# gradslam/gradslam

Measured on AMD Instinct MI355X. Metric: frames/sec PointFusion 640x480 RGB-D, higher is better.
Workload: dtype f32

## Files before the change

gradslam_amd/_C.py:

```python
import ctypes as C
import os

import torch

_HERE = os.path.dirname(os.path.abspath(__file__))
LIB_PATH = os.environ.get("GRADSLAM_HIP_LIB") or os.path.join(_HERE, "csrc", "libgradslam_hip.so")
if os.environ.get("GRADSLAM_HIP_LIB"):
    import warnings
    warnings.warn("GRADSLAM_HIP_LIB overrides the product library: %s" % LIB_PATH, RuntimeWarning)
ABI_VERSION = 3

_lib = None

_vp, _i64, _i32, _f = C.c_void_p, C.c_int64, C.c_int, C.c_float


class IcpParams(C.Structure):
    _fields_ = [("mode", C.c_int), ("numiters", C.c_int), ("damp", C.c_float),
                ("dist_thresh", C.c_float), ("lambda_max", C.c_float), ("B", C.c_float),
                ("B2", C.c_float), ("nu", C.c_float)]


class MapView(C.Structure):
    _fields_ = [("points", C.c_void_p), ("normals", C.c_void_p), ("colors", C.c_void_p), ("ccounts", C.c_void_p),
                ("capacity", C.c_int64), ("n_bound", C.c_int64), ("n_dev", C.c_void_p)]


class LocalizeSeq(C.Structure):
    _fields_ = [("vertex", C.c_void_p), ("depth", C.c_void_p), ("K16", C.c_void_p), ("prev_pose16", C.c_void_p),
                ("map", MapView), ("out_pose16", C.c_void_p), ("scratch", C.c_void_p)]


class UpdateSeq(C.Structure):
    _fields_ = [("map", MapView), ("vertex", C.c_void_p), ("normal", C.c_void_p), ("depth", C.c_void_p),
                ("rgb", C.c_void_p), ("alpha", C.c_void_p), ("pose16", C.c_void_p), ("K16", C.c_void_p),
                ("gvertex", C.c_void_p), ("gnormal", C.c_void_p), ("best_pix", C.c_void_p),
                ("new_count_out", C.c_void_p), ("scratch", C.c_void_p)]


class StepSeq(C.Structure):
    _fields_ = [("depth", C.c_void_p), ("rgb", C.c_void_p), ("K16", C.c_void_p), ("prev_pose16", C.c_void_p),
                ("out_pose16", C.c_void_p), ("vertex", C.c_void_p), ("normal", C.c_void_p), ("alpha", C.c_void_p),
                ("gvertex", C.c_void_p), ("gnormal", C.c_void_p), ("best_pix", C.c_void_p),
                ("new_count_out", C.c_void_p), ("map", MapView), ("loc_scratch", C.c_void_p),
                ("upd_scratch", C.c_void_p)]


class RenderSeq(C.Structure):
    _fields_ = [("map", MapView), ("poses16", C.c_void_p), ("K16", C.c_void_p), ("depth", C.c_void_p),
                ("color", C.c_void_p), ("normal", C.c_void_p), ("confidence", C.c_void_p), ("index", C.c_void_p),
                ("scratch", C.c_void_p)]


_PROTOS = {
    "gs_abi_version": [],
    "gs_last_error": [],
    "gs_scratch_bytes": [_i64, _i64],
    "gs_profile_begin": [_i32],
    "gs_profile_end": [],
    "gs_profile_read": [_i32, C.POINTER(C.c_double), C.POINTER(C.c_int64), C.POINTER(C.c_double)],
    "gs_frame_maps_f32": [_vp, _vp, _i32, _i32, _f, _vp, _vp, _vp, _vp, _vp],
    "gs_global_maps_f32": [_vp, _vp, _vp, _vp, _i32, _i32, _vp, _vp, _vp],
    "gs_alpha_f32": [_vp, _i64, _f, _f, _vp, _vp],
    "gs_alpha_backward_f32": [_vp, _i64, _f, _f, _vp, _vp, _vp, _vp],
    "gs_downsample_frame_f32": [_vp, _vp, _vp, _vp, _i32, _i32, _i32, _vp, _vp, _vp, _vp, _vp, _vp],
    "gs_project_map_f32": [_vp, _i64, _vp, _vp, _i32, _i32, _vp, _vp],
    "gs_active_table_i64": [_vp, _i64, _i32, _i64, _vp, _vp, _vp, _vp],
    "gs_select_targets_f32": [_vp, _i64, _i32, _i32, _vp, _vp, _vp, _vp, _vp, _vp, _i64, _vp, _vp, _vp],
    "gs_downsample_table_f32": [_vp, _i64, _i32, _vp, _vp, _vp, _vp, _vp, _vp, _vp, _vp, _vp],
    "gs_knn1_f32": [_vp, _i64, _vp, _i64, _vp, _vp, _vp, _vp],
    "gs_knn1_grid_scratch_bytes": [_i64, _i64],
    "gs_knn1_grid_f32": [_vp, _i64, _vp, _i64, _vp, _vp, _vp, C.POINTER(C.c_int64), _vp],
    "gs_gauss_newton_rows_f32": [_vp, _i64, _vp, _vp, _i64, _f, _vp, _vp, _vp, _vp, _vp, _vp],
    "gs_solve_normal_eq_f32": [_vp, _vp, _vp, _i64, _i32, _f, _vp, _vp],
    "gs_se3_exp_f32": [_vp, _vp, _vp],
    "gs_se3_exp_backward_f32": [_vp, _vp, _vp, _vp],
    "gs_transform_points_f32": [_vp, _i64, _vp, _vp, _vp],
    "gs_icp_scratch_bytes": [_i64, _i64],
    "gs_icp_f32": [_vp, _i64, _vp, _vp, _i64, _vp, _vp, C.POINTER(IcpParams), _vp, _vp, _vp, _vp],
    "gs_icp_trace_f32": [_vp, _i32, _vp, _vp],
    "gs_icp_dc_f32": [_vp, _i64, _vp, _vp, _vp, _i64, _vp, _vp, _vp, C.POINTER(IcpParams), _vp, _vp, _vp, _vp],
    "gs_frame_maps_backward_f32": [_vp, _vp, _i32, _i32, _f, _vp, _vp, _vp, _vp, _vp, _vp, _vp, _vp],
    "gs_frame_maps_backward_kbar_scratch_bytes": [_i32, _i32],
    "gs_global_maps_backward_f32": [_vp, _vp, _vp, _vp, _i32, _i32, _vp, _vp, _vp],
    "gs_downsample_frame_backward_f32": [_vp, _vp, _i32, _i32, _i32, _vp, _vp, _vp],
    "gs_icp_tape_bytes": [_i64, _i32],
    "gs_icp_tape_f32": [_vp, _i64, _vp, _vp, _i64, _vp, _vp, C.POINTER(IcpParams), _vp, _vp, _vp, _vp, _vp],
    "gs_icp_backward_scratch_bytes": [_i64, _i64],
    "gs_icp_backward_f32": [_vp, _vp, _i64, _vp, _vp, _i64, _vp, C.POINTER(IcpParams), _vp, _vp, _vp, _vp, _vp, _vp,
                            _vp],
    "gs_similar_rows_f32": [_vp, _i64, _vp, _vp, _vp, _vp, _i32, _f, _f, _vp, _vp],
    "gs_best_unique_rows_f32": [_vp, _i64, _vp, _vp, _vp, _i32, _i32, _i64, _vp, _vp, _vp, _vp, _vp],
    "gs_associate_f32": [_vp, _i64, _vp, _vp, _vp, _vp, _vp, _i32, _i32, _f, _f, _vp, _vp, _vp, _vp],
    "gs_best_table_i64": [_vp, _i32, _i32, _i64, _vp, _vp, _vp, _vp],
    "gs_rows_to_best_pix": [_vp, _i64, _i32, _i32, _vp, _vp],
    "gs_fuse_append_f32": [_vp, _vp, _vp, _vp, _i64, _i64, _vp, _vp, _vp, _vp, _vp, _vp, _i32, _i32, _i32,
                           _vp, _vp, _vp],
    "gs_append_valid_f32": [_vp, _vp, _vp, _vp, _i64, _i64, _vp, _vp, _vp, _vp, _vp, _i32, _i32, _vp, _vp, _vp],
    "gs_ingest_depth_u16_f32": [_vp, _i32, _i32, _vp, _i32, _i32, C.c_double, _vp],
    "gs_ingest_color_u8_f32": [_vp, _i32, _i32, _vp, _i32, _i32, _i32, _vp],
    "gs_ingest_frames_native_f32": [_vp, _vp, _i64, _i32, _i32, C.c_double, _i32, _vp, _vp, _vp],
    "gs_host_device_pointer": [_vp, C.POINTER(C.c_void_p)],
    "gs_global_maps_pose_backward_scratch_bytes": [_i32, _i32],
    "gs_global_maps_pose_backward_f32": [_vp, _vp, _vp, _vp, _vp, _i32, _i32, _vp, _vp, _vp],
    "gs_fuse_append_backward_f32": [_vp, _vp, _vp, _vp, _i64, _vp, _vp, _vp, _vp, _vp, _vp, _i32, _i32, _i32, _vp, _vp,
                                    _vp, _vp, _i64, _vp, _vp, _vp, _vp, _vp, _vp, _vp, _vp, _vp, _vp],
    "gs_update_map_scratch_bytes": [_i64, _i32, _i32],
    "gs_update_map_fusion_dc_f32": [_vp, _vp, _vp, _vp, _i64, _vp, _i64, _vp, _vp, _vp, _vp, _vp, _vp, _vp, _i32, _i32,
                                    _f, _f, _i32, _vp, _vp, _vp, _vp, _vp, _vp],
    "gs_icp_map_dc_f32": [_vp, _i64, _vp, _vp, _vp, _vp, _i64, _vp, _i32, _i32, _vp, _vp, C.POINTER(IcpParams), _vp, _vp,
                          _vp],
    "gs_lattice_source_f32": [_vp, _vp, _vp, _i32, _i32, _i32, _vp, _vp],
    "gs_relative_pose_f32": [_vp, _vp, _i64, _vp, _vp],
    "gs_project_map_dc_f32": [_vp, _i64, _vp, _vp, _vp, _i32, _i32, _vp, _vp],
    "gs_select_targets_dc_f32": [_vp, _i64, _vp, _i32, _i32, _vp, _vp, _vp, _vp, _vp, _vp, _i64, _vp, _vp, _vp],
    "gs_associate_dc_f32": [_vp, _i64, _vp, _vp, _vp, _vp, _vp, _vp, _i32, _i32, _f, _f, _vp, _vp, _vp, _vp],
    "gs_fuse_append_dc_f32": [_vp, _vp, _vp, _vp, _i64, _vp, _i64, _vp, _vp, _vp, _vp, _vp, _vp, _i32, _i32, _i32,
                              _vp, _vp, _vp],
    "gs_append_valid_dc_f32": [_vp, _vp, _vp, _vp, _i64, _vp, _i64, _vp, _vp, _vp, _vp, _vp, _i32, _i32, _vp, _vp,
                               _vp],
    "gs_frame_maps_batch_f32": [_vp, _i64, _i64, _vp, _i32, _i32, _i32, _i32, _f, _vp, _vp, _vp, _vp],
    "gs_localize_scratch_bytes": [_i32, _i32, _i32, _i64],
    "gs_localize_batch_f32": [C.POINTER(LocalizeSeq), _i32, _i32, _i32, _i32, C.POINTER(IcpParams), _vp],
    "gs_update_map_fusion_batch_f32": [C.POINTER(UpdateSeq), _i32, _i32, _i32, _f, _f, _i32, _vp],
    "gs_project_points_f32": [_vp, _i32, _i64, _vp, _i64, _vp, _vp],
    "gs_unproject_points_f32": [_vp, _i32, _i64, _vp, _i64, _vp, _vp, _vp],
    "gs_lie_small_f32": [_i32, _vp, _vp, _vp],
    "gs_localize_far_stats_i64": [_vp, _i32, _i32, _i32, _i64, C.POINTER(C.c_int64), _vp],
    "gs_localize_list_stats_i64": [_vp, _i32, _i32, _i32, _i64, C.POINTER(C.c_int64), _vp],
    "gs_localize_solve_stats_i64": [_vp, _i32, _i32, _i32, _i64, C.POINTER(C.c_int64), _vp],
    "gs_pointfusion_step_batch_f32": [C.POINTER(StepSeq), _i32, _i32, _i32, _i32, C.POINTER(IcpParams), _f, _f, _f, _i32, _vp],
    "gs_render_scratch_bytes": [_i32, _i32, _i32],
    "gs_render_map_dc_f32": [C.POINTER(RenderSeq), _i32, _i32, _i32, _i32, _i32, _f, _i32, _vp],
}
_RESTYPE = {"gs_last_error": C.c_char_p, "gs_scratch_bytes": _i64, "gs_icp_scratch_bytes": _i64,
            "gs_knn1_grid_scratch_bytes": _i64, "gs_update_map_scratch_bytes": _i64, "gs_global_maps_pose_backward_scratch_bytes": _i64, "gs_icp_tape_bytes": _i64, "gs_icp_backward_scratch_bytes": _i64,
            "gs_localize_scratch_bytes": _i64, "gs_frame_maps_backward_kbar_scratch_bytes": _i64,
            "gs_render_scratch_bytes": _i64}
EXPORTS = tuple(_PROTOS)


class HipExtensionError(RuntimeError):
    pass


def lib():
    global _lib
    if _lib is None:
        if not os.path.exists(LIB_PATH):
            raise HipExtensionError(
                "gradslam_amd: %s is missing. Build it with `python -m gradslam_amd.csrc.build` "
                "(hipcc --offload-arch=gfx950). There is no CPU / PyTorch fallback." % LIB_PATH)
        handle = C.CDLL(LIB_PATH)
        for name, argtypes in _PROTOS.items():
            fn = getattr(handle, name)
            fn.argtypes = argtypes
            fn.restype = _RESTYPE.get(name, C.c_int)
        if handle.gs_abi_version() != ABI_VERSION:
            raise HipExtensionError("libgradslam_hip.so ABI %d != expected %d; rebuild"
                                    % (handle.gs_abi_version(), ABI_VERSION))
        _lib = handle
    return _lib


def check(status, what):
    if status != 0:
        raise HipExtensionError("%s failed (code %d): %s" % (what, status, lib().gs_last_error().decode()))


def require_device(*tensors):
    dev = None
    for t in tensors:
        if t is None:
            continue
        if not t.is_cuda:
            raise HipExtensionError(
                "gradslam_amd kernels run on the GPU only (got a %s tensor). Move the data to a HIP "
                "device; there is no CPU fallback." % t.device)
        if not t.is_contiguous():
            raise HipExtensionError("internal error: non-contiguous tensor passed to the HIP library")
        if dev is None:
            dev = t.device
        elif t.device != dev:
            raise HipExtensionError("tensors live on different devices: %s vs %s" % (dev, t.device))
    return dev


def ptr(t):
    return None if t is None else C.c_void_p(t.data_ptr())


def stream(device):
    return C.c_void_p(torch.cuda.current_stream(device).cuda_stream)


class Workspace:
    _instances = {}

    def __init__(self, device):
        self.device = device
        self._bufs = {}

    @classmethod
    def get(cls, device):
        device = torch.device(device)
        if device.index is None:
            device = torch.device("cuda", torch.cuda.current_device())
        key = (device, torch.cuda.current_stream(device).cuda_stream)
        ws = cls._instances.get(key)
        if ws is None:
            ws = cls._instances[key] = Workspace(device)
        return ws

    def bytes(self, name, nbytes):
        buf = self._bufs.get(name)
        if buf is None or buf.numel() < nbytes:
            nbytes = int(nbytes * 1.5) + 4096
            buf = self._bufs[name] = torch.empty(nbytes, dtype=torch.uint8, device=self.device)
        return buf

    def scratch(self, n_map, n_pix):
        return self.bytes("scratch", lib().gs_scratch_bytes(int(n_map), int(n_pix)))

    def tensor(self, name, shape, dtype):
        n = 1
        for s in shape:
            n *= int(s)
        item = torch.empty((), dtype=dtype).element_size()
        buf = self.bytes(name, max(n, 1) * item)
        return buf[: n * item].view(dtype).view(*shape)
```

gradslam_amd/csrc/gs_common.h:

```cpp
#pragma once
#include <hip/hip_runtime.h>
#include <atomic>
#include <stdint.h>
#include <stdio.h>

#include "../../include/gradslam_hip.h"

#define GS_ABI_VERSION 3

constexpr int GS_MAX_BATCH = 8;
struct GsClearJob {
  int n;
  size_t bytes;
  char* ptr[GS_MAX_BATCH];
};
constexpr int GS_CLEAR_ITEMS = 8;
struct GsPixelTables {
  int n;
  uint64_t* key_pix[GS_MAX_BATCH];
  int32_t* best_pix[GS_MAX_BATCH];
  int32_t* any_flag[GS_MAX_BATCH];
  int32_t* call_flag;
};
int gs_frame_maps_batch_clear(const float* depth, int64_t depth_stride_seq, int64_t depth_stride_frame, const float* K16,
                              int n_frames, int frames_per_K, int H, int W, float two_sigma_sq, float* vertex,
                              float* normal, float* alpha, const GsClearJob* job, void* stream,
                              const GsPixelTables* tables = nullptr);

int gs_update_map_fusion_batch_impl(const gs_update_seq* seqs_host, int B, int H, int W, float dist_th, float dot_th,
                                    int renorm_all, void* stream, bool tables_ready);
int32_t* gs_update_map_call_flag(void* scratch_of_first_sequence);
void gs_update_map_tables(void* scratch, int32_t** any_flag, uint64_t** key_pix);

void gs_set_error(const char* fmt, ...);

#define GS_REQUIRE(cond, msg)                  \
  do {                                         \
    if (!(cond)) {                             \
      gs_set_error("%s: %s", __func__, msg);   \
      return GS_ERR_INVALID;                   \
    }                                          \
  } while (0)

#define GS_HIP(call)                                                            \
  do {                                                                          \
    hipError_t e_ = (call);                                                     \
    if (e_ != hipSuccess) {                                                     \
      gs_set_error("%s: %s -> %s", __func__, #call, hipGetErrorString(e_));     \
      return GS_ERR_HIP;                                                        \
    }                                                                           \
  } while (0)

#define GS_LAUNCH_CHECK() GS_HIP(hipGetLastError())

static inline hipStream_t gs_stream(void* s) { return reinterpret_cast<hipStream_t>(s); }
static inline int64_t gs_ceil_div(int64_t a, int64_t b) { return (a + b - 1) / b; }
static inline size_t gs_align(size_t x, size_t a = 256) { return (x + a - 1) / a * a; }

enum GsProfKind { GS_PROF_KNN = 0, GS_PROF_LINEARIZE = 1, GS_PROF_FRAME = 2, GS_PROF_PROJECT = 3,
                  GS_PROF_ASSOC = 4, GS_PROF_FUSE = 5, GS_PROF_COMPACT = 6, GS_PROF_SOLVE = 7, GS_PROF_ICP_FUSED = 8,
                  GS_PROF_KINDS = 9 };
extern std::atomic<bool> g_gs_prof_on;
int gs_prof_open(int kind, double work, hipStream_t st, int launches);
void gs_prof_close(int slot, hipStream_t st);
struct GsProf {
  int slot;
  hipStream_t st;
  GsProf(int kind, double work, hipStream_t s, int launches = 1) : slot(-1), st(s) {
    if (g_gs_prof_on) slot = gs_prof_open(kind, work, s, launches);
  }
  ~GsProf() {
    if (slot >= 0) gs_prof_close(slot, st);
  }
};

#define GS_DEV __device__ __forceinline__

GS_DEV float gs_fma(float a, float b, float c) { return __builtin_fmaf(a, b, c); }

GS_DEV float gs_dot3_fma(float a0, float a1, float a2, float b0, float b1, float b2) {
  float acc = a0 * b0;
  acc = gs_fma(a1, b1, acc);
  acc = gs_fma(a2, b2, acc);
  return acc;
}
GS_DEV float gs_dot3_plain(float a0, float a1, float a2, float b0, float b1, float b2) {
  float p0 = a0 * b0, p1 = a1 * b1, p2 = a2 * b2;
  float s = p0 + p1;
  return s + p2;
}
GS_DEV float gs_norm3(float x, float y, float z) {
  float acc = x * x;
  acc = gs_fma(y, y, acc);
  acc = gs_fma(z, z, acc);
  return __builtin_sqrtf(acc);
}

GS_DEV float gs_expf_spec(float x) {
  if (x < -87.0f) return 0.0f;
  if (x > 88.0f) return __builtin_inff();
  float n = __builtin_rintf(x * 1.44269504088896341f);
  float r = gs_fma(-n, 0.693359375f, x);
  r = gs_fma(-n, -2.12194440e-4f, r);
  float p = 1.9875691500e-4f;
  p = gs_fma(p, r, 1.3981999507e-3f);
  p = gs_fma(p, r, 8.3334519073e-3f);
  p = gs_fma(p, r, 4.1665795894e-2f);
  p = gs_fma(p, r, 1.6666665459e-1f);
  p = gs_fma(p, r, 5.0000001201e-1f);
  float r2 = r * r;
  float y = gs_fma(p, r2, r);
  y = y + 1.0f;
  int32_t bits = __float_as_int(y) + (((int32_t)n) << 23);
  return __int_as_float(bits);
}

GS_DEV float gs_alpha_of(float vx, float vy, float vz, float two_sigma_sq, float eps) {
  float s = vx * vx + vy * vy;
  s = s + vz * vz;
  float a = gs_expf_spec((-s) / two_sigma_sq);
  a = a < eps ? eps : a;
  a = a > 1.01f ? 1.01f : a;
  return a;
}

struct GsKinv {
  float k00, k11, k02, k12;
};
GS_DEV GsKinv gs_kinv(const float* __restrict__ K) {
  const float eps = 1e-6f;
  float fx = K[0], fy = K[5], cx = K[2], cy = K[6];
  GsKinv r;
  r.k00 = 1.0f / (fx + eps);
  r.k11 = 1.0f / (fy + eps);
  r.k02 = (-1.0f * cx) / (fx + eps);
  r.k12 = (-1.0f * cy) / (fy + eps);
  return r;
}

GS_DEV void gs_rigid_fma(const float* __restrict__ T, float p0, float p1, float p2, float& o0,
                         float& o1, float& o2) {
  o0 = gs_dot3_fma(T[0], T[1], T[2], p0, p1, p2) + T[3];
  o1 = gs_dot3_fma(T[4], T[5], T[6], p0, p1, p2) + T[7];
  o2 = gs_dot3_fma(T[8], T[9], T[10], p0, p1, p2) + T[11];
}

struct GsCount {
  int64_t host;
  const int64_t* dev;
};
GS_DEV int64_t gs_count(const GsCount c) {
  if (!c.dev) return c.host;
  const int64_t raw = *c.dev;
  const uint32_t lo = (uint32_t)__builtin_amdgcn_readfirstlane((int)(uint32_t)raw);
  const uint32_t hi = (uint32_t)__builtin_amdgcn_readfirstlane((int)(uint32_t)((uint64_t)raw >> 32));
  const int64_t v = (int64_t)(((uint64_t)hi << 32) | lo);
  return v < c.host ? (v < 0 ? 0 : v) : c.host;
}

constexpr int GS_WAVE = 64;

GS_DEV int gs_wave_incl_scan(int v) {
  const int lane = threadIdx.x & (GS_WAVE - 1);
#pragma unroll
  for (int d = 1; d < GS_WAVE; d <<= 1) {
    int t = __shfl_up(v, d, GS_WAVE);
    if (lane >= d) v += t;
  }
  return v;
}

template <int BLOCK>
GS_DEV int gs_block_excl_scan(int v, int* smem, int* total) {
  constexpr int NW = BLOCK / GS_WAVE;
  const int lane = threadIdx.x & (GS_WAVE - 1);
  const int wave = threadIdx.x / GS_WAVE;
  int incl = gs_wave_incl_scan(v);
  if (lane == GS_WAVE - 1) smem[wave] = incl;
  __syncthreads();
  if (threadIdx.x == 0) {
    int run = 0;
    for (int w = 0; w < NW; ++w) {
      int c = smem[w];
      smem[w] = run;
      run += c;
    }
    smem[NW] = run;
  }
  __syncthreads();
  int base = smem[wave];
  *total = smem[NW];
  __syncthreads();
  return base + incl - v;
}

GS_DEV double gs_wave_sum_f64(double v) {
#pragma unroll
  for (int d = GS_WAVE / 2; d > 0; d >>= 1) v += __shfl_down(v, d, GS_WAVE);
  return v;
}
```

gradslam_amd/csrc/gs_frame.hip:

```cpp
#include <stdarg.h>
#include <string.h>

#include "gs_compact.h"

static thread_local char g_err[512] = "";

void gs_set_error(const char* fmt, ...) {
  va_list ap;
  va_start(ap, fmt);
  vsnprintf(g_err, sizeof(g_err), fmt, ap);
  va_end(ap);
}

#include <mutex>
#include <vector>
std::atomic<bool> g_gs_prof_on{false};
namespace {
std::mutex g_prof_mu;
struct ProfRec { hipEvent_t a, b; int kind; double work; bool closed; int launches; };
std::vector<ProfRec> g_prof;
size_t g_prof_used = 0;
double g_prof_ms[GS_PROF_KINDS], g_prof_work[GS_PROF_KINDS];
int64_t g_prof_n[GS_PROF_KINDS];
}
// ... 12 lines not shown
}

extern "C" int gs_profile_begin(int max_records) {
  GS_REQUIRE(max_records > 0 && max_records <= (1 << 20), "max_records out of range");
  std::lock_guard<std::mutex> lock(g_prof_mu);
  while (g_prof.size() < (size_t)max_records) {
    ProfRec r;
    GS_HIP(hipEventCreate(&r.a));
    GS_HIP(hipEventCreate(&r.b));
    r.kind = 0; r.work = 0; r.closed = false; r.launches = 1;
    g_prof.push_back(r);
  }
  g_prof_used = 0;
  for (int k = 0; k < GS_PROF_KINDS; ++k) { g_prof_ms[k] = 0; g_prof_work[k] = 0; g_prof_n[k] = 0; }
  g_gs_prof_on = true;
  return GS_OK;
}
extern "C" int gs_profile_end(void) {
  g_gs_prof_on = false;
  GS_HIP(hipDeviceSynchronize());
  std::lock_guard<std::mutex> lock(g_prof_mu);
  for (size_t i = 0; i < g_prof_used; ++i) {
    const ProfRec& r = g_prof[i];
    if (!r.closed) continue;
    float ms = 0.f;
    if (hipEventElapsedTime(&ms, r.a, r.b) != hipSuccess) continue;
    g_prof_ms[r.kind] += ms; g_prof_work[r.kind] += r.work; g_prof_n[r.kind] += r.launches;
  }
  return GS_OK;
}
extern "C" int gs_profile_read(int kind, double* ms_total, int64_t* launches, double* work_total) {
  GS_REQUIRE(kind >= 0 && kind < GS_PROF_KINDS && ms_total && launches && work_total, "bad arguments");
  std::lock_guard<std::mutex> lock(g_prof_mu);
  *ms_total = g_prof_ms[kind]; *launches = g_prof_n[kind]; *work_total = g_prof_work[kind];
  return GS_OK;
}

extern "C" int gs_abi_version(void) { return GS_ABI_VERSION; }
extern "C" const char* gs_last_error(void) { return g_err; }

extern "C" int64_t gs_scratch_bytes(int64_t n_map, int64_t n_pix) {
  int64_t n = n_map > n_pix ? n_map : n_pix;
  return (int64_t)(gs_cp_scratch_bytes(n) + gs_align(8 * (size_t)(n_pix > 0 ? n_pix : 1)) +
                   gs_align(8 * (size_t)(n_map > 0 ? n_map : 1)) + 4096);
}

__global__ void gs_cp_scan_tiles_kernel(const int32_t* __restrict__ tile_counts, int64_t ntiles,
                                        int64_t* __restrict__ tile_offsets,
                                        int64_t* __restrict__ count_out, GsCount base_count) {
  __shared__ int smem[1024 / GS_WAVE + 1];
  __shared__ int64_t carry;
  if (threadIdx.x == 0) carry = 0;
  __syncthreads();
  for (int64_t t0 = 0; t0 < ntiles; t0 += 1024) {
    int64_t t = t0 + threadIdx.x;
    int c = (t < ntiles) ? tile_counts[t] : 0;
    int total;
    int excl = gs_block_excl_scan<1024>(c, smem, &total);
    if (t < ntiles) tile_offsets[t] = carry + excl;
    __syncthreads();
    if (threadIdx.x == 0) carry += total;
    __syncthreads();
  }
  if (threadIdx.x == 0 && count_out) count_out[0] = gs_count(base_count) + carry;
}

constexpr int FM_TW = 64;
constexpr int FM_TH = 8;
constexpr int FM_LW = FM_TW + 2;
constexpr int FM_LH = FM_TH + 2;

GS_DEV void fm_vertex(float d, int h, int w, const GsKinv& k, float& x, float& y, float& z) {
  float u = (float)w, v = (float)h;
  float ax = k.k00 * u;
  ax = gs_fma(0.0f, v, ax);
  ax = gs_fma(k.k02, 1.0f, ax);
  float ay = 0.0f * u;
  ay = gs_fma(k.k11, v, ay);
  ay = gs_fma(k.k12, 1.0f, ay);
  float az = 0.0f * u;
  az = gs_fma(0.0f, v, az);
  az = gs_fma(1.0f, 1.0f, az);
  float validf = d > 0.0f ? 1.0f : 0.0f;
  x = (ax * d) * validf;
  y = (ay * d) * validf;
  z = (az * d) * validf;
}

struct GsRow3 {
  float x, y, z;
};
GS_DEV void frame_maps_body(const float* __restrict__ depth, const float* __restrict__ K16, int H, int W,
                            float two_sigma_sq, float* __restrict__ vertex, float* __restrict__ normal,
                            float* __restrict__ alpha, uint8_t* __restrict__ valid,
                            uint64_t* __restrict__ key_pix = nullptr, int32_t* __restrict__ best_pix = nullptr) {
  __shared__ float tile[FM_LH][FM_LW];
  const int w_base = blockIdx.x * FM_TW, h_base = blockIdx.y * FM_TH;
  for (int i = threadIdx.x; i < FM_LH * FM_LW; i += 256) {
    int lh = i / FM_LW, lw = i - lh * FM_LW;
    int gh = h_base + lh - 1, gw = w_base + lw - 1;
    gh = gh < 0 ? 0 : (gh > H - 1 ? H - 1 : gh);
    gw = gw < 0 ? 0 : (gw > W - 1 ? W - 1 : gw);
    tile[lh][lw] = depth[(size_t)gh * W + gw];
  }
  __syncthreads();
  const GsKinv k = gs_kinv(K16);
  const int lane = threadIdx.x & 63, wave = threadIdx.x >> 6;
  const int w = w_base + lane;
  if (w >= W) return;
#pragma unroll
  for (int r = 0; r < 2; ++r) {
    const int lh = wave * 2 + r;
    const int h = h_base + lh;
    if (h >= H) continue;
    const size_t p = (size_t)h * W + w;
    const float d = tile[lh + 1][lane + 1];
    float vx, vy, vz;
    fm_vertex(d, h, w, k, vx, vy, vz);
    if (vertex) reinterpret_cast<GsRow3*>(vertex)[p] = GsRow3{vx, vy, vz};
    if (valid) valid[p] = d > 0.0f ? 1 : 0;
    if (alpha) alpha[p] = gs_alpha_of(vx, vy, vz, two_sigma_sq, 1e-7f);
    if (key_pix) { key_pix[p] = ~0ull; best_pix[p] = -1; }
    if (normal) {
      const int w0 = (w < W - 1) ? w : W - 2;
      const int h0 = (h < H - 1) ? h : H - 2;
      const int lw0 = w0 - w_base + 1, lh0 = h0 - h_base + 1;
      float a0x, a0y, a0z, a1x, a1y, a1z, b0x, b0y, b0z, b1x, b1y, b1z;
      fm_vertex(tile[lh + 1][lw0], h, w0, k, a0x, a0y, a0z);
      fm_vertex(tile[lh + 1][lw0 + 1], h, w0 + 1, k, a1x, a1y, a1z);
      fm_vertex(tile[lh0][lane + 1], h0, w, k, b0x, b0y, b0z);
      fm_vertex(tile[lh0 + 1][lane + 1], h0 + 1, w, k, b1x, b1y, b1z);
      const float dhx = a1x - a0x, dhy = a1y - a0y, dhz = a1z - a0z;
      const float dvx = b1x - b0x, dvy = b1y - b0y, dvz = b1z - b0z;
      const float nx = gs_fma(dhy, dvz, -(dhz * dvy));
      const float ny = gs_fma(dhz, dvx, -(dhx * dvz));
      const float nz = gs_fma(dhx, dvy, -(dhy * dvx));
      const float nrm = gs_norm3(nx, ny, nz);
      const float den = (nrm == 0.0f) ? 1.0f : nrm;
      const float validf = d > 0.0f ? 1.0f : 0.0f;
      reinterpret_cast<GsRow3*>(normal)[p] = GsRow3{(nx / den) * validf, (ny / den) * validf, (nz / den) * validf};
    }
  }
}

__global__ void __launch_bounds__(256) gs_frame_maps_kernel(
    const float* __restrict__ depth, const float* __restrict__ K16, int H, int W, float two_sigma_sq,
    float* __restrict__ vertex, float* __restrict__ normal, float* __restrict__ alpha,
    uint8_t* __restrict__ valid) {
  frame_maps_body(depth, K16, H, W, two_sigma_sq, vertex, normal, alpha, valid);
}
__global__ void __launch_bounds__(256) gs_frame_maps_batch_kernel(
    const float* __restrict__ depth, int64_t stride_seq, int64_t stride_frame, const float* __restrict__ K16,
    int frames_per_K, int H, int W, float two_sigma_sq, float* __restrict__ vertex, float* __restrict__ normal,
    float* __restrict__ alpha, const int n_frames, const GsClearJob job, const GsPixelTables tabs) {
  if ((int)blockIdx.z >= n_frames) {
    const size_t blk = ((size_t)(blockIdx.z - n_frames) * gridDim.y + blockIdx.y) * gridDim.x + blockIdx.x;
    const size_t n16 = job.bytes / 16, per = (n16 + 256 * GS_CLEAR_ITEMS - 1) / (256 * GS_CLEAR_ITEMS);
    const size_t r = blk / per;
    if (r >= (size_t)job.n) return;
    float4* dst = reinterpret_cast<float4*>(job.ptr[r]);
    const size_t base = (blk % per) * 256 * GS_CLEAR_ITEMS + threadIdx.x;
#pragma unroll
    for (int u = 0; u < GS_CLEAR_ITEMS; ++u) {
      const size_t i = base + (size_t)u * 256;
      if (i < n16) dst[i] = make_float4(0.0f, 0.0f, 0.0f, 0.0f);
    }
    return;
  }
  const size_t f = blockIdx.z, P = (size_t)H * W;
  const size_t b = f / frames_per_K, l = f % frames_per_K;
  const bool tb = (int)f < tabs.n;
  if (tb && blockIdx.x == 0 && blockIdx.y == 0 && threadIdx.x == 0) {
    tabs.any_flag[f][0] = 0;
    tabs.any_flag[f][1] = 0;
    if (f == 0 && tabs.call_flag) *tabs.call_flag = 0;
  }
  frame_maps_body(depth + b * stride_seq + l * stride_frame, K16 + 16 * b, H, W, two_sigma_sq, vertex + 3 * f * P,
                  normal ? normal + 3 * f * P : nullptr, alpha ? alpha + f * P : nullptr, nullptr,
                  tb ? tabs.key_pix[f] : nullptr, tb ? tabs.best_pix[f] : nullptr);
}

extern "C" int gs_frame_maps_f32(const float* depth, const float* K16, int H, int W,
                                 float two_sigma_sq, float* vertex, float* normal, float* alpha,
                                 uint8_t* valid, void* stream) {
  GS_REQUIRE(depth && K16, "depth and K16 must not be NULL");
  GS_REQUIRE(H >= 2 && W >= 2, "image must be at least 2x2");
  dim3 grid((unsigned)gs_ceil_div(W, FM_TW), (unsigned)gs_ceil_div(H, FM_TH));
  const double bytes = (double)H * W * (4.0 + (vertex ? 12 : 0) + (normal ? 12 : 0) + (alpha ? 4 : 0) + (valid ? 1 : 0));
  GsProf prof(GS_PROF_FRAME, bytes, gs_stream(stream));
  hipLaunchKernelGGL(gs_frame_maps_kernel, grid, dim3(256), 0, gs_stream(stream), depth, K16, H, W,
                     two_sigma_sq, vertex, normal, alpha, valid);
  GS_LAUNCH_CHECK();
  return GS_OK;
}

int gs_frame_maps_batch_clear(const float* depth, int64_t depth_stride_seq, int64_t depth_stride_frame, const float* K16,
                              int n_frames, int frames_per_K, int H, int W, float two_sigma_sq, float* vertex,
                              float* normal, float* alpha, const GsClearJob* job, void* stream,
                              const GsPixelTables* tables) {
  GS_REQUIRE(depth && K16 && vertex, "depth, K16 and vertex must not be NULL");
  GsPixelTables tabs;
  tabs.n = 0; tabs.call_flag = nullptr;
  if (tables && tables->n > 0) {
    GS_REQUIRE(tables->n <= GS_MAX_BATCH && tables->n <= n_frames, "bad pixel tables");
    tabs = *tables;
  }
  GS_REQUIRE(H >= 2 && W >= 2, "image must be at least 2x2");
  GS_REQUIRE(n_frames > 0 && n_frames <= 65535 && frames_per_K > 0 && n_frames % frames_per_K == 0, "bad frame count");
  GS_REQUIRE(depth_stride_frame >= (int64_t)H * W && depth_stride_seq >= 0, "bad depth strides");
  dim3 grid((unsigned)gs_ceil_div(W, FM_TW), (unsigned)gs_ceil_div(H, FM_TH), (unsigned)n_frames);
  GsClearJob none;
  none.n = 0; none.bytes = 0;
  if (job && job->n > 0 && job->bytes > 0) {
    GS_REQUIRE(job->n <= GS_MAX_BATCH && job->bytes % 16 == 0, "bad clear job");
    const int64_t per = gs_ceil_div((int64_t)(job->bytes / 16), 256 * GS_CLEAR_ITEMS);
    const int64_t slices = gs_ceil_div(per * job->n, (int64_t)grid.x * grid.y);
    GS_REQUIRE(n_frames + slices <= 65535, "clear job too large for the launch");
    grid.z += (unsigned)slices;
  } else {
    job = &none;
  }
  const double bytes = (double)n_frames * H * W * (4.0 + 12.0 + (normal ? 12 : 0) + (alpha ? 4 : 0)) +
                       (double)tabs.n * H * W * 12.0;
  GsProf prof(GS_PROF_FRAME, bytes, gs_stream(stream));
  hipLaunchKernelGGL(gs_frame_maps_batch_kernel, grid, dim3(256), 0, gs_stream(stream), depth, depth_stride_seq,
                     depth_stride_frame, K16, frames_per_K, H, W, two_sigma_sq, vertex, normal, alpha, n_frames, *job, tabs);
  GS_LAUNCH_CHECK();
  return GS_OK;
}

extern "C" int gs_frame_maps_batch_f32(const float* depth, int64_t depth_stride_seq, int64_t depth_stride_frame,
                                       const float* K16, int n_frames, int frames_per_K, int H, int W,
                                       float two_sigma_sq, float* vertex, float* normal, float* alpha, void* stream) {
  return gs_frame_maps_batch_clear(depth, depth_stride_seq, depth_stride_frame, K16, n_frames, frames_per_K, H, W,
                                   two_sigma_sq, vertex, normal, alpha, nullptr, stream);
}

__global__ void __launch_bounds__(256) gs_global_maps_kernel(
    const float* __restrict__ vertex, const float* __restrict__ normal,
    const float* __restrict__ depth, const float* __restrict__ pose16, int64_t P,
    float* __restrict__ gvertex, float* __restrict__ gnormal) {
  const int64_t p = (int64_t)blockIdx.x * 256 + threadIdx.x;
  if (p >= P) return;
  float T[12];
#pragma unroll
  for (int i = 0; i < 12; ++i) T[i] = pose16[i];
  if (gvertex) {
    const float v0 = vertex[3 * p], v1 = vertex[3 * p + 1], v2 = vertex[3 * p + 2];
    const float validf = depth[p] > 0.0f ? 1.0f : 0.0f;
    float g0, g1, g2;
    gs_rigid_fma(T, v0, v1, v2, g0, g1, g2);
    gvertex[3 * p] = g0 * validf;
    gvertex[3 * p + 1] = g1 * validf;
    gvertex[3 * p + 2] = g2 * validf;
  }
  if (gnormal) {
    const float n0 = normal[3 * p], n1 = normal[3 * p + 1], n2 = normal[3 * p + 2];
    gnormal[3 * p] = gs_dot3_fma(T[0], T[1], T[2], n0, n1, n2);
    gnormal[3 * p + 1] = gs_dot3_fma(T[4], T[5], T[6], n0, n1, n2);
    gnormal[3 * p + 2] = gs_dot3_fma(T[8], T[9], T[10], n0, n1, n2);
  }
}

extern "C" int gs_global_maps_f32(const float* vertex, const float* normal, const float* depth,
                                  const float* pose16, int H, int W, float* gvertex,
                                  float* gnormal, void* stream) {
  GS_REQUIRE(H > 0 && W > 0, "empty image");
  GS_REQUIRE(!gvertex || (vertex && depth), "gvertex needs vertex and depth");
  GS_REQUIRE(!gnormal || normal, "gnormal needs normal");
  const int64_t P = (int64_t)H * W;
  hipStream_t st = gs_stream(stream);
  if (!pose16) {
    if (gvertex) GS_HIP(hipMemcpyAsync(gvertex, vertex, P * 12, hipMemcpyDeviceToDevice, st));
    if (gnormal) GS_HIP(hipMemcpyAsync(gnormal, normal, P * 12, hipMemcpyDeviceToDevice, st));
    return GS_OK;
  }
  GsProf prof(GS_PROF_FRAME, (double)P * (4.0 + (gvertex ? 24 : 0) + (gnormal ? 24 : 0)), st);
  hipLaunchKernelGGL(gs_global_maps_kernel, dim3((unsigned)gs_ceil_div(P, 256)), dim3(256), 0, st,
                     vertex, normal, depth, pose16, P, gvertex, gnormal);
  GS_LAUNCH_CHECK();
  return GS_OK;
}

__global__ void __launch_bounds__(256) gs_alpha_kernel(const float* __restrict__ pts, int64_t n,
                                                       float two_sigma_sq, float eps,
                                                       float* __restrict__ alpha) {
  const int64_t i = (int64_t)blockIdx.x * 256 + threadIdx.x;
  if (i >= n) return;
  alpha[i] = gs_alpha_of(pts[3 * i], pts[3 * i + 1], pts[3 * i + 2], two_sigma_sq, eps);
}

extern "C" int gs_alpha_f32(const float* points, int64_t n, float two_sigma_sq, float eps,
                            float* alpha, void* stream) {
  GS_REQUIRE(n >= 0, "negative n");
  if (n == 0) return GS_OK;
  GS_REQUIRE(points && alpha, "NULL pointer");
  hipLaunchKernelGGL(gs_alpha_kernel, dim3((unsigned)gs_ceil_div(n, 256)), dim3(256), 0,
                     gs_stream(stream), points, n, two_sigma_sq, eps, alpha);
  GS_LAUNCH_CHECK();
  return GS_OK;
}

__global__ void __launch_bounds__(256) gs_alpha_bwd_kernel(const float* __restrict__ pts, int64_t n, float two_sigma_sq,
                                                           float eps, const float* __restrict__ alpha_bar,
                                                           float* __restrict__ pts_bar, float* __restrict__ sigma_terms) {
  const int64_t i = (int64_t)blockIdx.x * 256 + threadIdx.x;
  if (i >= n) return;
  const float x = pts[3 * i], y = pts[3 * i + 1], z = pts[3 * i + 2];
  float S = x * x + y * y;
  S = S + z * z;
  const float a = gs_expf_spec((-S) / two_sigma_sq);
  const bool pass = a >= eps && a <= 1.01f;
  const float g = pass ? alpha_bar[i] * a : 0.0f;
  const float k = -2.0f / two_sigma_sq;
  pts_bar[3 * i] = g * k * x;
  pts_bar[3 * i + 1] = g * k * y;
  pts_bar[3 * i + 2] = g * k * z;
  if (sigma_terms) sigma_terms[i] = g * S;
}

extern "C" int gs_alpha_backward_f32(const float* points, int64_t n, float two_sigma_sq, float eps,
                                     const float* alpha_bar, float* points_bar, float* sigma_terms, void* stream) {
  GS_REQUIRE(n >= 0, "negative n");
  if (n == 0) return GS_OK;
  GS_REQUIRE(points && alpha_bar && points_bar, "NULL pointer");
  hipLaunchKernelGGL(gs_alpha_bwd_kernel, dim3((unsigned)gs_ceil_div(n, 256)), dim3(256), 0, gs_stream(stream), points, n,
                     two_sigma_sq, eps, alpha_bar, points_bar, sigma_terms);
  GS_LAUNCH_CHECK();
  return GS_OK;
}

GS_DEV void fb_ray(int h, int w, const GsKinv& k, float& rx, float& ry) {
  rx = k.k00 * (float)w + k.k02;
  ry = k.k11 * (float)h + k.k12;
}
GS_DEV void fb_vertex(const float* __restrict__ depth, int W, int h, int w, const GsKinv& k, float* v) {
  const float d = depth[(size_t)h * W + w];
  float rx, ry;
  fb_ray(h, w, k, rx, ry);
  const float m = d > 0.0f ? 1.0f : 0.0f;
  v[0] = rx * d * m; v[1] = ry * d * m; v[2] = d * m;
}

__global__ void __launch_bounds__(256) gs_frame_bwd_diff_kernel(const float* __restrict__ depth,
                                                                const float* __restrict__ K16, int H, int W,
                                                                const float* __restrict__ normal_bar,
                                                                float* __restrict__ dhdv_bar) {
  const int64_t p = (int64_t)blockIdx.x * 256 + threadIdx.x;
  if (p >= (int64_t)H * W) return;
  const int h = (int)(p / W), w = (int)(p % W);
  const GsKinv k = gs_kinv(K16);
  const int w0 = (w < W - 1) ? w : W - 2, h0 = (h < H - 1) ? h : H - 2;
  float a0[3], a1[3], b0[3], b1[3];
  fb_vertex(depth, W, h, w0, k, a0);
  fb_vertex(depth, W, h, w0 + 1, k, a1);
  fb_vertex(depth, W, h0, w, k, b0);
  fb_vertex(depth, W, h0 + 1, w, k, b1);
  const float dh[3] = {a1[0] - a0[0], a1[1] - a0[1], a1[2] - a0[2]};
  const float dv[3] = {b1[0] - b0[0], b1[1] - b0[1], b1[2] - b0[2]};
  const float nr[3] = {dh[1] * dv[2] - dh[2] * dv[1], dh[2] * dv[0] - dh[0] * dv[2], dh[0] * dv[1] - dh[1] * dv[0]};
  const float nrm = sqrtf(nr[0] * nr[0] + nr[1] * nr[1] + nr[2] * nr[2]);
  const float m = depth[p] > 0.0f ? 1.0f : 0.0f;
  const float g[3] = {normal_bar[3 * p] * m, normal_bar[3 * p + 1] * m, normal_bar[3 * p + 2] * m};
  float nb[3];
  if (nrm > 0.0f) {
    const float inv = 1.0f / nrm;
    const float nh[3] = {nr[0] * inv, nr[1] * inv, nr[2] * inv};
    const float dot = nh[0] * g[0] + nh[1] * g[1] + nh[2] * g[2];
    for (int c = 0; c < 3; ++c) nb[c] = (g[c] - nh[c] * dot) * inv;
  } else {
    for (int c = 0; c < 3; ++c) nb[c] = g[c];
  }
  float* o = dhdv_bar + 6 * p;
  o[0] = dv[1] * nb[2] - dv[2] * nb[1];
  o[1] = dv[2] * nb[0] - dv[0] * nb[2];
  o[2] = dv[0] * nb[1] - dv[1] * nb[0];
  o[3] = nb[1] * dh[2] - nb[2] * dh[1];
  o[4] = nb[2] * dh[0] - nb[0] * dh[2];
  o[5] = nb[0] * dh[1] - nb[1] * dh[0];
// ... 156 lines not shown
```

gradslam_amd/csrc/gs_fuse.hip:

```cpp
#include "gs_assoc_dev.h"
#include "gs_compact.h"

__global__ void __launch_bounds__(256) gs_fuse_init_kernel(int32_t* __restrict__ pix_of, int64_t n,
                                                           int32_t* __restrict__ any_flag) {
  const int64_t i = (int64_t)blockIdx.x * 256 + threadIdx.x;
  if (i == 0) *any_flag = 0;
  if (i < n) pix_of[i] = -1;
}

__global__ void __launch_bounds__(256) gs_fuse_scatter_kernel(const int32_t* __restrict__ best_pix,
                                                              int64_t P, GsCount n_map_c,
                                                              int32_t* __restrict__ pix_of,
                                                              int32_t* __restrict__ any_flag) {
  const int64_t p = (int64_t)blockIdx.x * 256 + threadIdx.x;
  if (p >= P) return;
  const int32_t n = best_pix[p];
  if (n >= 0 && n < gs_count(n_map_c)) {
    pix_of[n] = (int32_t)p;
    *any_flag = 1;
  }
}

struct FrameGlobalMaps {
  const float* __restrict__ gvertex;
  const float* __restrict__ gnormal;
  __device__ void operator()(const int64_t p, float* fp, float* fn) const {
#pragma unroll
    for (int k = 0; k < 3; ++k) {
      fp[k] = gvertex[3 * p + k];
      fn[k] = gnormal[3 * p + k];
    }
  }
  __device__ void vertex_of(const int64_t p, float* fp) const {
#pragma unroll
    for (int k = 0; k < 3; ++k) fp[k] = gvertex[3 * p + k];
  }
  __device__ void normal_of(const int64_t p, float* fn) const {
#pragma unroll
    for (int k = 0; k < 3; ++k) fn[k] = gnormal[3 * p + k];
  }
};
struct FrameLocalMaps {
  const float* __restrict__ vertex;
  const float* __restrict__ normal;
  float T[12];
  __device__ void operator()(const int64_t p, float* fp, float* fn) const {
    float v[3], n[3];
#pragma unroll
    for (int k = 0; k < 3; ++k) {
      v[k] = vertex[3 * p + k];
      n[k] = normal[3 * p + k];
    }
    const float validf = v[2] > 0.0f ? 1.0f : 0.0f;
    float g0, g1, g2;
    gs_rigid_fma(T, v[0], v[1], v[2], g0, g1, g2);
    fp[0] = g0 * validf; fp[1] = g1 * validf; fp[2] = g2 * validf;
    fn[0] = gs_dot3_fma(T[0], T[1], T[2], n[0], n[1], n[2]);
    fn[1] = gs_dot3_fma(T[4], T[5], T[6], n[0], n[1], n[2]);
    fn[2] = gs_dot3_fma(T[8], T[9], T[10], n[0], n[1], n[2]);
  }
  __device__ void vertex_of(const int64_t p, float* fp) const {
    float v[3];
#pragma unroll
    for (int k = 0; k < 3; ++k) v[k] = vertex[3 * p + k];
    const float validf = v[2] > 0.0f ? 1.0f : 0.0f;
    float g0, g1, g2;
    gs_rigid_fma(T, v[0], v[1], v[2], g0, g1, g2);
    fp[0] = g0 * validf; fp[1] = g1 * validf; fp[2] = g2 * validf;
  }
  __device__ void normal_of(const int64_t p, float* fn) const {
    float n[3];
#pragma unroll
    for (int k = 0; k < 3; ++k) n[k] = normal[3 * p + k];
    fn[0] = gs_dot3_fma(T[0], T[1], T[2], n[0], n[1], n[2]);
    fn[1] = gs_dot3_fma(T[4], T[5], T[6], n[0], n[1], n[2]);
    fn[2] = gs_dot3_fma(T[8], T[9], T[10], n[0], n[1], n[2]);
  }
};
GS_DEV FrameLocalMaps frame_local_maps(const float* vertex, const float* normal, const float* pose16) {
  FrameLocalMaps f;
  f.vertex = vertex; f.normal = normal;
#pragma unroll
  for (int i = 0; i < 12; ++i) f.T[i] = pose16[i];
  return f;
}

template <class Frame>
GS_DEV void fuse_merge_row(float* __restrict__ points, float* __restrict__ normals, float* __restrict__ colors,
                           float* __restrict__ ccounts, const int64_t n, const int32_t p, const Frame& frame,
                           const float* __restrict__ rgb, const float* __restrict__ alpha) {
  const float a = p >= 0 ? alpha[p] : 0.0f;
  const float cc = ccounts[n];
  float P[3], N[3], C[3], fp[3] = {0.0f, 0.0f, 0.0f}, fn[3] = {0.0f, 0.0f, 0.0f}, fc[3] = {0.0f, 0.0f, 0.0f};
#pragma unroll
  for (int k = 0; k < 3; ++k) {
    P[k] = points[3 * n + k];
    N[k] = normals[3 * n + k];
    C[k] = colors[3 * n + k];
  }
  if (p >= 0) {
    frame((int64_t)p, fp, fn);
#pragma unroll
    for (int k = 0; k < 3; ++k) fc[k] = rgb[3 * (int64_t)p + k];
  }
  const float cc2 = cc + a;
  const float inv = 1.0f / (cc2 == 0.0f ? 1.0f : cc2);
#pragma unroll
  for (int k = 0; k < 3; ++k) {
    P[k] = ((cc * P[k]) + (a * fp[k])) * inv;
    N[k] = ((cc * N[k]) + (a * fn[k])) * inv;
    C[k] = ((cc * C[k]) + (a * fc[k])) * inv;
  }
#pragma unroll
  for (int k = 0; k < 3; ++k) points[3 * n + k] = P[k];
#pragma unroll
  for (int k = 0; k < 3; ++k) normals[3 * n + k] = N[k];
#pragma unroll
  for (int k = 0; k < 3; ++k) colors[3 * n + k] = C[k];
  ccounts[n] = cc2;
}

__global__ void __launch_bounds__(256) gs_fuse_merge_kernel(
    float* __restrict__ points, float* __restrict__ normals, float* __restrict__ colors,
    float* __restrict__ ccounts, GsCount n_map_c, const int32_t* __restrict__ pix_of,
    const int32_t* __restrict__ any_flag, const float* __restrict__ gvertex,
    const float* __restrict__ gnormal, const float* __restrict__ rgb, const float* __restrict__ alpha,
    int renorm_all) {
  const int64_t n = (int64_t)blockIdx.x * 256 + threadIdx.x;
  if (n >= gs_count(n_map_c)) return;
  if (*any_flag == 0 && renorm_all != 2) return;
  const int32_t p = pix_of[n];
  if (p < 0 && !renorm_all) return;
  fuse_merge_row(points, normals, colors, ccounts, n, p, FrameGlobalMaps{gvertex, gnormal}, rgb, alpha);
}

struct PredNewPixel {
  const float* depth;
  const int32_t* best_pix;
  __device__ bool operator()(int64_t p) const {
    return depth[p] > 0.0f && (best_pix == nullptr || best_pix[p] < 0);
  }
};
template <class Frame>
struct EmitAppendT {
  float* points;
  float* normals;
  float* colors;
  float* ccounts;
  GsCount n_map;
  Frame frame;
  const float* rgb;
  const float* alpha;
  __device__ void operator()(int64_t p, int64_t pos) const {
    const int64_t r = gs_count(n_map) + pos;
    float v[3], nn[3] = {0.0f, 0.0f, 0.0f}, c[3] = {0.0f, 0.0f, 0.0f};
    frame.vertex_of(p, v);
    if (normals) frame.normal_of(p, nn);
    if (colors) {
#pragma unroll
      for (int k = 0; k < 3; ++k) c[k] = rgb[3 * p + k];
    }
    const float a = ccounts ? alpha[p] : 0.0f;
#pragma unroll
    for (int k = 0; k < 3; ++k) points[3 * r + k] = v[k];
    if (normals) {
#pragma unroll
      for (int k = 0; k < 3; ++k) normals[3 * r + k] = nn[k];
    }
    if (colors) {
#pragma unroll
      for (int k = 0; k < 3; ++k) colors[3 * r + k] = c[k];
    }
    if (ccounts) ccounts[r] = a;
  }
};
typedef EmitAppendT<FrameGlobalMaps> EmitAppend;

static int fuse_append(float* points, float* normals, float* colors, float* ccounts, GsCount n_map_c,
                       int64_t capacity, const int32_t* best_pix, const float* gvertex, const float* gnormal,
                       const float* rgb, const float* alpha, const float* depth, int H, int W, int renorm_all,
                       int64_t* new_count_out, void* scratch, void* stream) {
  const int64_t n_map_host = n_map_c.host;
  GS_REQUIRE(H > 0 && W > 0 && n_map_host >= 0 && capacity >= n_map_host, "bad sizes");
  GS_REQUIRE(points && normals && colors && ccounts && best_pix && gvertex && gnormal && rgb && alpha &&
                 depth && new_count_out && scratch,
             "NULL pointer");
  hipStream_t st = gs_stream(stream);
  const int64_t P = (int64_t)H * W;
  const int64_t n_map = n_map_host;
  char* base = reinterpret_cast<char*>(scratch) + gs_cp_scratch_bytes(P > n_map ? P : n_map);
  int32_t* any_flag = reinterpret_cast<int32_t*>(base);
  int32_t* pix_of = reinterpret_cast<int32_t*>(base + 256);
  GsProf prof(GS_PROF_FUSE, 88.0 * (double)n_map + 45.0 * (double)P, st);
  if (n_map > 0) {
    hipLaunchKernelGGL(gs_fuse_init_kernel, dim3((unsigned)gs_ceil_div(n_map, 256)), dim3(256), 0, st,
                       pix_of, n_map, any_flag);
    hipLaunchKernelGGL(gs_fuse_scatter_kernel, dim3((unsigned)gs_ceil_div(P, 256)), dim3(256), 0, st,
                       best_pix, P, n_map_c, pix_of, any_flag);
    hipLaunchKernelGGL(gs_fuse_merge_kernel, dim3((unsigned)gs_ceil_div(n_map, 256)), dim3(256), 0, st,
                       points, normals, colors, ccounts, n_map_c, pix_of, any_flag, gvertex, gnormal, rgb,
                       alpha, renorm_all);
    GS_LAUNCH_CHECK();
  }
  EmitAppend emit{points, normals, colors, ccounts, n_map_c, FrameGlobalMaps{gvertex, gnormal}, rgb, alpha};
  return gs_compact(GsCount{P, nullptr}, PredNewPixel{depth, best_pix}, emit, new_count_out, n_map_c, capacity,
                    scratch, st);
}

extern "C" int gs_fuse_append_f32(float* points, float* normals, float* colors, float* ccounts,
                                  int64_t n_map_host, int64_t capacity, const int32_t* best_pix,
                                  const float* gvertex, const float* gnormal, const float* rgb,
                                  const float* alpha, const float* depth, int H, int W, int renorm_all,
                                  int64_t* new_count_out, void* scratch, void* stream) {
  return fuse_append(points, normals, colors, ccounts, GsCount{n_map_host, nullptr}, capacity, best_pix, gvertex,
                     gnormal, rgb, alpha, depth, H, W, renorm_all, new_count_out, scratch, stream);
}
extern "C" int gs_fuse_append_dc_f32(float* points, float* normals, float* colors, float* ccounts,
                                     int64_t n_map_bound, const int64_t* n_map_dev, int64_t capacity,
                                     const int32_t* best_pix, const float* gvertex, const float* gnormal,
                                     const float* rgb, const float* alpha, const float* depth, int H, int W,
                                     int renorm_all, int64_t* new_count_out, void* scratch, void* stream) {
  GS_REQUIRE(n_map_dev && capacity >= n_map_bound + (int64_t)H * W, "device-count fuse needs capacity >= bound + H*W");
  return fuse_append(points, normals, colors, ccounts, GsCount{n_map_bound, n_map_dev}, capacity, best_pix,
                     gvertex, gnormal, rgb, alpha, depth, H, W, renorm_all, new_count_out, scratch, stream);
}

static int append_valid(float* points, float* normals, float* colors, float* ccounts, GsCount n_map_c,
                        int64_t capacity, const float* gvertex, const float* gnormal, const float* rgb,
                        const float* alpha, const float* depth, int H, int W, int64_t* new_count_out,
                        void* scratch, void* stream) {
  GS_REQUIRE(H > 0 && W > 0 && n_map_c.host >= 0 && capacity >= n_map_c.host, "bad sizes");
  GS_REQUIRE(points && gvertex && depth && new_count_out && scratch, "NULL pointer");
  EmitAppend emit{points, gnormal ? normals : nullptr, rgb ? colors : nullptr, alpha ? ccounts : nullptr,
                  n_map_c, FrameGlobalMaps{gvertex, gnormal}, rgb, alpha};
  return gs_compact(GsCount{(int64_t)H * W, nullptr}, PredNewPixel{depth, nullptr}, emit, new_count_out, n_map_c,
                    capacity, scratch, gs_stream(stream));
}
extern "C" int gs_append_valid_f32(float* points, float* normals, float* colors, float* ccounts,
                                   int64_t n_map_host, int64_t capacity, const float* gvertex,
                                   const float* gnormal, const float* rgb, const float* alpha,
                                   const float* depth, int H, int W, int64_t* new_count_out,
                                   void* scratch, void* stream) {
  return append_valid(points, normals, colors, ccounts, GsCount{n_map_host, nullptr}, capacity, gvertex, gnormal,
                      rgb, alpha, depth, H, W, new_count_out, scratch, stream);
}
extern "C" int gs_append_valid_dc_f32(float* points, float* normals, float* colors, float* ccounts,
                                      int64_t n_map_bound, const int64_t* n_map_dev, int64_t capacity,
                                      const float* gvertex, const float* gnormal, const float* rgb,
                                      const float* alpha, const float* depth, int H, int W,
                                      int64_t* new_count_out, void* scratch, void* stream) {
  GS_REQUIRE(n_map_dev && capacity >= n_map_bound + (int64_t)H * W, "device-count append needs capacity >= bound + H*W");
  return append_valid(points, normals, colors, ccounts, GsCount{n_map_bound, n_map_dev}, capacity, gvertex,
                      gnormal, rgb, alpha, depth, H, W, new_count_out, scratch, stream);
}

__global__ void __launch_bounds__(256) gs_fuse_bwd_rows_kernel(
    const float* __restrict__ points, const float* __restrict__ normals, const float* __restrict__ colors,
    const float* __restrict__ ccounts, int64_t n_old, const int32_t* __restrict__ pix_of,
    const int32_t* __restrict__ any_flag, const float* __restrict__ gvertex, const float* __restrict__ gnormal,
    const float* __restrict__ rgb, const float* __restrict__ alpha, int renorm_all,
    const float* __restrict__ P_bar, const float* __restrict__ N_bar, const float* __restrict__ C_bar,
    const float* __restrict__ F_bar, float* __restrict__ oP_bar, float* __restrict__ oN_bar,
    float* __restrict__ oC_bar, float* __restrict__ oF_bar, float* __restrict__ gv_bar, float* __restrict__ gn_bar,
    float* __restrict__ rgb_bar, float* __restrict__ alpha_bar) {
  const int64_t n = (int64_t)blockIdx.x * 256 + threadIdx.x;
  if (n >= n_old) return;
  const int32_t p = (*any_flag != 0) ? pix_of[n] : -1;
  if ((*any_flag == 0 && renorm_all != 2) || (p < 0 && !renorm_all)) {
#pragma unroll
    for (int k = 0; k < 3; ++k) {
      oP_bar[3 * n + k] = P_bar[3 * n + k];
      oN_bar[3 * n + k] = N_bar[3 * n + k];
      oC_bar[3 * n + k] = C_bar[3 * n + k];
    }
    oF_bar[n] = F_bar[n];
    return;
  }
  const double a = p >= 0 ? (double)alpha[p] : 0.0;
  const double cc = (double)ccounts[n];
  const double cc2 = cc + a;
  const double inv = 1.0 / (cc2 == 0.0 ? 1.0 : cc2);
  double inv_bar = 0.0, cc_bar = 0.0, a_bar = 0.0;
  const float* olds[3] = {points, normals, colors};
  const float* frames[3] = {gvertex, gnormal, rgb};
  const float* bars[3] = {P_bar, N_bar, C_bar};
  float* obars[3] = {oP_bar, oN_bar, oC_bar};
  float* fbars[3] = {gv_bar, gn_bar, rgb_bar};
#pragma unroll
  for (int t = 0; t < 3; ++t) {
#pragma unroll
    for (int k = 0; k < 3; ++k) {
      const double x = (double)olds[t][3 * n + k];
      const double f = p >= 0 ? (double)frames[t][3 * (int64_t)p + k] : 0.0;
      const double xb = (double)bars[t][3 * n + k];
      const double ub = xb * inv;
      inv_bar += xb * (cc * x + a * f);
      obars[t][3 * n + k] = (float)(cc * ub);
      if (p >= 0) fbars[t][3 * (int64_t)p + k] = (float)(a * ub);
      cc_bar += x * ub;
      a_bar += f * ub;
    }
  }
  const double cc2_bar = (double)F_bar[n] + (cc2 != 0.0 ? -inv * inv * inv_bar : 0.0);
  oF_bar[n] = (float)(cc_bar + cc2_bar);
  if (p >= 0) alpha_bar[p] = (float)(a_bar + cc2_bar);
}

struct EmitAppendBackward {
  const float* P_bar;
  const float* N_bar;
  const float* C_bar;
  const float* F_bar;
  int64_t n_old;
  float* gv_bar;
  float* gn_bar;
  float* rgb_bar;
  float* alpha_bar;
  __device__ void operator()(int64_t p, int64_t pos) const {
    const int64_t r = n_old + pos;
#pragma unroll
    for (int k = 0; k < 3; ++k) {
      gv_bar[3 * p + k] = P_bar[3 * r + k];
      gn_bar[3 * p + k] = N_bar[3 * r + k];
      rgb_bar[3 * p + k] = C_bar[3 * r + k];
    }
    alpha_bar[p] = F_bar[r];
  }
};

extern "C" int gs_fuse_append_backward_f32(const float* points, const float* normals, const float* colors,
                                           const float* ccounts, int64_t n_old, const int32_t* best_pix,
                                           const float* gvertex, const float* gnormal, const float* rgb,
                                           const float* alpha, const float* depth, int H, int W, int renorm_all,
                                           const float* P_bar, const float* N_bar, const float* C_bar,
                                           const float* F_bar, int64_t n_new, float* old_points_bar,
                                           float* old_normals_bar, float* old_colors_bar, float* old_ccounts_bar,
                                           float* gvertex_bar, float* gnormal_bar, float* rgb_bar, float* alpha_bar,
                                           void* scratch, void* stream) {
  GS_REQUIRE(H > 0 && W > 0 && n_old >= 0 && n_new >= n_old, "bad sizes");
  GS_REQUIRE(best_pix && gvertex && gnormal && rgb && alpha && depth && P_bar && N_bar && C_bar && F_bar && gvertex_bar &&
                 gnormal_bar && rgb_bar && alpha_bar && scratch,
             "NULL pointer");
  hipStream_t st = gs_stream(stream);
  const int64_t P = (int64_t)H * W;
  GS_HIP(hipMemsetAsync(gvertex_bar, 0, 12 * (size_t)P, st));
  GS_HIP(hipMemsetAsync(gnormal_bar, 0, 12 * (size_t)P, st));
  GS_HIP(hipMemsetAsync(rgb_bar, 0, 12 * (size_t)P, st));
  GS_HIP(hipMemsetAsync(alpha_bar, 0, 4 * (size_t)P, st));
  char* base = reinterpret_cast<char*>(scratch) + gs_cp_scratch_bytes(P > n_old ? P : n_old);
  int32_t* any_flag = reinterpret_cast<int32_t*>(base);
  int32_t* pix_of = reinterpret_cast<int32_t*>(base + 256);
  if (n_old > 0) {
    GS_REQUIRE(points && normals && colors && ccounts && old_points_bar && old_normals_bar && old_colors_bar &&
                   old_ccounts_bar,
               "NULL pointer");
    const GsCount n_old_c{n_old, nullptr};
    hipLaunchKernelGGL(gs_fuse_init_kernel, dim3((unsigned)gs_ceil_div(n_old, 256)), dim3(256), 0, st, pix_of, n_old,
                       any_flag);
    hipLaunchKernelGGL(gs_fuse_scatter_kernel, dim3((unsigned)gs_ceil_div(P, 256)), dim3(256), 0, st, best_pix, P,
                       n_old_c, pix_of, any_flag);
    hipLaunchKernelGGL(gs_fuse_bwd_rows_kernel, dim3((unsigned)gs_ceil_div(n_old, 256)), dim3(256), 0, st, points,
                       normals, colors, ccounts, n_old, pix_of, any_flag, gvertex, gnormal, rgb, alpha, renorm_all, P_bar,
                       N_bar, C_bar, F_bar, old_points_bar, old_normals_bar, old_colors_bar, old_ccounts_bar,
                       gvertex_bar, gnormal_bar, rgb_bar, alpha_bar);
    GS_LAUNCH_CHECK();
  }
  EmitAppendBackward emit{P_bar, N_bar, C_bar, F_bar, n_old, gvertex_bar, gnormal_bar, rgb_bar, alpha_bar};
  int64_t* cnt = reinterpret_cast<int64_t*>(base + 128);
  return gs_compact(P, PredNewPixel{depth, best_pix}, emit, cnt, 0, n_new - n_old, scratch, st);
}

constexpr int32_t MU_TIE_MARK = 0x7fffffff;
struct MuSeq {
  float* points; float* normals; float* colors; float* ccounts;
  GsCount n_map;
  int64_t capacity;
  const float* vertex; const float* normal; const float* depth; const float* rgb; const float* alpha;
  const float* pose16; const float* K16;
  float* gvertex; float* gnormal;
  int32_t* best_pix;
  int64_t* new_count_out;
  int32_t* any_flag;
  uint64_t* key_pix;
  int32_t* tile_counts;
  uint64_t* key_pt;
  int32_t* pix;
  int32_t* pix_of;
};
struct MuBatch {
  int B, H, W, renorm_all;
  int64_t P, ntiles;
  float u_hi, v_hi, dist_th, dot_th;
  int32_t* call_flag;
  int zero_call_flag;
  MuSeq s[GS_MAX_BATCH];
};

__global__ void __launch_bounds__(256) gs_mu_pixel_init_kernel(const MuBatch mb) {
  const MuSeq& q = mb.s[blockIdx.x % mb.B];
  const int64_t p = (int64_t)(blockIdx.x / mb.B) * 256 + threadIdx.x;
  if (p == 0) { q.any_flag[0] = 0; q.any_flag[1] = 0; }
  if (blockIdx.x == 0 && threadIdx.x == 0 && mb.zero_call_flag) *mb.call_flag = 0;
  if (p >= mb.P) return;
  float T[12];
#pragma unroll
  for (int i = 0; i < 12; ++i) T[i] = q.pose16[i];
  const float validf = q.depth[p] > 0.0f ? 1.0f : 0.0f;
  float g0, g1, g2;
  gs_rigid_fma(T, q.vertex[3 * p], q.vertex[3 * p + 1], q.vertex[3 * p + 2], g0, g1, g2);
  q.gvertex[3 * p] = g0 * validf;
  q.gvertex[3 * p + 1] = g1 * validf;
  q.gvertex[3 * p + 2] = g2 * validf;
  const float n0 = q.normal[3 * p], n1 = q.normal[3 * p + 1], n2 = q.normal[3 * p + 2];
  q.gnormal[3 * p] = gs_dot3_fma(T[0], T[1], T[2], n0, n1, n2);
  q.gnormal[3 * p + 1] = gs_dot3_fma(T[4], T[5], T[6], n0, n1, n2);
  q.gnormal[3 * p + 2] = gs_dot3_fma(T[8], T[9], T[10], n0, n1, n2);
  q.key_pix[p] = ~0ull;
  q.best_pix[p] = -1;
}

__global__ void __launch_bounds__(256) gs_mu_project_key_kernel(const MuBatch mb) {
  const MuSeq& q = mb.s[blockIdx.x % mb.B];
  const int64_t n = (int64_t)(blockIdx.x / mb.B) * 256 + threadIdx.x;
  if (n >= gs_count(q.n_map)) return;
  const GsCamera c = gs_camera(q.pose16, q.K16);
  const int32_t p = gs_project_point(c, q.points[3 * n], q.points[3 * n + 1], q.points[3 * n + 2], mb.H, mb.W, mb.u_hi,
                                     mb.v_hi);
  int32_t pk = -1;
  if (p >= 0) {
    float fp[3], fn[3];
    if (q.gvertex) FrameGlobalMaps{q.gvertex, q.gnormal}((int64_t)p, fp, fn);
    else frame_local_maps(q.vertex, q.normal, q.pose16)((int64_t)p, fp, fn);
    if (gs_is_similar_v(q.points, q.normals, fp, fn, n, mb.dist_th, mb.dot_th)) {
      const uint64_t k = gs_assoc_key_v(q.points, q.ccounts, fp, n);
      const unsigned long long old = atomicMin(reinterpret_cast<unsigned long long*>(&q.key_pix[p]), (unsigned long long)k);
      if (old == (unsigned long long)k) {
        q.best_pix[p] = MU_TIE_MARK;
        q.any_flag[1] = 1;
      }
      q.key_pt[n] = k;
      pk = p;
    }
  }
  q.pix[n] = pk;
}

GS_DEV void mu_settle_ties(const MuSeq& q, const unsigned blk, const unsigned nblk) {
  if (q.any_flag[1] == 0) return;
  const int64_t n_map = gs_count(q.n_map);
  for (int64_t n = (int64_t)blk * GS_CP_BLOCK + threadIdx.x; n < n_map; n += (int64_t)nblk * GS_CP_BLOCK) {
    const int32_t p = q.pix[n];
    if (p < 0 || q.best_pix[p] == -1) continue;
    if (q.key_pt[n] == q.key_pix[p]) atomicMin(reinterpret_cast<unsigned*>(&q.best_pix[p]), (unsigned)n);
  }
}

__global__ void __launch_bounds__(GS_CP_BLOCK) gs_mu_winner_count_kernel(const MuBatch mb) {
  __shared__ int smem[GS_CP_BLOCK / GS_WAVE + 1];
  const MuSeq& q = mb.s[blockIdx.x % mb.B];
  const unsigned blk = blockIdx.x / mb.B;
  const int64_t base = (int64_t)blk * GS_CP_TILE + (int64_t)threadIdx.x * GS_CP_ITEMS;
  int c = 0;
  uint64_t kk[GS_CP_ITEMS];
  float dd[GS_CP_ITEMS];
#pragma unroll
  for (int i = 0; i < GS_CP_ITEMS; ++i) {
    const int64_t pc = base + i < mb.P ? base + i : mb.P - 1;
    kk[i] = q.key_pix[pc];
    dd[i] = q.depth[pc];
  }
  bool any = false;
#pragma unroll
  for (int i = 0; i < GS_CP_ITEMS; ++i) {
    const int64_t p = base + i;
    if (p < mb.P) {
      const bool matched = kk[i] != ~0ull;
      any = any || matched;
      if (dd[i] > 0.0f && !matched) ++c;
    }
  }
  if (any) {
    q.any_flag[0] = 1;
    *mb.call_flag = 1;
  }
  int total;
  (void)gs_block_excl_scan<GS_CP_BLOCK>(c, smem, &total);
  if (threadIdx.x == 0) q.tile_counts[blk] = total;
  mu_settle_ties(q, blk, gridDim.x / mb.B);
}

GS_DEV void mu_merge_body(const MuBatch& mb, const unsigned bid) {
  const MuSeq& q = mb.s[bid % mb.B];
  const int64_t n = (int64_t)(bid / mb.B) * 256 + threadIdx.x;
  if (n >= gs_count(q.n_map)) return;
  if (*mb.call_flag == 0) return;
  int32_t p = q.pix[n];
  if (p >= 0) {
    bool win = q.key_pt[n] == q.key_pix[p];
    if (win) {
      const int32_t bp = q.best_pix[p];
      win = bp == -1 || bp == (int32_t)n;
      if (win && bp == -1) q.best_pix[p] = (int32_t)n;
    }
    if (!win) p = -1;
  }
  if (p < 0 && !mb.renorm_all) return;
  if (q.gvertex) fuse_merge_row(q.points, q.normals, q.colors, q.ccounts, n, p, FrameGlobalMaps{q.gvertex, q.gnormal}, q.rgb, q.alpha);
  else fuse_merge_row(q.points, q.normals, q.colors, q.ccounts, n, p, frame_local_maps(q.vertex, q.normal, q.pose16), q.rgb, q.alpha);
}

GS_DEV void mu_append_body(const MuBatch& mb, const unsigned bid) {
  __shared__ int smem[GS_CP_BLOCK / GS_WAVE + 1];
  const MuSeq& q = mb.s[bid % mb.B];
  const unsigned blk = bid / mb.B;
  int before = 0, all = 0;
  for (int64_t t = threadIdx.x; t < mb.ntiles; t += GS_CP_BLOCK) {
    const int v = q.tile_counts[t];
    all += v;
    if (t < (int64_t)blk) before += v;
  }
  int tile_prefix, total_new, tile_new;
  (void)gs_block_excl_scan<GS_CP_BLOCK>(before, smem, &tile_prefix);
  (void)gs_block_excl_scan<GS_CP_BLOCK>(all, smem, &total_new);
  const int64_t n_map = gs_count(q.n_map);
  if (blk == 0 && threadIdx.x == 0) q.new_count_out[0] = n_map + total_new;
  const int64_t base = (int64_t)blk * GS_CP_TILE + (int64_t)threadIdx.x * GS_CP_ITEMS;
  bool keep[GS_CP_ITEMS];
  int c = 0;
  {
    uint64_t kk[GS_CP_ITEMS];
    float dd[GS_CP_ITEMS];
#pragma unroll
    for (int i = 0; i < GS_CP_ITEMS; ++i) {
      const int64_t pc = base + i < mb.P ? base + i : mb.P - 1;
      kk[i] = q.key_pix[pc];
      dd[i] = q.depth[pc];
    }
#pragma unroll
    for (int i = 0; i < GS_CP_ITEMS; ++i) {
      keep[i] = base + i < mb.P && dd[i] > 0.0f && kk[i] == ~0ull;
      c += keep[i] ? 1 : 0;
    }
  }
  int w = gs_block_excl_scan<GS_CP_BLOCK>(c, smem, &tile_new);
  __shared__ unsigned short loc_s[GS_CP_TILE];
#pragma unroll
  for (int i = 0; i < GS_CP_ITEMS; ++i) {
    if (keep[i]) loc_s[w++] = (unsigned short)(threadIdx.x * GS_CP_ITEMS + i);
  }
  __syncthreads();
  const int64_t tile_base = (int64_t)blk * GS_CP_TILE;
  if (q.gvertex) {
    const EmitAppend emit{q.points, q.normals, q.colors, q.ccounts, q.n_map, FrameGlobalMaps{q.gvertex, q.gnormal}, q.rgb, q.alpha};
    for (int r = threadIdx.x; r < tile_new; r += GS_CP_BLOCK) {
      const int64_t pos = (int64_t)tile_prefix + r;
      if (n_map + pos < q.capacity) emit(tile_base + loc_s[r], pos);
    }
  } else {
    const EmitAppendT<FrameLocalMaps> emit{q.points, q.normals, q.colors, q.ccounts, q.n_map,
                                           frame_local_maps(q.vertex, q.normal, q.pose16), q.rgb, q.alpha};
    for (int r = threadIdx.x; r < tile_new; r += GS_CP_BLOCK) {
      const int64_t pos = (int64_t)tile_prefix + r;
      if (n_map + pos < q.capacity) emit(tile_base + loc_s[r], pos);
    }
  }
}

static_assert(GS_CP_BLOCK == 256, "merge and append blocks share a launch");
__global__ void __launch_bounds__(256) gs_mu_merge_append_kernel(const MuBatch mb, const unsigned nb_append) {
  if (blockIdx.x < nb_append) mu_append_body(mb, blockIdx.x);
  else mu_merge_body(mb, blockIdx.x - nb_append);
}

extern "C" int64_t gs_update_map_scratch_bytes(int64_t n_map_bound, int H, int W) {
  const int64_t P = (int64_t)H * W;
  return (int64_t)(256 + gs_align(8 * (size_t)P) + gs_align(4 * (size_t)gs_cp_tiles(P)) +
                   gs_align(8 * (size_t)(n_map_bound > 0 ? n_map_bound : 1)) +
                   2 * gs_align(4 * (size_t)(n_map_bound > 0 ? n_map_bound : 1)) + 4096);
}

int32_t* gs_update_map_call_flag(void* scratch0) { return reinterpret_cast<int32_t*>(scratch0) + 32; }
void gs_update_map_tables(void* scratch, int32_t** any_flag, uint64_t** key_pix) {
  *any_flag = reinterpret_cast<int32_t*>(scratch);
  *key_pix = reinterpret_cast<uint64_t*>(reinterpret_cast<char*>(scratch) + 256);
}

static int update_chunk(const gs_update_seq* seqs, int B, int H, int W, float dist_th, float dot_th, int renorm_all,
                        hipStream_t st, int phase, int32_t* call_flag, bool first_chunk, bool tables_ready) {
  MuBatch mb;
  mb.B = B; mb.H = H; mb.W = W; mb.renorm_all = renorm_all;
  mb.call_flag = call_flag; mb.zero_call_flag = first_chunk ? 1 : 0;
  mb.P = (int64_t)H * W;
  mb.ntiles = gs_cp_tiles(mb.P);
  mb.u_hi = (float)((double)W - 0.999); mb.v_hi = (float)((double)H - 0.999);
  mb.dist_th = dist_th; mb.dot_th = dot_th;
  int64_t n_max = 0;
  double bytes_assoc = 0.0, bytes_fuse = 0.0;
  for (int b = 0; b < B; ++b) {
    const gs_update_seq& u = seqs[b];
    const int64_t n_map = u.map.n_bound;
    n_max = n_map > n_max ? n_map : n_max;
    char* q = reinterpret_cast<char*>(u.scratch);
    MuSeq& m = mb.s[b];
    m.points = u.map.points; m.normals = u.map.normals; m.colors = u.map.colors; m.ccounts = u.map.ccounts;
    m.n_map = GsCount{u.map.n_bound, u.map.n_dev};
    m.capacity = u.map.capacity;
    m.vertex = u.vertex; m.normal = u.normal; m.depth = u.depth; m.rgb = u.rgb; m.alpha = u.alpha;
    m.pose16 = u.pose16; m.K16 = u.K16;
    m.gvertex = u.gvertex; m.gnormal = u.gnormal; m.best_pix = u.best_pix; m.new_count_out = u.new_count_out;
    m.any_flag = reinterpret_cast<int32_t*>(q); q += 256;
    m.key_pix = reinterpret_cast<uint64_t*>(q); q += gs_align(8 * (size_t)mb.P);
    m.tile_counts = reinterpret_cast<int32_t*>(q); q += gs_align(4 * (size_t)mb.ntiles);
    m.key_pt = reinterpret_cast<uint64_t*>(q); q += gs_align(8 * (size_t)(n_map > 0 ? n_map : 1));
    m.pix = reinterpret_cast<int32_t*>(q); q += gs_align(4 * (size_t)(n_map > 0 ? n_map : 1));
    m.pix_of = reinterpret_cast<int32_t*>(q);
    bytes_assoc += 72.0 * (double)n_map;
    bytes_fuse += 104.0 * (double)n_map + 49.0 * (double)mb.P;
  }
  const unsigned uB = (unsigned)B;
  const unsigned pb = uB * (unsigned)gs_ceil_div(mb.P, 256), nb = uB * (unsigned)gs_ceil_div(n_max > 0 ? n_max : 1, 256);
  if (phase == 0) {
    if (!tables_ready) {
      GsProf prof(GS_PROF_FRAME, (double)B * (double)mb.P * 64.0, st);
      hipLaunchKernelGGL(gs_mu_pixel_init_kernel, dim3(pb), dim3(256), 0, st, mb);
    }
    if (n_max > 0) {
      GsProf prof(GS_PROF_ASSOC, bytes_assoc, st, 1);
      hipLaunchKernelGGL(gs_mu_project_key_kernel, dim3(nb), dim3(256), 0, st, mb);
    }
    GsProf prof(GS_PROF_FUSE, bytes_fuse / 3.0, st, 1);
    hipLaunchKernelGGL(gs_mu_winner_count_kernel, dim3(uB * (unsigned)mb.ntiles), dim3(GS_CP_BLOCK), 0, st, mb);
  } else {
    GsProf prof(GS_PROF_FUSE, bytes_fuse * (2.0 / 3.0), st, 1);
    const unsigned nb_append = uB * (unsigned)mb.ntiles;
    hipLaunchKernelGGL(gs_mu_merge_append_kernel, dim3(nb_append + (n_max > 0 ? nb : 0u)), dim3(256), 0, st, mb, nb_append);
  }
  GS_LAUNCH_CHECK();
  return GS_OK;
}

int gs_update_map_fusion_batch_impl(const gs_update_seq* seqs_host, int B, int H, int W, float dist_th, float dot_th,
                                    int renorm_all, void* stream, bool tables_ready) {
  GS_REQUIRE(seqs_host && B > 0 && H > 0 && W > 0, "bad arguments");
  GS_REQUIRE((int64_t)H * W < (1ll << 31), "too large for int32 indices");
  for (int b = 0; b < B; ++b) {
    const gs_update_seq& u = seqs_host[b];
    GS_REQUIRE(u.map.n_bound >= 0 && u.map.n_bound < 0x7fffffff, "bad map size");
    GS_REQUIRE(u.map.capacity >= u.map.n_bound + (int64_t)H * W, "capacity must cover n_bound + H*W rows");
    GS_REQUIRE(u.map.points && u.map.normals && u.map.colors && u.map.ccounts && u.vertex && u.normal && u.depth && u.rgb &&
                   u.alpha && u.pose16 && u.K16 && u.best_pix && u.new_count_out && u.scratch,
               "NULL pointer");
    GS_REQUIRE((u.gvertex && u.gnormal) || (tables_ready && !u.gvertex && !u.gnormal), "gvertex / gnormal: both or none");
    GS_REQUIRE(u.new_count_out != u.map.n_dev, "new_count_out must not alias the map's device count");
  }
  hipStream_t st = gs_stream(stream);
  int32_t* call_flag = gs_update_map_call_flag(seqs_host[0].scratch);
  for (int phase = 0; phase < 2; ++phase) {
    for (int c0 = 0; c0 < B; c0 += GS_MAX_BATCH) {
      const int nb = B - c0 < GS_MAX_BATCH ? B - c0 : GS_MAX_BATCH;
      const int rc = update_chunk(seqs_host + c0, nb, H, W, dist_th, dot_th, renorm_all, st, phase, call_flag, c0 == 0,
                                  tables_ready);
      if (rc != GS_OK) return rc;
    }
  }
  return GS_OK;
}

extern "C" int gs_update_map_fusion_batch_f32(const gs_update_seq* seqs_host, int B, int H, int W, float dist_th,
                                              float dot_th, int renorm_all, void* stream) {
  return gs_update_map_fusion_batch_impl(seqs_host, B, H, W, dist_th, dot_th, renorm_all, stream, false);
}

extern "C" int gs_update_map_fusion_dc_f32(float* points, float* normals, float* colors, float* ccounts,
                                           int64_t n_map_bound, const int64_t* n_map_dev, int64_t capacity,
                                           const float* vertex, const float* normal, const float* depth,
                                           const float* rgb, const float* alpha, const float* pose16,
                                           const float* K16, int H, int W, float dist_th, float dot_th,
                                           int renorm_all, float* gvertex, float* gnormal, int32_t* best_pix,
                                           int64_t* new_count_out, void* scratch, void* stream) {
  gs_update_seq u;
  u.map = gs_map_view{points, normals, colors, ccounts, capacity, n_map_bound, n_map_dev};
  u.vertex = vertex; u.normal = normal; u.depth = depth; u.rgb = rgb; u.alpha = alpha;
  u.pose16 = pose16; u.K16 = K16;
  u.gvertex = gvertex; u.gnormal = gnormal; u.best_pix = best_pix; u.new_count_out = new_count_out; u.scratch = scratch;
  return gs_update_map_fusion_batch_f32(&u, 1, H, W, dist_th, dot_th, renorm_all, stream);
}
```

gradslam_amd/csrc/gs_icp_loop.hip:

```cpp
#include <stdlib.h>
#include <string.h>

#include <memory>
#include <type_traits>

#include "gs_icp_math.h"
#include "gs_knn.h"
#include "gs_knn_bbox.h"

constexpr int GS_ICP_MAX_ITERS = 1024;
struct GsIcpState {
  IcpSmall s[2];
  float trace[GS_ICP_MAX_ITERS * 12];
};

struct TapePtrs {
  float* src;
  int32_t* idx;
  float* sys;
};
GS_DEV void tape_write_sys(float* __restrict__ sys, int it, const double* S, float damp) {
  float* t = sys + 28 * it;
  for (int i = 0; i < 27; ++i) t[i] = (float)S[i];
  t[27] = damp;
// ... 1022 lines not shown
  GS_REQUIRE(prm, "params_host must not be NULL");
  GS_REQUIRE(n_src > 0 && n_tgt > 0, "empty point set");
  GS_REQUIRE(n_tgt < 0x7fffffffll && n_src < 0x7fffffffll, "too many points");
  GS_REQUIRE(src && tgt && tgt_normals && init16 && out_T16 && icp_scratch, "NULL pointer");
  GS_REQUIRE(prm->numiters >= 0 && prm->numiters <= GS_ICP_MAX_ITERS, "numiters must be in [0, 1024]");
  GS_REQUIRE(prm->mode == 0 || prm->mode == 1, "mode must be 0 (ICP) or 1 (gradICP)");
  hipStream_t st = gs_stream(stream);
  IcpScratch sc = icp_carve(icp_scratch, n_src);
  hipLaunchKernelGGL(gs_icp_init_kernel, dim3(1), dim3(64), 0, st, sc.state, init16, prm->damp, prm->numiters,
                     compose16, out_T16);
  const bool dev_counts = n_src_dev || n_tgt_dev || flt.pix;
  const bool use_grid = prm->numiters > 0 && (dev_counts || (icp_grid_enabled() && gs_knn_use_grid(n_src, n_tgt)));
  const GsCount n_src_c{n_src, n_src_dev}, n_tgt_c{n_tgt, n_tgt_dev};
  float* bufs[2] = {sc.srcA, sc.srcB};
  TapePtrs tp = {nullptr, nullptr, nullptr};
  if (tape) {
    GsIcpTape t = gs_icp_tape_carve(tape, n_src, prm->numiters);
    tp.src = t.src; tp.idx = t.idx; tp.sys = t.sys;
  }
  auto cloud = [&](int it) { return tp.src ? tp.src + (size_t)it * 3 * (size_t)n_src : bufs[it & 1]; };
  auto tidx = [&](int it, int which) { return tp.idx ? tp.idx + ((size_t)it * 2 + which) * (size_t)n_src : nullptr; };

  if (use_grid) {
    int rc = gs_knn_grid_build(tgt, n_tgt_c, n_src, sc.grid, st, flt, tgt_normals);
    if (rc != GS_OK) return rc;
    GridMem gm = grid_carve(sc.grid, n_src, n_tgt);
    const int nfs = (int)icp_rows(n_src);
    const bool reduce_rows = nfs > FS_REDUCE_ROWS;
    const float* cur_in = src;
    int h = 0;
    double prof_bytes = 0.0;
    if (g_gs_prof_on) {
      int64_t n_binned = n_tgt;
      if (flt.pix) {
        unsigned hits = 0;
        GS_HIP(hipMemcpyAsync(&hits, gm.bbox + 6, 4, hipMemcpyDeviceToHost, st));
        GS_HIP(hipStreamSynchronize(st));
        n_binned = hits;
      }
      prof_bytes = icp_alg_bytes(prm->numiters, n_src, n_src, n_binned);
    }
    std::unique_ptr<GsProf> prof_loop(new GsProf(GS_PROF_ICP_FUSED, prof_bytes, st, 2 * prm->numiters));
    const IcpHalfPlan plan = icp_half_plan(n_src, 1);
    IcpHalfBatch hb;
    hb.B = 1;
    hb.weak_room = 0.0f;
    hb.l[0] = IcpHalfLists{nullptr, nullptr, nullptr, nullptr};
    hb.w[0] = IcpHalfWide{nullptr, nullptr};
    for (int it = 0; it < prm->numiters; ++it) {
      float* cur = cloud(it);
      hb.s[0] = IcpHalfSeq{cur_in, cur, tgt, tgt_normals, n_tgt_c, gm.g, gm.cell_start, gm.sorted, gm.sorted_n,
                           reinterpret_cast<float*>(sc.best), sc.partials[(h + 1) & 1], sc.partials[h & 1], &sc.state->s[h & 1], &sc.state->s[(h + 1) & 1],
                           sc.state->trace, out_idx, tidx(it, 0), nullptr};
      icp_half_launch<true>(plan, hb, n_src_c, prm, it, 0, st);
      ++h;
      if (reduce_rows) {
        GsProf prof(GS_PROF_SOLVE, 1.0, st);
        hipLaunchKernelGGL(gs_icp_reduce_rows_kernel, dim3(1), dim3(FS_BLOCK), 0, st, sc.partials[(h + 1) & 1], n_src_c,
                           sc.rowred);
      }
      hb.s[0] = IcpHalfSeq{cur, nullptr, tgt, tgt_normals, n_tgt_c, gm.g, gm.cell_start, gm.sorted, gm.sorted_n,
                           reinterpret_cast<float*>(sc.best), reduce_rows ? sc.rowred : sc.partials[(h + 1) & 1], sc.partials[h & 1], &sc.state->s[h & 1],
                           &sc.state->s[(h + 1) & 1], sc.state->trace, nullptr, tidx(it, 1), tp.sys};
      icp_half_launch<false>(plan, hb, n_src_c, prm, it, reduce_rows ? 1 : 0, st);
      ++h;
      cur_in = cur;
    }
    prof_loop.reset();
    if (prm->numiters > 0) {
      GsProf prof(GS_PROF_SOLVE, 1.0, st);
      hipLaunchKernelGGL(gs_icp_finish_kernel, dim3(1), dim3(FS_BLOCK), 0, st, sc.partials[(h + 1) & 1], n_src_c,
                         sc.state, h & 1, *prm, compose16, out_T16);
    }
    GS_LAUNCH_CHECK();
    if (tape) return icp_tape_finish(tape, sc.state, n_src, prm->numiters, st);
    return GS_OK;
  }

  GS_HIP(hipMemsetAsync(sc.best, 0xff, 8 * (size_t)n_src, st));
  const int nblk = (int)gs_ceil_div(n_src, LIN_BLOCK);
  double* partials = sc.partials[0];
  const float* cur_in = src;
  for (int it = 0; it < prm->numiters; ++it) {
    float* cur = cloud(it);
    gs_knn_brute_launch(cur_in, sc.state->s[0].T_step, cur, n_src, tgt, n_tgt, sc.best, st);
    {
      GsProf prof(GS_PROF_LINEARIZE, 44.0 * (double)n_src, st);
      hipLaunchKernelGGL((gs_icp_linearize_kernel<true>), dim3(nblk), dim3(LIN_BLOCK), 0, st, cur, nullptr, n_src,
                         tgt, tgt_normals, n_tgt, sc.best, prm->dist_thresh, partials, out_idx, tidx(it, 0));
    }
    {
      GsProf prof(GS_PROF_SOLVE, 1.0, st);
      hipLaunchKernelGGL(gs_icp_solve_kernel, dim3(1), dim3(SUM_BLOCK), 0, st, partials, nblk, sc.state, it, tp.sys);
    }
    gs_knn_brute_launch(cur, sc.state->s[0].Tr, nullptr, n_src, tgt, n_tgt, sc.best, st);
    {
      GsProf prof(GS_PROF_LINEARIZE, 44.0 * (double)n_src, st);
      hipLaunchKernelGGL((gs_icp_linearize_kernel<false>), dim3(nblk), dim3(LIN_BLOCK), 0, st, cur,
                         sc.state->s[0].Tr, n_src, tgt, tgt_normals, n_tgt, sc.best, prm->dist_thresh, partials,
                         nullptr, tidx(it, 1));
    }
    {
      GsProf prof(GS_PROF_SOLVE, 1.0, st);
      hipLaunchKernelGGL(gs_icp_update_kernel, dim3(1), dim3(SUM_BLOCK), 0, st, partials, nblk, sc.state, *prm, it,
                         compose16, out_T16);
    }
    cur_in = cur;
  }
  GS_LAUNCH_CHECK();
  if (tape) return icp_tape_finish(tape, sc.state, n_src, prm->numiters, st);
  return GS_OK;
}

extern "C" int gs_icp_f32(const float* src, int64_t n_src, const float* tgt, const float* tgt_normals,
                          int64_t n_tgt, const float* init16, const float* compose16,
                          const gs_icp_params* prm, float* out_T16, int64_t* out_idx, void* icp_scratch,
                          void* stream) {
  return icp_run(src, n_src, tgt, tgt_normals, n_tgt, init16, compose16, prm, out_T16, out_idx, icp_scratch, nullptr,
                 stream);
}

extern "C" int gs_icp_dc_f32(const float* src, int64_t n_src_bound, const int64_t* n_src_dev, const float* tgt,
                             const float* tgt_normals, int64_t n_tgt_bound, const int64_t* n_tgt_dev,
                             const float* init16, const float* compose16, const gs_icp_params* prm, float* out_T16,
                             int64_t* out_idx, void* icp_scratch, void* stream) {
  return icp_run(src, n_src_bound, tgt, tgt_normals, n_tgt_bound, init16, compose16, prm, out_T16, out_idx,
                 icp_scratch, nullptr, stream, n_src_dev, n_tgt_dev);
}

extern "C" int gs_icp_map_dc_f32(const float* src, int64_t n_src_bound, const int64_t* n_src_dev,
                                 const float* map_points, const float* map_normals, const int32_t* pix,
                                 int64_t n_map_bound, const int64_t* n_map_dev, int W, int ds, const float* init16,
                                 const float* compose16, const gs_icp_params* prm, float* out_T16,
                                 void* icp_scratch, void* stream) {
  GS_REQUIRE(pix && W > 0 && ds > 0, "bad target filter");
  return icp_run(src, n_src_bound, map_points, map_normals, n_map_bound, init16, compose16, prm, out_T16, nullptr,
                 icp_scratch, nullptr, stream, n_src_dev, n_map_dev, GsTargetFilter{pix, W, ds});
}


struct LocSeq {
  const float* vertex;
  const float* depth;
  const float* pose16;
  float* lattice;
  GsIcpState* state;
  float* out_pose16;
  char* clear_ptr;
  int64_t* n_valid;
  int* far_n;
  int* lstat;
  float4* wl_cq;
  unsigned* sync;
};
struct LocBatch {
  int B, W, ds, Wl;
  int64_t n_lat;
  size_t clear_bytes;
  float damp;
  int numiters;
  int count_valid;
  LocSeq s[GS_MAX_BATCH];
};
constexpr int LP_CLEAR_ITEMS = 8;

GS_DEV void loc_prep_block(const LocBatch& lb, const unsigned bid, const unsigned nb_lat) {
  const LocSeq& q = lb.s[bid % lb.B];
  const unsigned blk = bid / lb.B;
  if (blk < nb_lat) {
    const int64_t e = (int64_t)blk * 256 + threadIdx.x;
    int valid = 0;
    if (e < lb.n_lat) {
      const int64_t p = (e / lb.Wl) * lb.ds * (int64_t)lb.W + (e % lb.Wl) * lb.ds;
      float g0 = __builtin_nanf(""), g1 = g0, g2 = g0;
      if (q.depth[p] > 0.0f) {
        float T[12];
#pragma unroll
        for (int i = 0; i < 12; ++i) T[i] = q.pose16[i];
        gs_rigid_fma(T, q.vertex[3 * p], q.vertex[3 * p + 1], q.vertex[3 * p + 2], g0, g1, g2);
        valid = 1;
      }
      q.lattice[3 * e] = g0; q.lattice[3 * e + 1] = g1; q.lattice[3 * e + 2] = g2;
      if (q.wl_cq) q.wl_cq[e] = make_float4(0.0f, 0.0f, 0.0f, 0.0f);
    }
    const unsigned long long m = lb.count_valid ? __ballot(valid) : 0ull;
    if ((threadIdx.x & 63) == 0 && m) atomicAdd(reinterpret_cast<unsigned long long*>(q.n_valid), (unsigned long long)__popcll(m));
    if (blk == 0 && threadIdx.x == 0) {
      IcpSmall sm;
      for (int i = 0; i < 16; ++i) {
        const float id = (i % 5 == 0) ? 1.0f : 0.0f;
        sm.T_total[i] = id; sm.T_step[i] = id; sm.Tr[i] = id;
      }
      for (int i = 0; i < 8; ++i) sm.xi[i] = 0.0f;
      sm.damp = lb.damp;
      sm.err = 0.0f;
      sm.pad[0] = sm.pad[1] = 0.0f;
      q.state->s[0] = sm;
      q.state->s[1] = sm;
      if (q.far_n)
        for (int i = 0; i < FS_FAR_PASSES; ++i) q.far_n[i] = 0;
      if (q.lstat)
        for (int i = 0; i < 3 * GL_STAT_LAUNCHES; ++i) q.lstat[i] = 0;
      if (q.sync)
        for (int i = 0; i < PS_WORDS; ++i) q.sync[i] = 0u;
      if (lb.numiters == 0) icp_write_result(sm, q.pose16, q.out_pose16);
    }
    return;
  }
  float4* dst = reinterpret_cast<float4*>(q.clear_ptr);
  const size_t n16 = lb.clear_bytes / 16;
  const size_t base = (size_t)(blk - nb_lat) * 256 * LP_CLEAR_ITEMS + threadIdx.x;
#pragma unroll
  for (int u = 0; u < LP_CLEAR_ITEMS; ++u) {
    const size_t i = base + (size_t)u * 256;
    if (i < n16) dst[i] = make_float4(0.0f, 0.0f, 0.0f, 0.0f);
  }
}
__global__ void __launch_bounds__(256) gs_loc_prep_kernel(const LocBatch lb, unsigned nb_lat) {
  loc_prep_block(lb, blockIdx.x, nb_lat);
}
static_assert(GB_BLOCK == 256, "lattice and bbox blocks share a launch");
__global__ void __launch_bounds__(256) gs_loc_prep_bbox_kernel(const LocBatch lb, const GsGridBatch gb, const unsigned nb_lat,
                                                               const float u_hi, const float v_hi) {
  const unsigned n_prep = (unsigned)lb.B * nb_lat;
  if (blockIdx.x < n_prep) loc_prep_block(lb, blockIdx.x, nb_lat);
  else gridb_bbox_block(gb, blockIdx.x - n_prep, u_hi, v_hi);
}

struct IcpRowsBatch {
  int B;
  const double* in[GS_MAX_BATCH];
  double* out[GS_MAX_BATCH];
};
__global__ void __launch_bounds__(FS_BLOCK) gs_icp_reduce_rows_batch_kernel(const IcpRowsBatch rb, GsCount n_src_c) {
  __shared__ double S[32];
  __shared__ double sub[FS_BLOCK / 32][32];
  const int nrows = (int)((gs_count(n_src_c) + FS_QPB - 1) / FS_QPB);
  icp_sum_rows<FS_BLOCK>(rb.in[blockIdx.x], nrows, S, sub);
  if (threadIdx.x < LIN_NV) rb.out[blockIdx.x][threadIdx.x] = S[threadIdx.x];
}

struct IcpFinishBatch {
  int B;
  const double* partials_in[GS_MAX_BATCH];
  GsIcpState* st[GS_MAX_BATCH];
  const float* compose16[GS_MAX_BATCH];
  float* out_T16[GS_MAX_BATCH];
  unsigned* sync[GS_MAX_BATCH];
  int nb, h0;
};
__global__ void __launch_bounds__(FS_BLOCK) gs_icp_finish_batch_kernel(const IcpFinishBatch fb, GsCount n_src_c, int buf,
                                                                       gs_icp_params prm) {
  __shared__ double red[FS_BLOCK / GS_WAVE];
  const int b = blockIdx.x;
  const int nrows_in = (int)((gs_count(n_src_c) + FS_QPB - 1) / FS_QPB);
  const double e1 = icp_sum_col27<FS_BLOCK>(fb.partials_in[b], nrows_in, red);
  if (threadIdx.x != 0) return;
  GsIcpState* st = fb.st[b];
  IcpSmall sm = st->s[buf];
  const int it = prm.numiters - 1;
  icp_update_math((float)e1, sm, prm, it < GS_ICP_MAX_ITERS ? st->trace + 12 * it : nullptr);
  st->s[buf ^ 1] = sm;
  icp_write_result(sm, fb.compose16[b], fb.out_T16[b]);
  if (unsigned* sy = fb.sync[b]) {
    const unsigned arrived = sy[PS_ARRIVED], want = (unsigned)fb.nb * (unsigned)(2 * prm.numiters - fb.h0);
    if (!(sy[PS_ERROR] == 0u && arrived == want && sy[PS_TICKET] >= (unsigned)fb.nb))
      for (int i = 0; i < 16; ++i) fb.out_T16[b][i] = __builtin_nanf("");
    sy[PS_NB] = (unsigned)fb.nb;
    sy[PS_H0] = (unsigned)fb.h0;
  }
}

static int64_t loc_lattice(int H, int W, int ds) { return (int64_t)((H + ds - 1) / ds) * ((W + ds - 1) / ds); }

struct ListMem {
  float4* lq;
  uint32_t* ls;
  int* stat;
};
static size_t list_mem_bytes(int64_t n_lat) {
  return gs_align(16 * (size_t)n_lat) + gs_align(4 * GL_SLOTS * (size_t)n_lat) + gs_align(4 * 3 * GL_STAT_LAUNCHES);
}
static ListMem list_carve(void* base, int64_t n_lat) {
  char* p = reinterpret_cast<char*>(base);
  ListMem m;
  m.lq = reinterpret_cast<float4*>(p); p += gs_align(16 * (size_t)n_lat);
  m.ls = reinterpret_cast<uint32_t*>(p); p += gs_align(4 * GL_SLOTS * (size_t)n_lat);
  m.stat = reinterpret_cast<int*>(p);
  return m;
}

struct FarMem {
  uint32_t* c;
  float4* cq;
  int* idx;
  int* n;
};
static size_t far_mem_bytes(int64_t n_lat) {
  return gs_align(4 * GS_FAR_SLOTS * (size_t)n_lat) + gs_align(16 * (size_t)n_lat) +
         gs_align(4 * FS_FAR_PASSES * (size_t)n_lat) + 256;
}
static FarMem far_carve(void* base, int64_t n_lat) {
  char* p = reinterpret_cast<char*>(base);
  FarMem m;
  m.c = reinterpret_cast<uint32_t*>(p); p += gs_align(4 * GS_FAR_SLOTS * (size_t)n_lat);
  m.cq = reinterpret_cast<float4*>(p); p += gs_align(16 * (size_t)n_lat);
  m.idx = reinterpret_cast<int*>(p); p += gs_align(4 * FS_FAR_PASSES * (size_t)n_lat);
  m.n = reinterpret_cast<int*>(p);
  return m;
}

struct FarBuildSeq {
  const float* src;
  const int* idx;
  const int* n;
  const GsGrid* gp;
  const int* cell_start;
  const float4* sorted;
  float* d2prev;
  FarMem m;
};
struct FarBuildBatch {
  int B;
  FarBuildSeq s[GS_MAX_BATCH];
};
constexpr int FAR_BLOCK = 512;
constexpr int FAR_BLOCKS_PER_SEQ = 64;
__global__ void __launch_bounds__(FAR_BLOCK) gs_icp_far_build_kernel(const FarBuildBatch fb) {
  const FarBuildSeq& q = fb.s[blockIdx.x % fb.B];
  const int blk = (int)(blockIdx.x / fb.B);
  const int n = *q.n;
  if (blk >= n) return;
  constexpr int NG = FAR_BLOCK / FS_HG;
  __shared__ float qs[NG][3];
  __shared__ float d1_s[NG];
  __shared__ uint8_t flag_s[NG];
  __shared__ int unres_q[NG], sq_s[NG];
  __shared__ int unres_n;
  __shared__ uint32_t stage_s[NG][GS_FAR_SLOTS + 4];
  const GsGrid g = *q.gp;
  const int grp = threadIdx.x / FS_HG, l16 = threadIdx.x & (FS_HG - 1);
  for (int base = blk; base < n; base += FAR_BLOCKS_PER_SEQ * NG) {
    if (threadIdx.x == 0) unres_n = 0;
    __syncthreads();
    const int e = base + grp * FAR_BLOCKS_PER_SEQ;
    if (e < n) {
      const int sq = q.idx[e];
      const float hx = q.src[3 * (int64_t)sq], hy = q.src[3 * (int64_t)sq + 1], hz = q.src[3 * (int64_t)sq + 2];
      const float4 found = q.m.cq[sq];
      const float d1 = sqrtf(found.x);
      const int kdone = (int)found.y;
      if (kdone >= 0) {
        const float R = far_emit_cube<FS_HG>(g, q.cell_start, q.sorted, hx, hy, hz, l16, d1, kdone, stage_s[grp],
                                             reinterpret_cast<int*>(&stage_s[grp][GS_FAR_SLOTS]));
        for (int u = l16; u < GS_FAR_SLOTS; u += FS_HG) q.m.c[GS_FAR_SLOTS * (int64_t)sq + u] = stage_s[grp][u];
        if (l16 == 0) {
          q.m.cq[sq] = make_float4(hx, hy, hz, R);
          if (R > 0.0f) q.d2prev[sq] = __uint_as_float(__float_as_uint(q.d2prev[sq]) | 0x80000000u);
        }
      } else if (l16 == 0) {
        qs[grp][0] = hx; qs[grp][1] = hy; qs[grp][2] = hz;
        d1_s[grp] = d1;
        sq_s[grp] = sq;
        unres_q[atomicAdd(&unres_n, 1)] = grp;
      }
    }
    __syncthreads();
    const int nun = unres_n;
    for (int u = 0; u < nun; u += FS_BQ) {
      const int nq = nun - u < FS_BQ ? nun - u : FS_BQ;
      block_brute_collect_multi<FAR_BLOCK, FS_BQ>(qs, unres_q + u, nq, q.sorted, q.cell_start[g.ncell], d1_s,
                                                  GS_FAR_RADD * g.c, sq_s, q.m.cq, q.m.c, flag_s);
      if ((int)threadIdx.x < nq) {
        const int gq = unres_q[u + threadIdx.x];
        const int s2 = sq_s[gq];
        if (flag_s[gq]) q.d2prev[s2] = __uint_as_float(__float_as_uint(q.d2prev[s2]) | 0x80000000u);
      }
    }
    __syncthreads();
  }
}

extern "C" int64_t gs_localize_scratch_bytes(int H, int W, int ds, int64_t n_map_bound) {
  if (H < 1 || W < 1 || ds < 1) return 0;
  const int64_t n_lat = loc_lattice(H, W, ds);
  return (int64_t)(gs_align(12 * (size_t)n_lat) + gs_align(4 * (size_t)(n_map_bound > 0 ? n_map_bound : 1)) + 256) +
         gs_icp_scratch_bytes(n_lat, n_map_bound) + (int64_t)list_mem_bytes(n_lat) +
         (int64_t)far_mem_bytes(n_lat);
}

static int64_t loc_rows(const gs_map_view& m) { return m.capacity > m.n_bound ? m.capacity : m.n_bound; }

struct LocCarve {
  float* lattice;
  int32_t* pix;
  int64_t* n_valid;
  IcpScratch sc;
  GridMem gm;
};
static LocCarve loc_carve(const gs_localize_seq& q, int64_t n_lat) {
  LocCarve c;
  char* p = reinterpret_cast<char*>(q.scratch);
  c.lattice = reinterpret_cast<float*>(p); p += gs_align(12 * (size_t)n_lat);
  const int64_t rows = loc_rows(q.map);
  c.pix = reinterpret_cast<int32_t*>(p); p += gs_align(4 * (size_t)rows);
  c.n_valid = reinterpret_cast<int64_t*>(p); p += 256;
  c.sc = icp_carve(p, n_lat);
  c.gm = grid_carve(c.sc.grid, n_lat, rows);
  return c;
}

static bool ps_device_fits() {
  constexpr int MAX_DEV = 64;
  static signed char fits[MAX_DEV] = {};
  int dev = 0;
  if (hipGetDevice(&dev) != hipSuccess || dev < 0 || dev >= MAX_DEV) return false;
  if (fits[dev] == 0) {
    hipDeviceProp_t p;
    const bool ok = hipGetDeviceProperties(&p, dev) == hipSuccess && strncmp(p.gcnArchName, "gfx950", 6) == 0 &&
                    p.multiProcessorCount == (int)(GS_XCDS * PS_CUS_PER_XCD);
    fits[dev] = ok ? 1 : -1;
  }
  return fits[dev] == 1;
}

static int localize_chunk(const gs_localize_seq* seqs, int B, int H, int W, int ds, const gs_icp_params* prm,
                          hipStream_t st, bool grid_cleared) {
  const int64_t n_lat = loc_lattice(H, W, ds);
  const int Wl = (W + ds - 1) / ds;
  LocBatch lb;
  GsGridBatch gb;
  IcpScratch sc[GS_MAX_BATCH];
  GridMem gm[GS_MAX_BATCH];
  lb.B = gb.B = B;
  lb.W = gb.W = W; gb.H = H;
  lb.ds = gb.ds = ds;
  lb.Wl = Wl; lb.n_lat = n_lat; lb.damp = prm->damp; lb.numiters = prm->numiters;
  gb.cells_cap = gs_knn_grid_cells_cap(n_lat);
  for (int b = 0; b < B; ++b) {
    const gs_localize_seq& q = seqs[b];
    const LocCarve cv = loc_carve(q, n_lat);
    float* lattice = cv.lattice;
    int32_t* pix = cv.pix;
    int64_t* n_valid = cv.n_valid;
    sc[b] = cv.sc;
    gm[b] = cv.gm;
    lb.s[b] = LocSeq{q.vertex, q.depth, q.prev_pose16, lattice, sc[b].state, q.out_pose16,
                     reinterpret_cast<char*>(gm[b].g), n_valid, nullptr, nullptr, nullptr,
                     reinterpret_cast<unsigned*>(sc[b].rowred + LIN_NV)};
    static int binned_normals = -1;
    if (binned_normals < 0) {
      const char* e = getenv("GRADSLAM_HIP_ICP_BINNED_NORMALS");
      binned_normals = (e && atoi(e) == 0) ? 0 : 1;
    }
    if (!binned_normals) gm[b].sorted_n = nullptr;
    gb.s[b] = GsGridSeq{q.map.points, GsCount{q.map.n_bound, q.map.n_dev}, pix, q.prev_pose16, q.K16,
                        binned_normals ? q.map.normals : nullptr, gm[b]};
    if (g_gs_prof_on) GS_HIP(hipMemsetAsync(n_valid, 0, 8, st));
  }
  static int far_lists = -1;
  if (far_lists < 0) {
    const char* e = getenv("GRADSLAM_HIP_ICP_FAR");
    far_lists = (e && atoi(e) != 0) ? 1 : 0;
  }
  const bool far_on = far_lists == 1 && prm->numiters > 0;
  FarMem fm[GS_MAX_BATCH];
  for (int b = 0; b < B; ++b) {
    fm[b] = far_carve(reinterpret_cast<char*>(sc[b].state) + gs_icp_scratch_bytes(n_lat, loc_rows(seqs[b].map)) +
                          list_mem_bytes(n_lat), n_lat);
    lb.s[b].far_n = fm[b].n;
    if (!far_on) fm[b] = FarMem{nullptr, nullptr, nullptr, nullptr};
  }
  static int ord_lists = -1, lists_from = FS_LISTS_FROM;
  if (ord_lists < 0) {
    const char* e = getenv("GRADSLAM_HIP_ICP_LISTS");
    ord_lists = (e && atoi(e) == 0) ? 0 : 1;
    const char* f = getenv("GRADSLAM_HIP_ICP_LISTS_FROM");
    if (f && atoi(f) >= 0) lists_from = atoi(f);
  }
  ListMem lm[GS_MAX_BATCH];
  for (int b = 0; b < B; ++b) {
    lm[b] = list_carve(reinterpret_cast<char*>(sc[b].state) + gs_icp_scratch_bytes(n_lat, loc_rows(seqs[b].map)), n_lat);
    lb.s[b].lstat = lm[b].stat;
  }
  static int wide_lists = -1;
  if (wide_lists < 0) {
    const char* e = getenv("GRADSLAM_HIP_ICP_WIDE");
    wide_lists = (e && atoi(e) == 0) ? 0 : 1;
  }
  const bool wide_on = wide_lists == 1 && !far_on && prm->numiters > 0;
  FarMem wm[GS_MAX_BATCH];
  for (int b = 0; b < B; ++b) {
    wm[b] = far_carve(reinterpret_cast<char*>(sc[b].state) + gs_icp_scratch_bytes(n_lat, loc_rows(seqs[b].map)) +
                          list_mem_bytes(n_lat), n_lat);
    lb.s[b].wl_cq = wide_on ? wm[b].cq : nullptr;
  }
  lb.count_valid = g_gs_prof_on ? 1 : 0;
  lb.clear_bytes = gs_knn_grid_clear_bytes(gm[0], gb.cells_cap);
  const unsigned nb_lat = (unsigned)gs_ceil_div(n_lat, 256);
  const unsigned nb_clear = (unsigned)gs_ceil_div((int64_t)(lb.clear_bytes / 16), 256 * LP_CLEAR_ITEMS);
  {
    double bytes = 0.0;
    for (int b = 0; b < B; ++b) bytes += 28.0 * n_lat + 24.0 * seqs[b].map.n_bound + 16.0 * gb.cells_cap;
    GsProf prof(GS_PROF_COMPACT, bytes, st, grid_cleared ? 4 : 5);
    int rc;
    if (grid_cleared) {
      const float u_hi = (float)((double)W - 0.999), v_hi = (float)((double)H - 0.999);
      hipLaunchKernelGGL(gs_loc_prep_bbox_kernel, dim3((unsigned)B * nb_lat + gs_knn_gridb_bbox_blocks(gb)), dim3(256), 0, st,
                         lb, gb, nb_lat, u_hi, v_hi);
      rc = gs_knn_grid_build_batch(gb, st, true);
    } else {
      hipLaunchKernelGGL(gs_loc_prep_kernel, dim3((unsigned)B * (nb_lat + nb_clear)), dim3(256), 0, st, lb, nb_lat);
      rc = gs_knn_grid_build_batch(gb, st);
    }
    if (rc != GS_OK) return rc;
  }
  if (prm->numiters == 0) { GS_LAUNCH_CHECK(); return GS_OK; }

  const int nfs = (int)icp_rows(n_lat);
  const bool reduce_rows = nfs > FS_REDUCE_ROWS;
  const GsCount n_src_c{n_lat, nullptr};
  double prof_bytes = 0.0;
  if (g_gs_prof_on) {
    for (int b = 0; b < B; ++b) {
      unsigned hits = 0;
      int64_t nv = 0;
      GS_HIP(hipMemcpyAsync(&hits, gm[b].bbox + 6, 4, hipMemcpyDeviceToHost, st));
      GS_HIP(hipMemcpyAsync(&nv, lb.s[b].n_valid, 8, hipMemcpyDeviceToHost, st));
      GS_HIP(hipStreamSynchronize(st));
      prof_bytes += icp_alg_bytes(prm->numiters, n_lat, nv, hits);
    }
  }
  std::unique_ptr<GsProf> prof_loop(new GsProf(GS_PROF_ICP_FUSED, prof_bytes, st, 2 * prm->numiters));
  static int persist_env = -1;
  if (persist_env < 0) {
    const char* e = getenv("GRADSLAM_HIP_ICP_PERSIST");
    persist_env = (e && atoi(e) == 1) ? 1 : 0;
  }
  const int ps_upb = (int)gs_ceil_div((int64_t)icp_rows(n_lat), PS_CUS_PER_XCD);
  const int ps_nb = (int)gs_ceil_div((int64_t)icp_rows(n_lat), ps_upb > 0 ? ps_upb : 1);
  bool persist_on = persist_env == 1 && ord_lists == 1 && !far_on && B <= (int)GS_XCDS && ps_upb <= PS_UPB &&
                    prm->numiters > lists_from + 1 && !getenv("GRADSLAM_HIP_ICP_TIMELINE") &&
                    !getenv("GRADSLAM_HIP_ICP_LANES") && ps_device_fits();
  for (int b = 0; b < B && persist_on; ++b) persist_on = gm[b].sorted_n != nullptr;
  const IcpHalfPlan plan = icp_half_plan(n_lat, B, far_on ? 4 : (persist_on ? 2 : 8));
  bool lists_on = ord_lists == 1 && !far_on && plan.upb * plan.G * FS_QPB <= FS_BLOCK;
  if (plan.G != 2) persist_on = false;
  for (int b = 0; b < B && lists_on; ++b) {
    const char* end = reinterpret_cast<const char*>(seqs[b].scratch) + gs_localize_scratch_bytes(H, W, ds, loc_rows(seqs[b].map));
    const char* first = reinterpret_cast<const char*>(reduce_rows ? sc[b].rowred : sc[b].partials[1]);
    if (reinterpret_cast<const char*>(sc[b].partials[0]) > first) first = reinterpret_cast<const char*>(sc[b].partials[0]);
    if (reinterpret_cast<const char*>(sc[b].partials[1]) > first) first = reinterpret_cast<const char*>(sc[b].partials[1]);
    if (end - first < (ptrdiff_t)(sizeof(double) * LIN_NV * FS_BLOCK)) lists_on = false;
  }
  IcpHalfBatch hb;
  hb.B = B;
  static float weak_room = -1.0f;
  if (weak_room < 0.0f) {
    const char* e = getenv("GRADSLAM_HIP_ICP_WEAK_ROOM");
    weak_room = e ? (float)atof(e) : 0.0f;
    if (!(weak_room >= 0.0f && weak_room < 1.0f)) weak_room = 0.0f;
  }
  hb.weak_room = weak_room;
  int h = 0;
  if (!lists_on) persist_on = false;
  int ps_it0 = prm->numiters, ps_h0 = 0;
  if (persist_on) {
    ps_it0 = lists_from + 1;
    if (ps_it0 >= prm->numiters) { persist_on = false; ps_it0 = prm->numiters; }
  }
  for (int it = 0; it < ps_it0; ++it) {
    for (int b = 0; b < B; ++b) {
      const gs_localize_seq& q = seqs[b];
      const float* cur_in = it == 0 ? lb.s[b].lattice : (((it - 1) & 1) ? sc[b].srcB : sc[b].srcA);
      float* cur = (it & 1) ? sc[b].srcB : sc[b].srcA;
      hb.s[b] = IcpHalfSeq{cur_in, cur, q.map.points, q.map.normals, GsCount{q.map.n_bound, q.map.n_dev}, gm[b].g,
                           gm[b].cell_start, gm[b].sorted, gm[b].sorted_n, reinterpret_cast<float*>(sc[b].best),
                           sc[b].partials[(h + 1) & 1], sc[b].partials[h & 1],
                           &sc[b].state->s[h & 1], &sc[b].state->s[(h + 1) & 1], sc[b].state->trace, nullptr, nullptr,
                           nullptr, fm[b].cq, fm[b].c, fm[b].idx, fm[b].n};
      hb.w[b] = wide_on ? IcpHalfWide{wm[b].cq, wm[b].c} : IcpHalfWide{nullptr, nullptr};
      hb.l[b] = lists_on ? IcpHalfLists{lm[b].lq, lm[b].ls, lm[b].stat, lb.s[b].sync + PS_WEAK}
                         : IcpHalfLists{nullptr, nullptr, nullptr, nullptr};
    }
    icp_half_launch<true>(plan, hb, n_src_c, prm, it, 0, st, lists_on && it > lists_from ? 2 : 0);
    if (far_on && fs_far_pass(it) >= 0) {
      const int fp = fs_far_pass(it);
      FarBuildBatch fbb;
      fbb.B = B;
      for (int b = 0; b < B; ++b)
        fbb.s[b] = FarBuildSeq{(it & 1) ? sc[b].srcB : sc[b].srcA, fm[b].idx + (int64_t)fp * n_lat, fm[b].n + fp, gm[b].g,
                               gm[b].cell_start, gm[b].sorted, reinterpret_cast<float*>(sc[b].best), fm[b]};
      hipLaunchKernelGGL(gs_icp_far_build_kernel, dim3((unsigned)B * FAR_BLOCKS_PER_SEQ), dim3(FAR_BLOCK), 0, st, fbb);
    }
    ++h;
    if (reduce_rows) {
      IcpRowsBatch rb;
      rb.B = B;
      for (int b = 0; b < B; ++b) { rb.in[b] = sc[b].partials[(h + 1) & 1]; rb.out[b] = sc[b].rowred; }
      hipLaunchKernelGGL(gs_icp_reduce_rows_batch_kernel, dim3((unsigned)B), dim3(FS_BLOCK), 0, st, rb, n_src_c);
    }
    for (int b = 0; b < B; ++b) {
      IcpHalfSeq& u = hb.s[b];
      u.src_in = (it & 1) ? sc[b].srcB : sc[b].srcA;
      u.src_out = nullptr;
      u.partials_in = reduce_rows ? sc[b].rowred : sc[b].partials[(h + 1) & 1];
      u.partials_out = sc[b].partials[h & 1];
      u.st_in = &sc[b].state->s[h & 1];
      u.st_out = &sc[b].state->s[(h + 1) & 1];
    }
    icp_half_launch<false>(plan, hb, n_src_c, prm, it, reduce_rows ? 1 : 0, st,
                           lists_on ? (it == lists_from ? (persist_on ? 3 : 1) : (it > lists_from ? 2 : 0)) : 0);
    ++h;
  }
  if (persist_on) {
    IcpPersistBatch pb;
    pb.B = B;
    pb.nb = ps_nb;
    pb.upb = ps_upb;
    pb.h0 = ps_h0 = h;
    pb.tl_h = 0;
    pb.timeline = nullptr;
    for (int b = 0; b < B; ++b) {
      const gs_localize_seq& q = seqs[b];
      pb.s[b] = IcpPersistSeq{((ps_it0 - 1) & 1) ? sc[b].srcB : sc[b].srcA, GsCount{q.map.n_bound, q.map.n_dev}, gm[b].g, gm[b].cell_start,
                              gm[b].sorted, gm[b].sorted_n, {sc[b].partials[0], sc[b].partials[1]}, sc[b].state, lm[b].lq, lm[b].ls,
                              lm[b].stat, wide_on ? wm[b].cq : nullptr, wide_on ? wm[b].c : nullptr, lb.s[b].sync};
    }
#ifdef GS_ICP_TIMELINE
    static const char* ptl_path = getenv("GRADSLAM_HIP_ICP_PERSIST_TIMELINE");
    static unsigned long long* ptl_buf = nullptr;
    constexpr size_t PTL_WORDS = 72 * (size_t)GS_XCDS * PS_CUS_PER_XCD;
    if (ptl_path) {
      if (!ptl_buf && hipMalloc(&ptl_buf, 8 * PTL_WORDS) != hipSuccess) ptl_buf = nullptr;
      if (ptl_buf) {
        (void)hipMemsetAsync(ptl_buf, 0, 8 * PTL_WORDS, st);
        pb.timeline = ptl_buf;
        static const char* tl_it_env = getenv("GRADSLAM_HIP_ICP_TIMELINE_IT");
        pb.tl_h = 2 * (tl_it_env ? atoi(tl_it_env) : prm->numiters - 1);
      }
    }
#endif
    hipLaunchKernelGGL(gs_icp_persist_kernel, dim3(GS_XCDS * PS_CUS_PER_XCD), dim3(PS_BLOCK), 0, st, pb, n_lat, prm->dist_thresh,
                       *prm);
#ifdef GS_ICP_TIMELINE
    if (pb.timeline) {
      std::unique_ptr<unsigned long long[]> hbuf(new unsigned long long[PTL_WORDS]);
      if (hipStreamSynchronize(st) == hipSuccess && hipMemcpy(hbuf.get(), ptl_buf, 8 * PTL_WORDS, hipMemcpyDeviceToHost) == hipSuccess) {
        FILE* f = fopen(ptl_path, "w");
        if (f) {
          fprintf(f, "# B=%d nb=%d upb=%d h0=%d tl_h=%d: per block: xcc lb end | first half: wait_done sums scalar check rare arrived at_barrier research hard brute - - | look-ahead: the same | start releases... (100 MHz ticks)\n",
                  B, pb.nb, pb.upb, pb.h0, pb.tl_h);
          for (size_t i = 0; i < PTL_WORDS / 72; ++i) {
            const unsigned long long* r = hbuf.get() + 72 * i;
            if (!r[0]) continue;
            fprintf(f, "%llu %llu %llu |", r[1], r[2], r[3]);
            for (int k = 8; k < 32; ++k) fprintf(f, " %llu%s", r[k], k == 19 ? " |" : "");
            fprintf(f, " | %llu", r[4]);
            for (int k = 32; k < 72; ++k) fprintf(f, " %llu", r[k]);
            fprintf(f, "\n");
          }
          fclose(f);
        }
      }
    }
#endif
    h = 2 * prm->numiters;
  }
  prof_loop.reset();
  {
    GsProf prof(GS_PROF_SOLVE, 1.0, st);
    IcpFinishBatch fb;
    fb.B = B;
    fb.nb = persist_on ? ps_nb : 0;
    fb.h0 = persist_on ? ps_h0 : 0;
    for (int b = 0; b < B; ++b) {
      fb.partials_in[b] = sc[b].partials[(h + 1) & 1];
      fb.st[b] = sc[b].state;
      fb.compose16[b] = seqs[b].prev_pose16;
      fb.out_T16[b] = seqs[b].out_pose16;
      fb.sync[b] = persist_on ? lb.s[b].sync : nullptr;
    }
    hipLaunchKernelGGL(gs_icp_finish_batch_kernel, dim3((unsigned)B), dim3(FS_BLOCK), 0, st, fb, n_src_c, h & 1, *prm);
  }
  GS_LAUNCH_CHECK();
  return GS_OK;
}

static int localize_batch(const gs_localize_seq* seqs_host, int B, int H, int W, int ds, const gs_icp_params* prm,
                          void* stream, bool grid_cleared) {
  GS_REQUIRE(seqs_host && prm && B > 0 && H > 0 && W > 0 && ds > 0, "bad arguments");
  GS_REQUIRE(prm->numiters >= 0 && prm->numiters <= GS_ICP_MAX_ITERS, "numiters must be in [0, 1024]");
  GS_REQUIRE(prm->mode == 0 || prm->mode == 1, "mode must be 0 (ICP) or 1 (gradICP)");
  GS_REQUIRE((int64_t)H * W < (1ll << 31), "image too large for int32 pixel ids");
  for (int b = 0; b < B; ++b) {
    const gs_localize_seq& q = seqs_host[b];
    GS_REQUIRE(q.vertex && q.depth && q.K16 && q.prev_pose16 && q.out_pose16 && q.scratch, "NULL pointer");
    GS_REQUIRE(q.map.points && q.map.normals && q.map.n_bound > 0 && q.map.n_bound < 0x7fffffffll,
               "every sequence needs a non-empty map (points + normals)");
    GS_REQUIRE(q.map.capacity <= 0 || q.map.n_bound <= q.map.capacity, "map.n_bound exceeds map.capacity");
  }
  hipStream_t st = gs_stream(stream);
  for (int c0 = 0; c0 < B; c0 += GS_MAX_BATCH) {
    const int nb = B - c0 < GS_MAX_BATCH ? B - c0 : GS_MAX_BATCH;
    const int rc = localize_chunk(seqs_host + c0, nb, H, W, ds, prm, st, grid_cleared);
    if (rc != GS_OK) return rc;
  }
  return GS_OK;
}
extern "C" int gs_localize_batch_f32(const gs_localize_seq* seqs_host, int B, int H, int W, int ds,
                                     const gs_icp_params* prm, void* stream) {
  return localize_batch(seqs_host, B, H, W, ds, prm, stream, false);
}

__global__ void __launch_bounds__(256) gs_far_stats_kernel(const int* __restrict__ far_idx, const int* __restrict__ far_n,
                                                          const float* __restrict__ d2prev, const float4* __restrict__ far_cq,
                                                          int64_t n_lat, int* __restrict__ out4) {
  const int n0 = far_n[0], n = n0 < 0 ? 0 : (n0 > (int)n_lat ? (int)n_lat : n0);
  if (blockIdx.x == 0 && threadIdx.x == 0) { out4[0] = n; out4[2] = far_n[1]; }
  int c = 0, built = 0;
  for (int i = blockIdx.x * 256 + threadIdx.x; i < n; i += gridDim.x * 256) {
    const int s = far_idx[i];
    if (s < 0 || s >= (int)n_lat) continue;
    c += (__float_as_uint(d2prev[s]) >> 31) ? 1 : 0;
    built += far_cq[s].w > 0.0f ? 1 : 0;
  }
  if (c) atomicAdd(&out4[1], c);
  if (built) atomicAdd(&out4[3], built);
}
extern "C" int gs_localize_far_stats_i64(const void* scratch, int H, int W, int ds, int64_t map_rows, int64_t* out4_host,
                                         void* stream) {
  GS_REQUIRE(scratch && out4_host && H > 0 && W > 0 && ds > 0 && map_rows > 0, "bad arguments");
  const int64_t n_lat = loc_lattice(H, W, ds);
  gs_localize_seq q;
  memset(&q, 0, sizeof(q));
  q.scratch = const_cast<void*>(scratch);
  q.map.capacity = map_rows; q.map.n_bound = map_rows;
  const LocCarve cv = loc_carve(q, n_lat);
  const FarMem fm = far_carve(reinterpret_cast<char*>(cv.sc.state) + gs_icp_scratch_bytes(n_lat, map_rows) +
                                  list_mem_bytes(n_lat), n_lat);
  hipStream_t st = gs_stream(stream);
  int* out4 = fm.n + 8;
  GS_HIP(hipMemsetAsync(out4, 0, 16, st));
  hipLaunchKernelGGL(gs_far_stats_kernel, dim3(64), dim3(256), 0, st, fm.idx, fm.n, reinterpret_cast<const float*>(cv.sc.best),
                     fm.cq, n_lat, out4);
  int h[4] = {0, 0, 0, 0};
  GsGrid g;
  GS_HIP(hipMemcpyAsync(h, out4, 16, hipMemcpyDeviceToHost, st));
  GS_HIP(hipMemcpyAsync(&g, cv.gm.g, sizeof(g), hipMemcpyDeviceToHost, st));
  GS_HIP(hipStreamSynchronize(st));
  for (int i = 0; i < 4; ++i) out4_host[i] = h[i];
  if (getenv("GRADSLAM_HIP_DEBUG_GRID"))
    fprintf(stderr, "grid: box (%.3f %.3f %.3f)-(%.3f %.3f %.3f) c %.4f cells %d x %d x %d = %d\n", g.ox, g.oy, g.oz, g.mx,
            g.my, g.mz, g.c, g.nx, g.ny, g.nz, g.ncell);
  return GS_OK;
}

extern "C" int gs_localize_list_stats_i64(const void* scratch, int H, int W, int ds, int64_t map_rows, int64_t* out192_host,
                                          void* stream) {
  GS_REQUIRE(scratch && out192_host && H > 0 && W > 0 && ds > 0 && map_rows > 0, "bad arguments");
  const int64_t n_lat = loc_lattice(H, W, ds);
  gs_localize_seq q;
  memset(&q, 0, sizeof(q));
  q.scratch = const_cast<void*>(scratch);
  q.map.capacity = map_rows; q.map.n_bound = map_rows;
  const LocCarve cv = loc_carve(q, n_lat);
  const ListMem lm = list_carve(reinterpret_cast<char*>(cv.sc.state) + gs_icp_scratch_bytes(n_lat, map_rows), n_lat);
  int h[3 * GL_STAT_LAUNCHES];
  hipStream_t st = gs_stream(stream);
  GS_HIP(hipMemcpyAsync(h, lm.stat, sizeof(h), hipMemcpyDeviceToHost, st));
  GS_HIP(hipStreamSynchronize(st));
  for (int i = 0; i < 3 * GL_STAT_LAUNCHES; ++i) out192_host[i] = h[i];
  return GS_OK;
}

extern "C" int gs_localize_solve_stats_i64(const void* scratch, int H, int W, int ds, int64_t map_rows, int64_t* out8_host,
                                           void* stream) {
  GS_REQUIRE(scratch && out8_host && H > 0 && W > 0 && ds > 0 && map_rows > 0, "bad arguments");
  const int64_t n_lat = loc_lattice(H, W, ds);
  gs_localize_seq q;
  memset(&q, 0, sizeof(q));
  q.scratch = const_cast<void*>(scratch);
  q.map.capacity = map_rows; q.map.n_bound = map_rows;
  const LocCarve cv = loc_carve(q, n_lat);
  unsigned h[PS_WORDS];
  hipStream_t st = gs_stream(stream);
  GS_HIP(hipMemcpyAsync(h, cv.sc.rowred + LIN_NV, sizeof(h), hipMemcpyDeviceToHost, st));
  GS_HIP(hipStreamSynchronize(st));
  static_assert(PS_WORDS == 8, "out8");
  for (int i = 0; i < PS_WORDS; ++i) out8_host[i] = h[i];
  return GS_OK;
}

extern "C" int gs_pointfusion_step_batch_f32(const gs_step_seq* seqs_host, int B, int H, int W, int ds,
                                             const gs_icp_params* prm, float two_sigma_sq, float dist_th, float dot_th,
                                             int renorm_all, void* stream) {
  GS_REQUIRE(seqs_host && prm && B > 0 && H > 0 && W > 0 && ds > 0, "bad arguments");
  const int64_t P = (int64_t)H * W;
  const gs_step_seq& s0 = seqs_host[0];
  const int64_t dstride = B > 1 ? seqs_host[1].depth - s0.depth : P;
  for (int b = 0; b < B; ++b) {
    const gs_step_seq& q = seqs_host[b];
    GS_REQUIRE(q.depth && q.rgb && q.K16 && q.prev_pose16 && q.out_pose16 && q.vertex && q.normal && q.alpha &&
                   q.best_pix && q.new_count_out && q.loc_scratch && q.upd_scratch, "NULL pointer");
    GS_REQUIRE((q.gvertex != nullptr) == (q.gnormal != nullptr) && (q.gvertex != nullptr) == (s0.gvertex != nullptr),
               "gvertex / gnormal: both or none, the same choice for every sequence");
    GS_REQUIRE(q.out_pose16 != q.prev_pose16, "out_pose16 must not alias prev_pose16");
    GS_REQUIRE(q.vertex == s0.vertex + 3 * P * b && q.normal == s0.normal + 3 * P * b && q.alpha == s0.alpha + P * b,
               "vertex / normal / alpha of the batch must be dense");
    GS_REQUIRE(q.depth == s0.depth + dstride * b && q.K16 == s0.K16 + 16 * (int64_t)b, "depth / K16 must be equally strided");
  }
  GS_REQUIRE(dstride >= P || B == 1, "overlapping depth images");
  const bool implicit_global = s0.gvertex == nullptr;
  std::unique_ptr<gs_update_seq[]> us(new gs_update_seq[B]);
  for (int c0 = 0; c0 < B; c0 += GS_MAX_BATCH) {
    const int nb = B - c0 < GS_MAX_BATCH ? B - c0 : GS_MAX_BATCH;
    const gs_step_seq* sq = seqs_host + c0;
    gs_localize_seq ls[GS_MAX_BATCH];
    for (int b = 0; b < nb; ++b) {
      const gs_step_seq& q = sq[b];
      ls[b].vertex = q.vertex; ls[b].depth = q.depth; ls[b].K16 = q.K16; ls[b].prev_pose16 = q.prev_pose16;
      ls[b].map = q.map; ls[b].out_pose16 = q.out_pose16; ls[b].scratch = q.loc_scratch;
      gs_update_seq& u = us[c0 + b];
      u.map = q.map; u.vertex = q.vertex; u.normal = q.normal; u.depth = q.depth; u.rgb = q.rgb;
      u.alpha = q.alpha; u.pose16 = q.out_pose16; u.K16 = q.K16; u.gvertex = q.gvertex;
      u.gnormal = q.gnormal; u.best_pix = q.best_pix; u.new_count_out = q.new_count_out;
      u.scratch = q.upd_scratch;
    }
    const int64_t n_lat = loc_lattice(H, W, ds);
    GsClearJob job;
    job.n = nb;
    for (int b = 0; b < nb; ++b) {
      GS_REQUIRE(ls[b].map.points && ls[b].map.n_bound > 0, "every sequence needs a non-empty map");
      const LocCarve cv = loc_carve(ls[b], n_lat);
      job.ptr[b] = reinterpret_cast<char*>(cv.gm.g);
      if (b == 0) job.bytes = gs_knn_grid_clear_bytes(cv.gm, gs_knn_grid_cells_cap(n_lat));
    }
    GsPixelTables tabs{};
    tabs.n = implicit_global ? nb : 0;
    tabs.call_flag = c0 == 0 ? gs_update_map_call_flag(seqs_host[0].upd_scratch) : nullptr;
    for (int b = 0; b < tabs.n; ++b) {
      gs_update_map_tables(sq[b].upd_scratch, &tabs.any_flag[b], &tabs.key_pix[b]);
      tabs.best_pix[b] = sq[b].best_pix;
    }
    int rc = gs_frame_maps_batch_clear(sq[0].depth, dstride, P, sq[0].K16, nb, 1, H, W, two_sigma_sq, sq[0].vertex,
                                       sq[0].normal, sq[0].alpha, &job, stream, &tabs);
    if (rc != GS_OK) return rc;
    rc = localize_batch(ls, nb, H, W, ds, prm, stream, true);
    if (rc != GS_OK) return rc;
  }
  return gs_update_map_fusion_batch_impl(us.get(), B, H, W, dist_th, dot_th, renorm_all, stream, implicit_global);
}

extern "C" int64_t gs_icp_tape_bytes(int64_t n_src, int numiters) { return (int64_t)gs_icp_tape_size(n_src, numiters); }

extern "C" int gs_icp_tape_f32(const float* src, int64_t n_src, const float* tgt, const float* tgt_normals,
                               int64_t n_tgt, const float* init16, const float* compose16,
                               const gs_icp_params* prm, float* out_T16, int64_t* out_idx, void* icp_scratch,
                               void* tape, void* stream) {
  GS_REQUIRE(tape, "tape must not be NULL");
  return icp_run(src, n_src, tgt, tgt_normals, n_tgt, init16, compose16, prm, out_T16, out_idx, icp_scratch, tape,
                 stream);
}

extern "C" int gs_icp_trace_f32(const void* icp_scratch, int numiters, float* trace_out, void* stream) {
  GS_REQUIRE(icp_scratch && trace_out && numiters >= 0 && numiters <= GS_ICP_MAX_ITERS, "bad arguments");
  const GsIcpState* st = reinterpret_cast<const GsIcpState*>(icp_scratch);
  GS_HIP(hipMemcpyAsync(trace_out, st->trace, sizeof(float) * 12 * (size_t)numiters, hipMemcpyDeviceToDevice,
                        gs_stream(stream)));
  return GS_OK;
}
```

gradslam_amd/csrc/gs_knn.h:

```cpp
#pragma once
#include "gs_common.h"

GS_DEV unsigned long long knn_pack(float d, uint32_t idx) {
  return ((unsigned long long)__float_as_uint(d) << 32) | (unsigned long long)idx;
}

int gs_knn_brute_launch(const float* src_in, const float* Tapply, float* src_out, int64_t n_src,
                        const float* tgt, int64_t n_tgt, unsigned long long* best, hipStream_t st);

constexpr int GS_GRID_MAXCELL = 1 << 22;
constexpr int GS_GRID_RINGS = 3;
constexpr int GS_GRID_TILE = 1024;

struct GsGrid {
  float ox, oy, oz;
  float mx, my, mz;
  float c, inv_c;
  int nx, ny, nz, ncell;
};

struct GsTargetFilter {
  const int32_t* pix;
  int W, ds;
};
GS_DEV bool gs_is_target(const GsTargetFilter& f, int64_t n) {
  if (!f.pix) return true;
  const int32_t p = f.pix[n];
  return p >= 0 && ((p / f.W) % f.ds == 0) && ((p % f.W) % f.ds == 0);
}

struct GridMem {
  GsGrid* g;
  unsigned* bbox;
  int* unres_count;
  int* cell_count;
  int* cell_start;
  int* tile_sums;
  float4* sorted;
  float4* sorted_n;
  float4* tlist;
  int* unres_list;
};

static inline GridMem grid_carve(void* scratch, int64_t n_src, int64_t n_tgt) {
  char* p = reinterpret_cast<char*>(scratch);
  GridMem m;
  m.g = reinterpret_cast<GsGrid*>(p); p += 128;
  m.bbox = reinterpret_cast<unsigned*>(p); p += 128;
  m.unres_count = reinterpret_cast<int*>(p); p += 256;
  m.tile_sums = reinterpret_cast<int*>(p); p += gs_align(4 * (size_t)(GS_GRID_MAXCELL / GS_GRID_TILE + 2));
  m.cell_count = reinterpret_cast<int*>(p); p += gs_align(4 * (size_t)(GS_GRID_MAXCELL + 1));
  m.cell_start = reinterpret_cast<int*>(p); p += gs_align(4 * (size_t)(GS_GRID_MAXCELL + 1));
  m.sorted = reinterpret_cast<float4*>(p); p += gs_align(16 * (size_t)(n_tgt > 0 ? n_tgt : 1));
  m.sorted_n = reinterpret_cast<float4*>(p); p += gs_align(16 * (size_t)(n_tgt > 0 ? n_tgt : 1));
  m.tlist = reinterpret_cast<float4*>(p); p += gs_align(16 * (size_t)(n_tgt > 0 ? n_tgt : 1));
  m.unres_list = reinterpret_cast<int*>(p);
  (void)n_src;
  return m;
}

size_t gs_knn_grid_scratch_bytes(int64_t n_src, int64_t n_tgt);

struct GsGridSeq {
  const float* tgt;
  GsCount n_tgt;
  int32_t* pix;
  const float* pose16;
  const float* K16;
  const float* nrm;
  GridMem m;
};
struct GsGridBatch {
  int B, H, W, ds;
  int cells_cap;
  GsGridSeq s[GS_MAX_BATCH];
};
int gs_knn_grid_cells_cap(int64_t n_src);
size_t gs_knn_grid_clear_bytes(const GridMem& m, int cells_cap);
int gs_knn_grid_build_batch(const GsGridBatch& gb, hipStream_t st, bool bbox_done = false);

int gs_knn_grid_build(const float* tgt, GsCount n_tgt, int64_t n_src, void* grid_scratch, hipStream_t st,
                      GsTargetFilter filter = GsTargetFilter{nullptr, 1, 1}, const float* nrm = nullptr);
int gs_knn_grid_query(const float* src_in, const float* Tapply, float* src_out, int64_t n_src,
                      const float* tgt, int64_t n_tgt, unsigned long long* best, void* grid_scratch,
                      hipStream_t st);
static inline bool gs_knn_use_grid(int64_t n_src, int64_t n_tgt) { return n_tgt >= 2048 && n_src >= 256; }

GS_DEV int grid_axis(float v, float o, float inv_c, int n) {
  const float f = (v - o) * inv_c;
  return f >= 0.0f ? (f < (float)n ? (int)f : n - 1) : 0;
}
GS_DEV int grid_cell(const GsGrid& g, float x, float y, float z) {
  const int ix = grid_axis(x, g.ox, g.inv_c, g.nx);
  const int iy = grid_axis(y, g.oy, g.inv_c, g.ny);
  const int iz = grid_axis(z, g.oz, g.inv_c, g.nz);
  return (iz * g.ny + iy) * g.nx + ix;
}

constexpr int GQ_G = 8;
constexpr int GL_RING_NF = 2;

GS_DEV unsigned long long grid_key(float qx, float qy, float qz, const float4 p) {
  const float dx = qx - p.x, dy = qy - p.y, dz = qz - p.z;
  float d = dx * dx;
  d = gs_fma(dy, dy, d);
  d = gs_fma(dz, dz, d);
  return d == d ? knn_pack(d, (uint32_t)__float_as_int(p.w)) : ~0ull;
}

template <int G>
GS_DEV unsigned long long grid_group_min(unsigned long long key) {
#pragma unroll
  for (int d = G / 2; d > 0; d >>= 1) {
    const unsigned long long o = __shfl_xor(key, d, G);
    key = o < key ? o : key;
  }
  return key;
}

struct GsQueryCell {
  float px, py, pz;
  int cx, cy, cz;
};
GS_DEV GsQueryCell grid_query_cell(const GsGrid& g, float qx, float qy, float qz) {
  GsQueryCell c;
  c.px = qx < g.ox ? g.ox : (qx > g.mx ? g.mx : qx);
  c.py = qy < g.oy ? g.oy : (qy > g.my ? g.my : qy);
  c.pz = qz < g.oz ? g.oz : (qz > g.mz ? g.mz : qz);
  c.cx = grid_axis(c.px, g.ox, g.inv_c, g.nx); c.cy = grid_axis(c.py, g.oy, g.inv_c, g.ny);
  c.cz = grid_axis(c.pz, g.oz, g.inv_c, g.nz);
  return c;
}

template <int G>
GS_DEV unsigned long long grid_search_stage0(const GsGrid& g, const int* __restrict__ cell_start,
                                             const float4* __restrict__ sorted, float qx, float qy, float qz, int lane,
                                             bool* resolved, int* win, const float rball = __builtin_inff()) {
  const GsQueryCell qc = grid_query_cell(g, qx, qy, qz);
  const float px = qc.px, py = qc.py, pz = qc.pz;
  const int cx = qc.cx, cy = qc.cy, cz = qc.cz;
  unsigned long long key = ~0ull;
  int bt = -1;
  const float fx = (px - g.ox) * g.inv_c - (float)cx, fy = (py - g.oy) * g.inv_c - (float)cy,
              fz = (pz - g.oz) * g.inv_c - (float)cz;
  const int x0 = (fx < 0.5f) ? cx - 1 : cx, y0 = (fy < 0.5f) ? cy - 1 : cy, z0 = (fz < 0.5f) ? cz - 1 : cz;
  const float BIG = 3.0e38f;
  const float ax = fminf(x0 >= 1 ? fx + (float)(cx - x0) : BIG, x0 + 2 < g.nx ? (float)(x0 + 2 - cx) - fx : BIG);
  const float ay = fminf(y0 >= 1 ? fy + (float)(cy - y0) : BIG, y0 + 2 < g.ny ? (float)(y0 + 2 - cy) - fy : BIG);
  const float az = fminf(z0 >= 1 ? fz + (float)(cz - z0) : BIG, z0 + 2 < g.nz ? (float)(z0 + 2 - cz) - fz : BIG);
  const float amin = fminf(ax, fminf(ay, az));
  const float rc = rball * g.inv_c * 1.0001f + 0.002f;
  const bool prune = rc < amin - 0.001f;
  bool ulx = true, uhx = true, uly = true, uhy = true, ulz = true, uhz = true;
  if (prune) {
    const float tx = fx + (float)(cx - x0), ty = fy + (float)(cy - y0), tz = fz + (float)(cz - z0);
    ulx = tx - rc < 1.0f; uhx = tx + rc >= 1.0f;
    uly = ty - rc < 1.0f; uhy = ty + rc >= 1.0f;
    ulz = tz - rc < 1.0f; uhz = tz + rc >= 1.0f;
  }
  int sb0 = 0, sb1 = 0, sb2 = 0, sb3 = 0, e1 = 0, e2 = 0, e3 = 0, total = 0;
  {
    const int xa = (x0 >= 0 && ulx) ? x0 : x0 + 1, xb = (x0 + 1 < g.nx && uhx) ? x0 + 1 : x0;
    const bool zl = z0 >= 0 && ulz, zh = z0 + 1 < g.nz && uhz, yl = y0 >= 0 && uly, yh = y0 + 1 < g.ny && uhy;
    const int r0 = (z0 * g.ny + y0) * g.nx, r1 = r0 + g.nx, r2 = r0 + g.ny * g.nx, r3 = r2 + g.nx;
    int se0 = 0, se1 = 0, se2 = 0, se3 = 0;
    if (zl && yl) { sb0 = cell_start[r0 + xa]; se0 = cell_start[r0 + xb + 1]; }
    if (zl && yh) { sb1 = cell_start[r1 + xa]; se1 = cell_start[r1 + xb + 1]; }
    if (zh && yl) { sb2 = cell_start[r2 + xa]; se2 = cell_start[r2 + xb + 1]; }
    if (zh && yh) { sb3 = cell_start[r3 + xa]; se3 = cell_start[r3 + xb + 1]; }
    e1 = se0 - sb0;
    e2 = e1 + (se1 - sb1);
    e3 = e2 + (se2 - sb2);
    total = e3 + (se3 - sb3);
  }
  for (int t0 = lane; t0 < total; t0 += 4 * G) {
    float4 p[4];
    bool in[4];
#pragma unroll
    for (int u = 0; u < 4; ++u) {
      const int t = t0 + u * G;
      in[u] = t < total;
      const int tt = in[u] ? t : 0;
      const int ix = tt < e1 ? sb0 + tt : (tt < e2 ? sb1 + (tt - e1) : (tt < e3 ? sb2 + (tt - e2) : sb3 + (tt - e3)));
      p[u] = sorted[ix];
    }
#pragma unroll
    for (int u = 0; u < 4; ++u) {
      const unsigned long long k2 = in[u] ? grid_key(qx, qy, qz, p[u]) : ~0ull;
      const bool better = k2 < key;
      key = better ? k2 : key;
      bt = better ? t0 + u * G : bt;
    }
  }
  {
    const unsigned long long kmin = grid_group_min<G>(key);
    const int bs = bt < e1 ? sb0 + bt : (bt < e2 ? sb1 + (bt - e1) : (bt < e3 ? sb2 + (bt - e2) : sb3 + (bt - e3)));
    *win = (key == kmin && bt >= 0) ? bs : -1;
    key = kmin;
  }
  const float rb = (amin < 1.0e30f) ? (amin - 0.001f) * g.c : BIG;
  const float bd = __uint_as_float((uint32_t)(key >> 32));
  *resolved = prune ? (bd == bd) : (rb > 0.0f && (rb >= 1.0e30f ? bd == bd : bd <= rb * rb));
  return key;
}

template <int G>
GS_DEV unsigned long long grid_search_rings(const GsGrid& g, const int* __restrict__ cell_start,
                                            const float4* __restrict__ sorted, float qx, float qy, float qz, int lane,
                                            unsigned long long key, bool* resolved, int* win,
                                            const int kmax = GS_GRID_RINGS, int* kdone = nullptr) {
  const GsQueryCell qc = grid_query_cell(g, qx, qy, qz);
  bool done = false;
  int bs = -1;
  int k = 1;
  for (; k <= kmax && !done; ++k) {
    const int side = 2 * k + 1, nrow = side * side;
    const int xa = qc.cx - k < 0 ? 0 : qc.cx - k, xb = qc.cx + k >= g.nx ? g.nx - 1 : qc.cx + k;
    for (int r = lane; r < nrow; r += G) {
      const int zz = qc.cz + r / side - k, yy = qc.cy + r % side - k;
      if (zz < 0 || zz >= g.nz || yy < 0 || yy >= g.ny) continue;
      const int row = (zz * g.ny + yy) * g.nx;
      const int je = cell_start[row + xb + 1];
      for (int j = cell_start[row + xa]; j < je; j += GL_RING_NF) {
// ... 562 lines not shown
```

gradslam_amd/csrc/gs_knn_bbox.h:

```cpp
#pragma once
#include "gs_assoc_dev.h"
#include "gs_knn.h"

GS_DEV unsigned grid_code(float v) {
  const unsigned b = __float_as_uint(v);
  return (b & 0x80000000u) ? ~b : (b | 0x80000000u);
}
GS_DEV float grid_decode(unsigned c) {
  return __uint_as_float((c & 0x80000000u) ? (c & 0x7fffffffu) : ~c);
}
constexpr int GB_BLOCK = 256;
constexpr int GB_ITEMS = 8;
GS_DEV void grid_bbox_body(const float* __restrict__ tgt, const int64_t n_tgt, const GsTargetFilter flt,
                           const GsCamera* cam, int H, float u_hi, float v_hi, int32_t* __restrict__ pix_out,
                           unsigned* __restrict__ bbox, int* __restrict__ unres_count, float4* __restrict__ tlist,
                           const unsigned blk) {
  if (blk == 0 && threadIdx.x == 0) { unres_count[0] = 0; unres_count[1] = 0; }
  if ((int64_t)blk * GB_BLOCK * GB_ITEMS >= n_tgt) return;
  __shared__ float red[6][GB_BLOCK / GS_WAVE];
  __shared__ int scan_s[GB_BLOCK / GS_WAVE + 1];
  __shared__ unsigned base_s;
  int hits = 0;
  unsigned hitmask = 0;
  float lo[3] = {3.0e38f, 3.0e38f, 3.0e38f}, hi[3] = {-3.0e38f, -3.0e38f, -3.0e38f};
  const int64_t i0 = (int64_t)blk * GB_ITEMS * GB_BLOCK + threadIdx.x;
  if (cam) {
    float v[GB_ITEMS][3];
#pragma unroll
    for (int u = 0; u < GB_ITEMS; ++u) {
      const int64_t i = i0 + (int64_t)u * GB_BLOCK, ic = i < n_tgt ? i : n_tgt - 1;
      v[u][0] = tgt[3 * ic]; v[u][1] = tgt[3 * ic + 1]; v[u][2] = tgt[3 * ic + 2];
    }
#pragma unroll
    for (int u = 0; u < GB_ITEMS; ++u) {
      const int64_t i = i0 + (int64_t)u * GB_BLOCK;
      if (i < n_tgt) {
        int ph = 0, pw = 0;
        const bool in = gs_project_point_hw(*cam, v[u][0], v[u][1], v[u][2], H, flt.W, u_hi, v_hi, ph, pw);
        pix_out[i] = in ? (int32_t)(ph * flt.W + pw) : -1;
        if (in && gs_on_lattice(ph, pw, flt.ds)) {
          ++hits;
          hitmask |= 1u << u;
#pragma unroll
          for (int k = 0; k < 3; ++k) {
            const float w = v[u][k];
            if (w > -3.0e38f && w < 3.0e38f) {
              lo[k] = w < lo[k] ? w : lo[k];
              hi[k] = w > hi[k] ? w : hi[k];
            }
          }
        }
      }
    }
  } else {
    bool t[GB_ITEMS];
    if (flt.pix) {
      int32_t px[GB_ITEMS];
#pragma unroll
      for (int u = 0; u < GB_ITEMS; ++u) {
        const int64_t i = i0 + (int64_t)u * GB_BLOCK;
        px[u] = flt.pix[i < n_tgt ? i : n_tgt - 1];
      }
#pragma unroll
      for (int u = 0; u < GB_ITEMS; ++u) {
        const int32_t p = px[u];
        t[u] = (i0 + (int64_t)u * GB_BLOCK < n_tgt) && p >= 0 && ((p / flt.W) % flt.ds == 0) && ((p % flt.W) % flt.ds == 0);
      }
    } else {
#pragma unroll
      for (int u = 0; u < GB_ITEMS; ++u) t[u] = i0 + (int64_t)u * GB_BLOCK < n_tgt;
    }
#pragma unroll
    for (int u = 0; u < GB_ITEMS; ++u) {
      if (t[u]) {
        const int64_t i = i0 + (int64_t)u * GB_BLOCK;
        ++hits;
        hitmask |= 1u << u;
#pragma unroll
        for (int k = 0; k < 3; ++k) {
          const float w = tgt[3 * i + k];
          if (w > -3.0e38f && w < 3.0e38f) {
            lo[k] = w < lo[k] ? w : lo[k];
            hi[k] = w > hi[k] ? w : hi[k];
          }
        }
      }
    }
  }
  const int lane = threadIdx.x & 63, wave = threadIdx.x >> 6;
#pragma unroll
  for (int k = 0; k < 3; ++k) {
    float a = lo[k], b = hi[k];
#pragma unroll
    for (int d = 32; d > 0; d >>= 1) {
      const float a2 = __shfl_down(a, d, GS_WAVE), b2 = __shfl_down(b, d, GS_WAVE);
      a = a2 < a ? a2 : a;
      b = b2 > b ? b2 : b;
    }
    if (lane == 0) { red[k][wave] = a; red[3 + k][wave] = b; }
  }
  const bool filtered = flt.pix != nullptr || cam != nullptr;
  __syncthreads();
  if (filtered) {
    int total;
    int pos = gs_block_excl_scan<GB_BLOCK>(hits, scan_s, &total);
    if (threadIdx.x == 0 && total) base_s = atomicAdd(&bbox[6], (unsigned)total);
    __syncthreads();
    if (hitmask) {
      const unsigned base = base_s;
#pragma unroll
      for (int u = 0; u < GB_ITEMS; ++u) {
        if (hitmask & (1u << u)) {
          const int64_t i = ((int64_t)blk * GB_ITEMS + u) * GB_BLOCK + threadIdx.x;
          tlist[base + (unsigned)pos] = make_float4(tgt[3 * i], tgt[3 * i + 1], tgt[3 * i + 2], __int_as_float((int)i));
          ++pos;
        }
      }
    }
  }
  if (threadIdx.x < 3) {
    const int k = threadIdx.x;
    float a = red[k][0], b = red[3 + k][0];
    for (int w = 1; w < GB_BLOCK / GS_WAVE; ++w) {
      a = red[k][w] < a ? red[k][w] : a;
      b = red[3 + k][w] > b ? red[3 + k][w] : b;
    }
    if (a <= b) {
      atomicMax(&bbox[k], ~grid_code(a));
      atomicMax(&bbox[3 + k], grid_code(b));
    }
  }
}

GS_DEV void gridb_bbox_block(const GsGridBatch& gb, const unsigned bid, float u_hi, float v_hi) {
  const GsGridSeq& q = gb.s[bid % gb.B];
  const unsigned blk = bid / gb.B;
  const GsTargetFilter flt{q.pix, gb.W, gb.ds};
  if (q.pose16) {
    const GsCamera cam = gs_camera(q.pose16, q.K16);
    grid_bbox_body(q.tgt, gs_count(q.n_tgt), flt, &cam, gb.H, u_hi, v_hi, q.pix, q.m.bbox, q.m.unres_count, q.m.tlist,
                   blk);
  } else {
    grid_bbox_body(q.tgt, gs_count(q.n_tgt), flt, nullptr, 0, 0.0f, 0.0f, nullptr, q.m.bbox, q.m.unres_count, q.m.tlist,
                   blk);
  }
}
static inline unsigned gs_knn_gridb_bbox_blocks(const GsGridBatch& gb) {
  int64_t n_max = 1;
  for (int b = 0; b < gb.B; ++b) n_max = gb.s[b].n_tgt.host > n_max ? gb.s[b].n_tgt.host : n_max;
  return (unsigned)gb.B * (unsigned)gs_ceil_div(n_max, GB_BLOCK * GB_ITEMS);
}
```

gradslam_amd/slam/_fastpath.py:

```python
import os

import torch

from .. import _C, ops
from ..structures.pointclouds import _ATTRS
from .fusionutils import RENORMALIZE_UNMATCHED

__all__ = ["try_step"]

f32 = torch.float32
FASTPATH = os.environ.get("GRADSLAM_HIP_FASTPATH", "1") != "0"
STEP_GLOBAL_MAPS = os.environ.get("GRADSLAM_HIP_STEP_GLOBAL_MAPS", "0") == "1"


def _kwargs_key(kw):
    def norm(v):
        if torch.is_tensor(v):
            return ("tensor", id(v), int(v._version), tuple(v.shape), str(v.dtype), str(v.device))
        return v
    return tuple(sorted((k, norm(v)) for k, v in kw.items()))


def _dense_frames(t, inner):
    if t.dtype != f32 or t.stride()[2:] != inner:
        return None
    B = t.shape[0]
    sb = t.stride(0) if B > 1 else inner[0] * t.shape[2]
    if B > 1 and sb < inner[0] * t.shape[2]:
        return None
    return t.data_ptr(), sb


class StepPlan(object):
    def __init__(self, slam, B, H, W, device):
        self.B, self.H, self.W, self.P, self.device = B, H, W, H * W, device
        self.lib = _C.lib()
        self.seqs = (_C.StepSeq * B)()
        prov = slam.odomprov
        kw = prov._kwargs()
        self.kw_tensors = [v for v in kw.values() if torch.is_tensor(v)]
        self.prm = _C.IcpParams(int(prov._mode), int(kw.get("numiters", 20)), float(kw.get("damp", 1e-8)),
                                ops._thresh(kw.get("dist_thresh")), float(kw.get("lambda_max", 2.0)),
                                float(kw.get("B", 1.0)), float(kw.get("B2", 1.0)), float(kw.get("nu", 200.0)))
        self.key = (float(slam.sigma), float(slam.dist_th), float(slam.dot_th), int(slam.dsratio), _kwargs_key(kw),
                    int(prov._mode))
        self.sigma = float(slam.sigma)
        self.tss = ops.two_sigma_sq(slam.sigma)
        self.dist_th, self.dot_th, self.ds = float(slam.dist_th), float(slam.dot_th), int(slam.dsratio)
        self.caps = [-1] * B
        self.bufs = [None] * B
        self.scratch = [None] * B
        self.stream = _C.stream(device)
        self.stream_id = torch.cuda.current_stream(device).cuda_stream

    def _bind_map(self, pc, b):
        bufs = tuple(pc._buf[k][b] for k in _ATTRS)
        cap = int(bufs[0].shape[0])
        if any(t.shape[0] != cap for t in bufs):
            return False
        q = self.seqs[b]
        m = q.map
        m.points, m.normals, m.colors, m.ccounts = (t.data_ptr() for t in bufs)
        m.capacity = cap
        if cap != self.caps[b]:
            ws = _C.Workspace.get(self.device)
            loc = ws.bytes("localize%d" % b, self.lib.gs_localize_scratch_bytes(self.H, self.W, self.ds, cap))
            upd = ws.bytes("map_update%d" % b, self.lib.gs_update_map_scratch_bytes(cap, self.H, self.W))
            self.scratch[b] = (loc, upd)
            q.loc_scratch, q.upd_scratch = loc.data_ptr(), upd.data_ptr()
            self.caps[b] = cap
        self.bufs[b] = bufs
        return True

    def run(self, pc, live, prev):
        B, P, H, W = self.B, self.P, self.H, self.W
        dev = self.device
        d = _dense_frames(live._depth_image, (W, 1, 1))
        r = _dense_frames(live._rgb_image, (3 * W, 3, 1))
        K, pp = live._intrinsics, prev._poses
        if d is None or r is None or K.dtype != f32 or pp.dtype != f32 or not K.is_contiguous() or not pp.is_contiguous():
            return None
        grp = pc._dcount[0].group
        grp.poll()
        bounds = grp.bounds
        for b in range(B):
            bufs = self.bufs[b]
            if (bufs is None or any(bufs[i] is not pc._buf[k][b] for i, k in enumerate(_ATTRS)) or
                    bounds[b] + P > self.caps[b]):
                if bounds[b] + P > int(pc._buf["points"][b].shape[0]):
                    pc._reserve(b, P, pc.RESERVE_FRAMES)
                    bounds = grp.bounds
                if not self._bind_map(pc, b):
                    return None
        gm = STEP_GLOBAL_MAPS
        out = torch.empty(B * (13 if gm else 7) * P, dtype=f32, device=dev)
        poses_out = torch.empty(B * 16, dtype=f32, device=dev)
        best = torch.empty((B, P), dtype=torch.int32, device=dev)
        o = out.data_ptr()
        v0, n0, a0, po0 = o, o + 12 * P * B, o + 24 * P * B, poses_out.data_ptr()
        gv0, gn0 = o + 28 * P * B, o + 28 * P * B + 12 * P * B
        pair = getattr(grp, "_step_counts", None)
        if pair is None or pair[0].shape[0] != B or pair[0].device != dev:
            pair = grp._step_counts = [torch.zeros(B, dtype=torch.int64, device=dev) for _ in range(2)]
        cnt_new = pair[0] if pair[0].data_ptr() != grp.dev.data_ptr() else pair[1]
        d0, ds_ = d
        r0, rs_ = r
        k0, p0, c0, n_dev0, b0 = K.data_ptr(), pp.data_ptr(), cnt_new.data_ptr(), grp.dev.data_ptr(), best.data_ptr()
        seqs = self.seqs
        for b in range(B):
            q = seqs[b]
            q.depth, q.rgb = d0 + 4 * ds_ * b, r0 + 4 * rs_ * b
            q.K16, q.prev_pose16, q.out_pose16 = k0 + 64 * b, p0 + 64 * b, po0 + 64 * b
            q.vertex, q.normal, q.alpha = v0 + 12 * P * b, n0 + 12 * P * b, a0 + 4 * P * b
            q.gvertex, q.gnormal = (gv0 + 12 * P * b, gn0 + 12 * P * b) if gm else (None, None)
            q.best_pix = b0 + 4 * P * b
            q.new_count_out = c0 + 8 * b
            q.map.n_bound = bounds[b]
            q.map.n_dev = n_dev0 + 8 * b
        _C.check(self.lib.gs_pointfusion_step_batch_f32(seqs, B, H, W, self.ds, self.prm, self.tss, self.dist_th,
                                                        self.dot_th, 1 if RENORMALIZE_UNMATCHED else 0, self.stream), "gs_pointfusion_step_batch_f32")
        n3 = 3 * P * B
        live._vertex_map = out[:n3].view(B, 1, H, W, 3)
        live._normal_map = out[n3:2 * n3].view(B, 1, H, W, 3)
        live._alpha_cache = (self.sigma, out[2 * n3:2 * n3 + P * B].view(B, 1, H, W, 1))
        live._poses = poses_out.view(B, 1, 4, 4)
        if gm:
            g = 7 * P * B
            live._global_vertex_map = out[g:g + n3].view(B, 1, H, W, 3)
            live._global_normal_map = out[g + n3:g + 2 * n3].view(B, 1, H, W, 3)
        else:
            live._global_vertex_map = live._global_normal_map = None
        grp.advance(cnt_new, P)
        pc._padded_cache.clear()
        pc.equisized = True if B == 1 else None
        return pc, live._poses


def try_step(slam, pointclouds, live_frame, prev_frame):
    if not ops.DEVICE_COUNTS or not FASTPATH or prev_frame is None or slam.odom not in ("icp", "gradicp"):
        return None
    B = len(pointclouds._n_host)
    dc = pointclouds._dcount
    if B == 0 or len(dc) != B:
        return None
    g0 = dc[0].group
    if len(g0.bounds) != B or any(dc[b].group is not g0 or dc[b].index != b for b in range(B)) or min(g0.bounds) <= 0:
        return None
    if live_frame._channels_first or prev_frame._channels_first or live_frame._L != 1 or live_frame._B != B:
        return None
    if prev_frame._poses is None or live_frame._intrinsics.data_ptr() != prev_frame._intrinsics.data_ptr():
        return None
    if tuple(prev_frame._poses.shape) != (B, 1, 4, 4):
        return None
    dev = live_frame.device
    if dev.type != "cuda" or pointclouds.device != dev or prev_frame.device != dev:
        return None
    bufs = pointclouds._buf
    if any(bufs[k] is None for k in _ATTRS) or bufs["points"][0].dtype != f32 or bufs["features"][0].shape[-1] != 1:
        return None
    if torch.is_grad_enabled() and (live_frame._depth_image.requires_grad or live_frame._rgb_image.requires_grad or
                                    prev_frame._poses.requires_grad or
                                    any(t.requires_grad for k in _ATTRS for t in bufs[k])):
        return None
    from ..odometry.gradicp import GradICPOdometryProvider
    from ..odometry.icp import ICPOdometryProvider
    if type(slam.odomprov) not in (ICPOdometryProvider, GradICPOdometryProvider):
        return None
    H, W = live_frame.h, live_frame.w
    plan = getattr(slam, "_step_plan", None)
    key = (float(slam.sigma), float(slam.dist_th), float(slam.dot_th), int(slam.dsratio),
           _kwargs_key(slam.odomprov._kwargs()), int(slam.odomprov._mode))
    if (plan is None or (plan.B, plan.H, plan.W, plan.device) != (B, H, W, dev) or plan.key != key or
            plan.stream_id != torch.cuda.current_stream(dev).cuda_stream):
        plan = slam._step_plan = StepPlan(slam, B, H, W, dev)
    return plan.run(pointclouds, live_frame, prev_frame)
```

include/gradslam_hip.h:

```cpp
#ifndef GRADSLAM_HIP_H
#define GRADSLAM_HIP_H

#include <stdint.h>

#ifdef __cplusplus
extern "C" {
#endif

#define GS_API __attribute__((visibility("default")))

#define GS_OK 0
#define GS_ERR_INVALID 1
#define GS_ERR_HIP 2
#define GS_ERR_CAPACITY 3

GS_API int gs_abi_version(void);
GS_API const char* gs_last_error(void);
GS_API int64_t gs_scratch_bytes(int64_t n_map, int64_t n_pix);

GS_API int gs_profile_begin(int max_records);
GS_API int gs_profile_end(void);
GS_API int gs_profile_read(int kind, double* ms_total, int64_t* launches, double* work_total);

GS_API int gs_frame_maps_f32(const float* depth, const float* K16, int H, int W, float two_sigma_sq,
// ... 112 lines not shown

GS_API int gs_icp_trace_f32(const void* icp_scratch, int numiters, float* trace_out, void* stream);

GS_API int gs_similar_rows_f32(const int64_t* rows, int64_t n_rows, const float* points,
                        const float* normals, const float* gvertex, const float* gnormal, int W,
                        float dist_th, float dot_th, uint8_t* mask, void* stream);

GS_API int gs_best_unique_rows_f32(const int64_t* rows, int64_t n_rows, const float* points,
                            const float* ccounts, const float* gvertex, int H, int W, int64_t b,
                            int32_t* best_pix, int64_t* rows_out, int64_t* count_out,
                            void* scratch, void* stream);

GS_API int gs_associate_f32(const int32_t* pix, int64_t n_map, const float* points,
                     const float* normals, const float* ccounts, const float* gvertex,
                     const float* gnormal, int H, int W, float dist_th, float dot_th,
                     int32_t* best_pix, uint8_t* similar, void* scratch, void* stream);

GS_API int gs_best_table_i64(const int32_t* best_pix, int H, int W, int64_t b, int64_t* rows_out,
                      int64_t* count_out, void* scratch, void* stream);
GS_API int gs_rows_to_best_pix(const int64_t* rows, int64_t n_rows, int H, int W, int32_t* best_pix,
                        void* stream);

GS_API int gs_fuse_append_f32(float* points, float* normals, float* colors, float* ccounts,
                       int64_t n_map_host, int64_t capacity, const int32_t* best_pix,
                       const float* gvertex, const float* gnormal, const float* rgb,
                       const float* alpha, const float* depth, int H, int W, int renorm_all,
                       int64_t* new_count_out, void* scratch, void* stream);

GS_API int gs_append_valid_f32(float* points, float* normals, float* colors, float* ccounts,
                        int64_t n_map_host, int64_t capacity, const float* gvertex,
                        const float* gnormal, const float* rgb, const float* alpha,
                        const float* depth, int H, int W, int64_t* new_count_out, void* scratch,
                        void* stream);

GS_API int gs_lattice_source_f32(const float* vertex, const float* depth, const float* pose16, int H, int W, int ds,
                                 float* out_pts, void* stream);

GS_API int gs_ingest_depth_u16_f32(const uint16_t* raw, int H0, int W0, float* out, int H, int W,
                                   double scale_div, void* stream);
GS_API int gs_ingest_color_u8_f32(const uint8_t* raw, int H0, int W0, float* out, int H, int W, int normalize,
                                  void* stream);
GS_API int gs_ingest_frames_native_f32(const uint16_t* depth_raw, const uint8_t* color_raw, int64_t n_frames, int H, int W,
                                       double scale_div, int normalize, float* depth_out, float* color_out, void* stream);
GS_API int gs_host_device_pointer(const void* host_ptr, void** dev_ptr_out);

GS_API int gs_project_map_dc_f32(const float* points, int64_t n_map_bound, const int64_t* n_map_dev,
                                 const float* pose16, const float* K16, int H, int W, int32_t* pix,
                                 void* stream);
GS_API int gs_select_targets_dc_f32(const int32_t* pix, int64_t n_map_bound, const int64_t* n_map_dev, int W,
                                    int ds, const float* points, const float* normals, const float* colors,
                                    float* out_pts, float* out_nrm, float* out_rgb, int64_t cap,
                                    int64_t* count_out, void* scratch, void* stream);
GS_API int gs_associate_dc_f32(const int32_t* pix, int64_t n_map_bound, const int64_t* n_map_dev,
                               const float* points, const float* normals, const float* ccounts,
                               const float* gvertex, const float* gnormal, int H, int W, float dist_th,
                               float dot_th, int32_t* best_pix, uint8_t* similar, void* scratch, void* stream);
GS_API int gs_fuse_append_dc_f32(float* points, float* normals, float* colors, float* ccounts,
                                 int64_t n_map_bound, const int64_t* n_map_dev, int64_t capacity,
                                 const int32_t* best_pix, const float* gvertex, const float* gnormal,
                                 const float* rgb, const float* alpha, const float* depth, int H, int W,
                                 int renorm_all, int64_t* new_count_out, void* scratch, void* stream);
GS_API int gs_append_valid_dc_f32(float* points, float* normals, float* colors, float* ccounts,
                                  int64_t n_map_bound, const int64_t* n_map_dev, int64_t capacity,
                                  const float* gvertex, const float* gnormal, const float* rgb,
                                  const float* alpha, const float* depth, int H, int W,
                                  int64_t* new_count_out, void* scratch, void* stream);

GS_API int gs_fuse_append_backward_f32(const float* points, const float* normals, const float* colors,
                                       const float* ccounts, int64_t n_old, const int32_t* best_pix,
                                       const float* gvertex, const float* gnormal, const float* rgb,
                                       const float* alpha, const float* depth, int H, int W, int renorm_all,
                                       const float* P_bar, const float* N_bar, const float* C_bar,
                                       const float* F_bar, int64_t n_new, float* old_points_bar,
                                       float* old_normals_bar, float* old_colors_bar, float* old_ccounts_bar,
                                       float* gvertex_bar, float* gnormal_bar, float* rgb_bar, float* alpha_bar,
                                       void* scratch, void* stream);

GS_API int64_t gs_update_map_scratch_bytes(int64_t n_map_bound, int H, int W);
GS_API int gs_update_map_fusion_dc_f32(float* points, float* normals, float* colors, float* ccounts,
                                       int64_t n_map_bound, const int64_t* n_map_dev, int64_t capacity,
                                       const float* vertex, const float* normal, const float* depth,
                                       const float* rgb, const float* alpha, const float* pose16, const float* K16,
                                       int H, int W, float dist_th, float dot_th, int renorm_all, float* gvertex,
                                       float* gnormal, int32_t* best_pix, int64_t* new_count_out, void* scratch,
                                       void* stream);

typedef struct gs_map_view {
  float* points;
  float* normals;
  float* colors;
  float* ccounts;
  int64_t capacity;
  int64_t n_bound;
  const int64_t* n_dev;
} gs_map_view;

GS_API int gs_frame_maps_batch_f32(const float* depth, int64_t depth_stride_seq, int64_t depth_stride_frame,
                                   const float* K16, int n_frames, int frames_per_K, int H, int W, float two_sigma_sq,
                                   float* vertex, float* normal, float* alpha, void* stream);

typedef struct gs_localize_seq {
  const float* vertex;
  const float* depth;
  const float* K16;
  const float* prev_pose16;
  gs_map_view map;
  float* out_pose16;
  void* scratch;
} gs_localize_seq;
GS_API int64_t gs_localize_scratch_bytes(int H, int W, int ds, int64_t n_map_bound);
GS_API int gs_localize_batch_f32(const gs_localize_seq* seqs_host, int B, int H, int W, int ds,
                                 const gs_icp_params* params_host, void* stream);
GS_API int gs_localize_far_stats_i64(const void* scratch, int H, int W, int ds, int64_t map_rows, int64_t* out4_host,
                                     void* stream);
GS_API int gs_localize_list_stats_i64(const void* scratch, int H, int W, int ds, int64_t map_rows, int64_t* out192_host,
                                      void* stream);
GS_API int gs_localize_solve_stats_i64(const void* scratch, int H, int W, int ds, int64_t map_rows, int64_t* out8_host,
                                       void* stream);

typedef struct gs_update_seq {
  gs_map_view map;
  const float* vertex;
  const float* normal;
  const float* depth;
  const float* rgb;
  const float* alpha;
  const float* pose16;
  const float* K16;
  float* gvertex;
  float* gnormal;
  int32_t* best_pix;
  int64_t* new_count_out;
  void* scratch;
} gs_update_seq;
GS_API int gs_update_map_fusion_batch_f32(const gs_update_seq* seqs_host, int B, int H, int W, float dist_th,
                                          float dot_th, int renorm_all, void* stream);

typedef struct gs_step_seq {
  const float* depth;
  const float* rgb;
  const float* K16;
  const float* prev_pose16;
  float* out_pose16;
  float* vertex;
  float* normal;
  float* alpha;
  float* gvertex;
  float* gnormal;
  int32_t* best_pix;
  int64_t* new_count_out;
  gs_map_view map;
  void* loc_scratch;
  void* upd_scratch;
} gs_step_seq;
GS_API int gs_pointfusion_step_batch_f32(const gs_step_seq* seqs_host, int B, int H, int W, int ds,
                                         const gs_icp_params* params_host, float two_sigma_sq, float dist_th,
                                         float dot_th, int renorm_all, void* stream);

GS_API int gs_project_points_f32(const float* cam_coords, int cdim, int64_t n, const float* proj16, int64_t pts_per_mat,
                                 float* out_uv, void* stream);
GS_API int gs_unproject_points_f32(const float* pixel_coords, int pdim, int64_t n, const float* kinv9,
                                   int64_t pts_per_mat, const float* depths, float* out_xyz, void* stream);
GS_API int gs_lie_small_f32(int op, const float* in, float* out, void* stream);

typedef struct gs_render_seq {
  gs_map_view map;
  const float* poses16;
  const float* K16;
  float* depth;
  float* color;
  float* normal;
  float* confidence;
  int64_t* index;
  void* scratch;
} gs_render_seq;
GS_API int64_t gs_render_scratch_bytes(int views, int H, int W);
GS_API int gs_render_map_dc_f32(const gs_render_seq* seqs_host, int B, int L, int H, int W, int radius,
                                float min_confidence, int cull_backfaces, void* stream);

#ifdef __cplusplus
}
#endif
#endif
```

Baseline: 3809.

## Hand over localization target list from map-update kernels to next frame's ICP

The map merge and append kernels now project each written map point with the output pose and emit the target pixel table, bounding box and target list straight into the localization scratch, along with a validation record (pose, count, pointer, sizes). On the next step the grid-bbox pass checks that record and skips re-projecting the whole map when it matches, and the scratch clear keeps the bbox region. Python tracks buffer identity and version to force a rebuild when the map was changed outside the step. This removes a full map projection pass per frame, at the cost of extra work and atomics in the update kernels and a more fragile state dependency across calls.

```diff
diff --git a/gradslam_amd/_C.py b/gradslam_amd/_C.py
--- a/gradslam_amd/_C.py
+++ b/gradslam_amd/_C.py
@@ -8,7 +8,7 @@
 if os.environ.get("GRADSLAM_HIP_LIB"):
     import warnings
     warnings.warn("GRADSLAM_HIP_LIB overrides the product library: %s" % LIB_PATH, RuntimeWarning)
-ABI_VERSION = 3
+ABI_VERSION = 4
 
 _lib = None
 
@@ -43,7 +43,7 @@
                 ("out_pose16", C.c_void_p), ("vertex", C.c_void_p), ("normal", C.c_void_p), ("alpha", C.c_void_p),
                 ("gvertex", C.c_void_p), ("gnormal", C.c_void_p), ("best_pix", C.c_void_p),
                 ("new_count_out", C.c_void_p), ("map", MapView), ("loc_scratch", C.c_void_p),
-                ("upd_scratch", C.c_void_p)]
+                ("upd_scratch", C.c_void_p), ("force_rebuild", C.c_int32)]
 
 
 class RenderSeq(C.Structure):
@@ -128,6 +128,8 @@
     "gs_lie_small_f32": [_i32, _vp, _vp, _vp],
     "gs_localize_far_stats_i64": [_vp, _i32, _i32, _i32, _i64, C.POINTER(C.c_int64), _vp],
     "gs_localize_list_stats_i64": [_vp, _i32, _i32, _i32, _i64, C.POINTER(C.c_int64), _vp],
+    "gs_localize_handover_stats_i64": [_vp, _i32, _i32, _i32, _i64, C.POINTER(C.c_int64), _vp],
+    "gs_localize_handover_offset": [_i32, _i32, _i32, _i64],
     "gs_localize_solve_stats_i64": [_vp, _i32, _i32, _i32, _i64, C.POINTER(C.c_int64), _vp],
     "gs_pointfusion_step_batch_f32": [C.POINTER(StepSeq), _i32, _i32, _i32, _i32, C.POINTER(IcpParams), _f, _f, _f, _i32, _vp],
     "gs_render_scratch_bytes": [_i32, _i32, _i32],
@@ -136,7 +138,7 @@
 _RESTYPE = {"gs_last_error": C.c_char_p, "gs_scratch_bytes": _i64, "gs_icp_scratch_bytes": _i64,
             "gs_knn1_grid_scratch_bytes": _i64, "gs_update_map_scratch_bytes": _i64, "gs_global_maps_pose_backward_scratch_bytes": _i64, "gs_icp_tape_bytes": _i64, "gs_icp_backward_scratch_bytes": _i64,
             "gs_localize_scratch_bytes": _i64, "gs_frame_maps_backward_kbar_scratch_bytes": _i64,
-            "gs_render_scratch_bytes": _i64}
+            "gs_render_scratch_bytes": _i64, "gs_localize_handover_offset": _i64}
 EXPORTS = tuple(_PROTOS)
 
 
diff --git a/gradslam_amd/csrc/gs_common.h b/gradslam_amd/csrc/gs_common.h
--- a/gradslam_amd/csrc/gs_common.h
+++ b/gradslam_amd/csrc/gs_common.h
@@ -6,7 +6,7 @@
 
 #include "../../include/gradslam_hip.h"
 
-#define GS_ABI_VERSION 3
+#define GS_ABI_VERSION 4
 
 constexpr int GS_MAX_BATCH = 8;
 struct GsClearJob {
@@ -22,13 +22,16 @@
   int32_t* any_flag[GS_MAX_BATCH];
   int32_t* call_flag;
 };
+struct GsHandoverJob;
 int gs_frame_maps_batch_clear(const float* depth, int64_t depth_stride_seq, int64_t depth_stride_frame, const float* K16,
                               int n_frames, int frames_per_K, int H, int W, float two_sigma_sq, float* vertex,
                               float* normal, float* alpha, const GsClearJob* job, void* stream,
-                              const GsPixelTables* tables = nullptr);
-
+                              const GsPixelTables* tables = nullptr, const GsHandoverJob* handover = nullptr);
+
+struct GsTargetEmit;
 int gs_update_map_fusion_batch_impl(const gs_update_seq* seqs_host, int B, int H, int W, float dist_th, float dot_th,
-                                    int renorm_all, void* stream, bool tables_ready);
+                                    int renorm_all, void* stream, bool tables_ready, const GsTargetEmit* targets = nullptr,
+                                    int ds = 0);
 int32_t* gs_update_map_call_flag(void* scratch_of_first_sequence);
 void gs_update_map_tables(void* scratch, int32_t** any_flag, uint64_t** key_pix);
 
@@ -158,6 +161,49 @@
   return v < c.host ? (v < 0 ? 0 : v) : c.host;
 }
 
+constexpr unsigned long long GS_HANDOVER_MAGIC = 0x31764f4854534721ull;
+struct GsHandover {
+  unsigned long long magic;
+  float pose16[16];
+  int64_t count;
+  const float* points;
+  int64_t rows;
+  int H, W, ds;
+  unsigned taken;
+};
+static_assert(sizeof(GsHandover) <= 256, "record slot");
+struct GsHandoverQuery {
+  GsHandover* rec;
+  const float* pose16;
+  GsCount n_tgt;
+  const float* points;
+  int64_t rows;
+  int H, W, ds;
+  int force;
+};
+GS_DEV bool gs_handover_valid(const GsHandoverQuery& h) {
+  if (!h.rec || h.force) return false;
+  const GsHandover* r = h.rec;
+  bool ok = r->magic == GS_HANDOVER_MAGIC && r->count == gs_count(h.n_tgt) && r->points == h.points && r->rows == h.rows &&
+            r->H == h.H && r->W == h.W && r->ds == h.ds;
+#pragma unroll
+  for (int i = 0; i < 16; ++i) ok = ok && __float_as_uint(r->pose16[i]) == __float_as_uint(h.pose16[i]);
+  return ok;
+}
+struct GsHandoverJob {
+  int n;
+  unsigned keep_lo16, keep_hi16;
+  GsHandoverQuery q[GS_MAX_BATCH];
+};
+struct GsTargetEmit {
+  int32_t* pix;
+  unsigned* bbox;
+  float4* tlist;
+  GsHandover* rec;
+  int64_t rows;
+  int emit;
+};
+
 constexpr int GS_WAVE = 64;
 
 GS_DEV int gs_wave_incl_scan(int v) {
diff --git a/gradslam_amd/csrc/gs_frame.hip b/gradslam_amd/csrc/gs_frame.hip
--- a/gradslam_amd/csrc/gs_frame.hip
+++ b/gradslam_amd/csrc/gs_frame.hip
@@ -188,7 +188,8 @@
 __global__ void __launch_bounds__(256) gs_frame_maps_batch_kernel(
     const float* __restrict__ depth, int64_t stride_seq, int64_t stride_frame, const float* __restrict__ K16,
     int frames_per_K, int H, int W, float two_sigma_sq, float* __restrict__ vertex, float* __restrict__ normal,
-    float* __restrict__ alpha, const int n_frames, const GsClearJob job, const GsPixelTables tabs) {
+    float* __restrict__ alpha, const int n_frames, const GsClearJob job, const GsPixelTables tabs,
+    const GsHandoverJob ho) {
   if ((int)blockIdx.z >= n_frames) {
     const size_t blk = ((size_t)(blockIdx.z - n_frames) * gridDim.y + blockIdx.y) * gridDim.x + blockIdx.x;
     const size_t n16 = job.bytes / 16, per = (n16 + 256 * GS_CLEAR_ITEMS - 1) / (256 * GS_CLEAR_ITEMS);
@@ -196,10 +197,15 @@
     if (r >= (size_t)job.n) return;
     float4* dst = reinterpret_cast<float4*>(job.ptr[r]);
     const size_t base = (blk % per) * 256 * GS_CLEAR_ITEMS + threadIdx.x;
+    size_t keep_lo = 0, keep_hi = 0;
+    if (blk % per == 0 && (int)r < ho.n && ho.q[r].rec) {
+      if (gs_handover_valid(ho.q[r])) { keep_lo = ho.keep_lo16; keep_hi = ho.keep_hi16; }
+      if (threadIdx.x == 0) ho.q[r].rec->taken = 0u;
+    }
 #pragma unroll
     for (int u = 0; u < GS_CLEAR_ITEMS; ++u) {
       const size_t i = base + (size_t)u * 256;
-      if (i < n16) dst[i] = make_float4(0.0f, 0.0f, 0.0f, 0.0f);
+      if (i < n16 && !(i >= keep_lo && i < keep_hi)) dst[i] = make_float4(0.0f, 0.0f, 0.0f, 0.0f);
     }
     return;
   }
@@ -233,8 +239,14 @@
 int gs_frame_maps_batch_clear(const float* depth, int64_t depth_stride_seq, int64_t depth_stride_frame, const float* K16,
                               int n_frames, int frames_per_K, int H, int W, float two_sigma_sq, float* vertex,
                               float* normal, float* alpha, const GsClearJob* job, void* stream,
-                              const GsPixelTables* tables) {
+                              const GsPixelTables* tables, const GsHandoverJob* handover) {
   GS_REQUIRE(depth && K16 && vertex, "depth, K16 and vertex must not be NULL");
+  GsHandoverJob ho;
+  ho.n = 0; ho.keep_lo16 = ho.keep_hi16 = 0;
+  if (handover && handover->n > 0) {
+    GS_REQUIRE(job && handover->n <= job->n && handover->keep_hi16 <= 256 * GS_CLEAR_ITEMS, "bad hand-over job");
+    ho = *handover;
+  }
   GsPixelTables tabs;
   tabs.n = 0; tabs.call_flag = nullptr;
   if (tables && tables->n > 0) {
@@ -260,7 +272,7 @@
                        (double)tabs.n * H * W * 12.0;
   GsProf prof(GS_PROF_FRAME, bytes, gs_stream(stream));
   hipLaunchKernelGGL(gs_frame_maps_batch_kernel, grid, dim3(256), 0, gs_stream(stream), depth, depth_stride_seq,
-                     depth_stride_frame, K16, frames_per_K, H, W, two_sigma_sq, vertex, normal, alpha, n_frames, *job, tabs);
+                     depth_stride_frame, K16, frames_per_K, H, W, two_sigma_sq, vertex, normal, alpha, n_frames, *job, tabs, ho);
   GS_LAUNCH_CHECK();
   return GS_OK;
 }
diff --git a/gradslam_amd/csrc/gs_fuse.hip b/gradslam_amd/csrc/gs_fuse.hip
--- a/gradslam_amd/csrc/gs_fuse.hip
+++ b/gradslam_amd/csrc/gs_fuse.hip
@@ -1,5 +1,6 @@
 #include "gs_assoc_dev.h"
 #include "gs_compact.h"
+#include "gs_knn_bbox.h"
 
 __global__ void __launch_bounds__(256) gs_fuse_init_kernel(int32_t* __restrict__ pix_of, int64_t n,
                                                            int32_t* __restrict__ any_flag) {
@@ -88,7 +89,7 @@
 template <class Frame>
 GS_DEV void fuse_merge_row(float* __restrict__ points, float* __restrict__ normals, float* __restrict__ colors,
                            float* __restrict__ ccounts, const int64_t n, const int32_t p, const Frame& frame,
-                           const float* __restrict__ rgb, const float* __restrict__ alpha) {
+                           const float* __restrict__ rgb, const float* __restrict__ alpha, float* P_final = nullptr) {
   const float a = p >= 0 ? alpha[p] : 0.0f;
   const float cc = ccounts[n];
   float P[3], N[3], C[3], fp[3] = {0.0f, 0.0f, 0.0f}, fn[3] = {0.0f, 0.0f, 0.0f}, fc[3] = {0.0f, 0.0f, 0.0f};
@@ -113,6 +114,10 @@
   }
 #pragma unroll
   for (int k = 0; k < 3; ++k) points[3 * n + k] = P[k];
+  if (P_final) {
+#pragma unroll
+    for (int k = 0; k < 3; ++k) P_final[k] = P[k];
+  }
 #pragma unroll
   for (int k = 0; k < 3; ++k) normals[3 * n + k] = N[k];
 #pragma unroll
@@ -152,8 +157,12 @@
   const float* rgb;
   const float* alpha;
   __device__ void operator()(int64_t p, int64_t pos) const {
+    float v[3];
+    emit_v(p, pos, v);
+  }
+  __device__ void emit_v(int64_t p, int64_t pos, float* v) const {
     const int64_t r = gs_count(n_map) + pos;
-    float v[3], nn[3] = {0.0f, 0.0f, 0.0f}, c[3] = {0.0f, 0.0f, 0.0f};
+    float nn[3] = {0.0f, 0.0f, 0.0f}, c[3] = {0.0f, 0.0f, 0.0f};
     frame.vertex_of(p, v);
     if (normals) frame.normal_of(p, nn);
     if (colors) {
@@ -386,9 +395,15 @@
   uint64_t* key_pt;
   int32_t* pix;
   int32_t* pix_of;
+  int32_t* t_pix;
+  unsigned* t_bbox;
+  float4* t_tlist;
+  GsHandover* t_rec;
+  int64_t t_rows;
 };
 struct MuBatch {
   int B, H, W, renorm_all;
+  int ds, emit;
   int64_t P, ntiles;
   float u_hi, v_hi, dist_th, dot_th;
   int32_t* call_flag;
@@ -489,11 +504,89 @@
   mu_settle_ties(q, blk, gridDim.x / mb.B);
 }
 
-GS_DEV void mu_merge_body(const MuBatch& mb, const unsigned bid) {
-  const MuSeq& q = mb.s[bid % mb.B];
-  const int64_t n = (int64_t)(bid / mb.B) * 256 + threadIdx.x;
-  if (n >= gs_count(q.n_map)) return;
-  if (*mb.call_flag == 0) return;
+GS_DEV GsCamera mu_emit_camera(const MuSeq& q) {
+  GsCamera c = gs_camera(q.pose16, q.K16);
+#pragma unroll
+  for (int i = 0; i < 9; ++i) c.Ri[i] = __int_as_float(__builtin_amdgcn_readfirstlane(__float_as_int(c.Ri[i])));
+#pragma unroll
+  for (int i = 0; i < 3; ++i) c.ti[i] = __int_as_float(__builtin_amdgcn_readfirstlane(__float_as_int(c.ti[i])));
+#pragma unroll
+  for (int i = 0; i < 12; ++i) c.K[i] = __int_as_float(__builtin_amdgcn_readfirstlane(__float_as_int(c.K[i])));
+  return c;
+}
+struct MuEmitAcc {
+  int hits;
+  float lo[3], hi[3];
+};
+GS_DEV MuEmitAcc mu_emit_acc() {
+  return MuEmitAcc{0, {3.0e38f, 3.0e38f, 3.0e38f}, {-3.0e38f, -3.0e38f, -3.0e38f}};
+}
+GS_DEV bool mu_emit_row(const MuBatch& mb, const MuSeq& q, const GsCamera& cam, const int64_t n, const float* v,
+                        MuEmitAcc& a) {
+  int ph = 0, pw = 0;
+  const bool in = gs_project_point_hw(cam, v[0], v[1], v[2], mb.H, mb.W, mb.u_hi, mb.v_hi, ph, pw);
+  q.t_pix[n] = in ? (int32_t)(ph * mb.W + pw) : -1;
+  if (!(in && gs_on_lattice(ph, pw, mb.ds))) return false;
+  ++a.hits;
+#pragma unroll
+  for (int k = 0; k < 3; ++k) {
+    const float w = v[k];
+    if (w > -3.0e38f && w < 3.0e38f) {
+      a.lo[k] = w < a.lo[k] ? w : a.lo[k];
+      a.hi[k] = w > a.hi[k] ? w : a.hi[k];
+    }
+  }
+  return true;
+}
+template <int ITEMS, class Entry>
+GS_DEV void mu_emit_block(const MuSeq& q, const MuEmitAcc& acc, const unsigned hitmask, const Entry& entry) {
+  __shared__ float red[6][256 / GS_WAVE];
+  __shared__ int scan_s[256 / GS_WAVE + 1];
+  __shared__ unsigned base_s;
+  const int lane = threadIdx.x & 63, wave = threadIdx.x >> 6;
+#pragma unroll
+  for (int k = 0; k < 3; ++k) {
+    float a = acc.lo[k], b = acc.hi[k];
+#pragma unroll
+    for (int d = 32; d > 0; d >>= 1) {
+      const float a2 = __shfl_down(a, d, GS_WAVE), b2 = __shfl_down(b, d, GS_WAVE);
+      a = a2 < a ? a2 : a;
+      b = b2 > b ? b2 : b;
+    }
+    if (lane == 0) { red[k][wave] = a; red[3 + k][wave] = b; }
+  }
+  __syncthreads();
+  int total;
+  int pos = gs_block_excl_scan<256>(acc.hits, scan_s, &total);
+  if (total == 0) return;
+  if (threadIdx.x == 0) base_s = atomicAdd(&q.t_bbox[6], (unsigned)total);
+  __syncthreads();
+  if (hitmask) {
+    const unsigned base = base_s;
+#pragma unroll
+    for (int u = 0; u < ITEMS; ++u) {
+      if (hitmask & (1u << u)) {
+        q.t_tlist[base + (unsigned)pos] = entry(u);
+        ++pos;
+      }
+    }
+  }
+  if (threadIdx.x < 3) {
+    const int k = threadIdx.x;
+    float a = red[k][0], b = red[3 + k][0];
+    for (int w = 1; w < 256 / GS_WAVE; ++w) {
+      a = red[k][w] < a ? red[k][w] : a;
+      b = red[3 + k][w] > b ? red[3 + k][w] : b;
+    }
+    if (a <= b) {
+      atomicMax(&q.t_bbox[k], ~grid_code(a));
+      atomicMax(&q.t_bbox[3 + k], grid_code(b));
+    }
+  }
+}
+
+GS_DEV bool mu_merge_row(const MuBatch& mb, const MuSeq& q, const int64_t n, float* P) {
+  if (*mb.call_flag == 0) return false;
   int32_t p = q.pix[n];
   if (p >= 0) {
     bool win = q.key_pt[n] == q.key_pix[p];
@@ -504,15 +597,65 @@
     }
     if (!win) p = -1;
   }
-  if (p < 0 && !mb.renorm_all) return;
-  if (q.gvertex) fuse_merge_row(q.points, q.normals, q.colors, q.ccounts, n, p, FrameGlobalMaps{q.gvertex, q.gnormal}, q.rgb, q.alpha);
-  else fuse_merge_row(q.points, q.normals, q.colors, q.ccounts, n, p, frame_local_maps(q.vertex, q.normal, q.pose16), q.rgb, q.alpha);
+  if (p < 0 && !mb.renorm_all) return false;
+  if (q.gvertex) fuse_merge_row(q.points, q.normals, q.colors, q.ccounts, n, p, FrameGlobalMaps{q.gvertex, q.gnormal}, q.rgb, q.alpha, P);
+  else fuse_merge_row(q.points, q.normals, q.colors, q.ccounts, n, p, frame_local_maps(q.vertex, q.normal, q.pose16), q.rgb, q.alpha, P);
+  return true;
+}
+
+GS_DEV void mu_merge_body(const MuBatch& mb, const unsigned bid) {
+  const MuSeq& q = mb.s[bid % mb.B];
+  const int64_t n0 = (int64_t)(bid / mb.B) * 256, n = n0 + threadIdx.x;
+  const int64_t n_map = gs_count(q.n_map);
+  if (n0 >= n_map) return;
+  const bool targets = mb.emit && q.t_rec;
+  const bool live = n < n_map;
+  float P[3] = {0.0f, 0.0f, 0.0f};
+  const bool rewritten = live && mu_merge_row(mb, q, n, P);
+  if (!targets) return;
+  MuEmitAcc acc = mu_emit_acc();
+  unsigned hitmask = 0;
+  const GsCamera cam = mu_emit_camera(q);
+  if (live) {
+    if (!rewritten) {
+#pragma unroll
+      for (int k = 0; k < 3; ++k) P[k] = q.points[3 * n + k];
+    }
+    hitmask = mu_emit_row(mb, q, cam, n, P, acc) ? 1u : 0u;
+  }
+  mu_emit_block<1>(q, acc, hitmask, [&](int) { return make_float4(P[0], P[1], P[2], __int_as_float((int)n)); });
+}
+
+template <class Emit>
+GS_DEV void mu_append_rows(const MuBatch& mb, const MuSeq& q, const Emit& emit, const int64_t tile_base,
+                           const unsigned short* loc_s, const int tile_prefix, const int tile_new, const int64_t n_map,
+                           const bool targets) {
+  MuEmitAcc acc = mu_emit_acc();
+  unsigned hitmask = 0;
+  GsCamera cam;
+  if (targets) cam = mu_emit_camera(q);
+  const int64_t row0 = n_map + (int64_t)tile_prefix + threadIdx.x;
+  int i = 0;
+  for (int r = threadIdx.x; r < tile_new; r += GS_CP_BLOCK, ++i) {
+    const int64_t pos = (int64_t)tile_prefix + r;
+    if (n_map + pos < q.capacity) {
+      float v[3];
+      emit.emit_v(tile_base + loc_s[r], pos, v);
+      if (targets && mu_emit_row(mb, q, cam, n_map + pos, v, acc)) hitmask |= 1u << i;
+    }
+  }
+  if (targets)
+    mu_emit_block<GS_CP_ITEMS>(q, acc, hitmask, [&](int u) {
+      const int64_t row = row0 + (int64_t)u * GS_CP_BLOCK;
+      return make_float4(q.points[3 * row], q.points[3 * row + 1], q.points[3 * row + 2], __int_as_float((int)row));
+    });
 }
 
 GS_DEV void mu_append_body(const MuBatch& mb, const unsigned bid) {
   __shared__ int smem[GS_CP_BLOCK / GS_WAVE + 1];
   const MuSeq& q = mb.s[bid % mb.B];
   const unsigned blk = bid / mb.B;
+  const bool targets = mb.emit && q.t_rec;
   int before = 0, all = 0;
   for (int64_t t = threadIdx.x; t < mb.ntiles; t += GS_CP_BLOCK) {
     const int v = q.tile_counts[t];
@@ -523,7 +666,21 @@
   (void)gs_block_excl_scan<GS_CP_BLOCK>(before, smem, &tile_prefix);
   (void)gs_block_excl_scan<GS_CP_BLOCK>(all, smem, &total_new);
   const int64_t n_map = gs_count(q.n_map);
-  if (blk == 0 && threadIdx.x == 0) q.new_count_out[0] = n_map + total_new;
+  if (blk == 0 && threadIdx.x == 0) {
+    q.new_count_out[0] = n_map + total_new;
+    if (GsHandover* rec = q.t_rec) {
+      if (mb.emit) {
+        for (int i = 0; i < 16; ++i) rec->pose16[i] = q.pose16[i];
+        rec->count = n_map + total_new;
+        rec->points = q.points;
+        rec->rows = q.t_rows;
+        rec->H = mb.H; rec->W = mb.W; rec->ds = mb.ds;
+        rec->magic = GS_HANDOVER_MAGIC;
+      } else {
+        rec->magic = 0ull;
+      }
+    }
+  }
   const int64_t base = (int64_t)blk * GS_CP_TILE + (int64_t)threadIdx.x * GS_CP_ITEMS;
   bool keep[GS_CP_ITEMS];
   int c = 0;
@@ -552,17 +709,11 @@
   const int64_t tile_base = (int64_t)blk * GS_CP_TILE;
   if (q.gvertex) {
     const EmitAppend emit{q.points, q.normals, q.colors, q.ccounts, q.n_map, FrameGlobalMaps{q.gvertex, q.gnormal}, q.rgb, q.alpha};
-    for (int r = threadIdx.x; r < tile_new; r += GS_CP_BLOCK) {
-      const int64_t pos = (int64_t)tile_prefix + r;
-      if (n_map + pos < q.capacity) emit(tile_base + loc_s[r], pos);
-    }
+    mu_append_rows(mb, q, emit, tile_base, loc_s, tile_prefix, tile_new, n_map, targets);
   } else {
     const EmitAppendT<FrameLocalMaps> emit{q.points, q.normals, q.colors, q.ccounts, q.n_map,
                                            frame_local_maps(q.vertex, q.normal, q.pose16), q.rgb, q.alpha};
-    for (int r = threadIdx.x; r < tile_new; r += GS_CP_BLOCK) {
-      const int64_t pos = (int64_t)tile_prefix + r;
-      if (n_map + pos < q.capacity) emit(tile_base + loc_s[r], pos);
-    }
+    mu_append_rows(mb, q, emit, tile_base, loc_s, tile_prefix, tile_new, n_map, targets);
   }
 }
 
@@ -586,16 +737,19 @@
 }
 
 static int update_chunk(const gs_update_seq* seqs, int B, int H, int W, float dist_th, float dot_th, int renorm_all,
-                        hipStream_t st, int phase, int32_t* call_flag, bool first_chunk, bool tables_ready) {
+                        hipStream_t st, int phase, int32_t* call_flag, bool first_chunk, bool tables_ready,
+                        const GsTargetEmit* targets, int ds) {
   MuBatch mb;
   mb.B = B; mb.H = H; mb.W = W; mb.renorm_all = renorm_all;
+  mb.ds = ds;
+  mb.emit = (targets && targets[0].emit && renorm_all != 0 && ds > 0) ? 1 : 0;
   mb.call_flag = call_flag; mb.zero_call_flag = first_chunk ? 1 : 0;
   mb.P = (int64_t)H * W;
   mb.ntiles = gs_cp_tiles(mb.P);
   mb.u_hi = (float)((double)W - 0.999); mb.v_hi = (float)((double)H - 0.999);
   mb.dist_th = dist_th; mb.dot_th = dot_th;
   int64_t n_max = 0;
-  double bytes_assoc = 0.0, bytes_fuse = 0.0;
+  double bytes_assoc = 0.0, bytes_fuse = 0.0, bytes_emit = 0.0;
   for (int b = 0; b < B; ++b) {
     const gs_update_seq& u = seqs[b];
     const int64_t n_map = u.map.n_bound;
@@ -614,8 +768,14 @@
     m.key_pt = reinterpret_cast<uint64_t*>(q); q += gs_align(8 * (size_t)(n_map > 0 ? n_map : 1));
     m.pix = reinterpret_cast<int32_t*>(q); q += gs_align(4 * (size_t)(n_map > 0 ? n_map : 1));
     m.pix_of = reinterpret_cast<int32_t*>(q);
+    m.t_pix = nullptr; m.t_bbox = nullptr; m.t_tlist = nullptr; m.t_rec = nullptr; m.t_rows = 0;
+    if (targets) {
+      const GsTargetEmit& t = targets[b];
+      m.t_pix = t.pix; m.t_bbox = t.bbox; m.t_tlist = t.tlist; m.t_rec = t.rec; m.t_rows = t.rows;
+    }
     bytes_assoc += 72.0 * (double)n_map;
     bytes_fuse += 104.0 * (double)n_map + 49.0 * (double)mb.P;
+    if (mb.emit) bytes_emit += 24.0 * (double)n_map;
   }
   const unsigned uB = (unsigned)B;
   const unsigned pb = uB * (unsigned)gs_ceil_div(mb.P, 256), nb = uB * (unsigned)gs_ceil_div(n_max > 0 ? n_max : 1, 256);
@@ -631,7 +791,7 @@
     GsProf prof(GS_PROF_FUSE, bytes_fuse / 3.0, st, 1);
     hipLaunchKernelGGL(gs_mu_winner_count_kernel, dim3(uB * (unsigned)mb.ntiles), dim3(GS_CP_BLOCK), 0, st, mb);
   } else {
-    GsProf prof(GS_PROF_FUSE, bytes_fuse * (2.0 / 3.0), st, 1);
+    GsProf prof(GS_PROF_FUSE, bytes_fuse * (2.0 / 3.0) + bytes_emit, st, 1);
     const unsigned nb_append = uB * (unsigned)mb.ntiles;
     hipLaunchKernelGGL(gs_mu_merge_append_kernel, dim3(nb_append + (n_max > 0 ? nb : 0u)), dim3(256), 0, st, mb, nb_append);
   }
@@ -640,8 +800,9 @@
 }
 
 int gs_update_map_fusion_batch_impl(const gs_update_seq* seqs_host, int B, int H, int W, float dist_th, float dot_th,
-                                    int renorm_all, void* stream, bool tables_ready) {
+                                    int renorm_all, void* stream, bool tables_ready, const GsTargetEmit* targets, int ds) {
   GS_REQUIRE(seqs_host && B > 0 && H > 0 && W > 0, "bad arguments");
+  GS_REQUIRE(!targets || ds > 0, "target hand-over needs the lattice step");
   GS_REQUIRE((int64_t)H * W < (1ll << 31), "too large for int32 indices");
   for (int b = 0; b < B; ++b) {
     const gs_update_seq& u = seqs_host[b];
@@ -659,7 +820,7 @@
     for (int c0 = 0; c0 < B; c0 += GS_MAX_BATCH) {
       const int nb = B - c0 < GS_MAX_BATCH ? B - c0 : GS_MAX_BATCH;
       const int rc = update_chunk(seqs_host + c0, nb, H, W, dist_th, dot_th, renorm_all, st, phase, call_flag, c0 == 0,
-                                  tables_ready);
+                                  tables_ready, targets ? targets + c0 : nullptr, ds);
       if (rc != GS_OK) return rc;
     }
   }
diff --git a/gradslam_amd/csrc/gs_icp_loop.hip b/gradslam_amd/csrc/gs_icp_loop.hip
--- a/gradslam_amd/csrc/gs_icp_loop.hip
+++ b/gradslam_amd/csrc/gs_icp_loop.hip
@@ -1198,6 +1198,7 @@
   int* lstat;
   float4* wl_cq;
   unsigned* sync;
+  GsHandover* ho_reset;
 };
 struct LocBatch {
   int B, W, ds, Wl;
@@ -1249,6 +1250,7 @@
         for (int i = 0; i < 3 * GL_STAT_LAUNCHES; ++i) q.lstat[i] = 0;
       if (q.sync)
         for (int i = 0; i < PS_WORDS; ++i) q.sync[i] = 0u;
+      if (q.ho_reset) { q.ho_reset->magic = 0ull; q.ho_reset->taken = 0u; }
       if (lb.numiters == 0) icp_write_result(sm, q.pose16, q.out_pose16);
     }
     return;
@@ -1293,6 +1295,8 @@
   const float* compose16[GS_MAX_BATCH];
   float* out_T16[GS_MAX_BATCH];
   unsigned* sync[GS_MAX_BATCH];
+  unsigned* ho_bbox[GS_MAX_BATCH];
+  GsHandover* ho_rec[GS_MAX_BATCH];
   int nb, h0;
 };
 __global__ void __launch_bounds__(FS_BLOCK) gs_icp_finish_batch_kernel(const IcpFinishBatch fb, GsCount n_src_c, int buf,
@@ -1314,6 +1318,10 @@
       for (int i = 0; i < 16; ++i) fb.out_T16[b][i] = __builtin_nanf("");
     sy[PS_NB] = (unsigned)fb.nb;
     sy[PS_H0] = (unsigned)fb.h0;
+  }
+  if (unsigned* bb = fb.ho_bbox[b]) {
+    for (int i = 0; i < 7; ++i) bb[i] = 0u;
+    fb.ho_rec[b]->magic = 0ull;
   }
 }
 
@@ -1430,7 +1438,7 @@
 extern "C" int64_t gs_localize_scratch_bytes(int H, int W, int ds, int64_t n_map_bound) {
   if (H < 1 || W < 1 || ds < 1) return 0;
   const int64_t n_lat = loc_lattice(H, W, ds);
-  return (int64_t)(gs_align(12 * (size_t)n_lat) + gs_align(4 * (size_t)(n_map_bound > 0 ? n_map_bound : 1)) + 256) +
+  return (int64_t)(gs_align(12 * (size_t)n_lat) + gs_align(4 * (size_t)(n_map_bound > 0 ? n_map_bound : 1)) + 256 + 256) +
          gs_icp_scratch_bytes(n_lat, n_map_bound) + (int64_t)list_mem_bytes(n_lat) +
          (int64_t)far_mem_bytes(n_lat);
 }
@@ -1441,6 +1449,7 @@
   float* lattice;
   int32_t* pix;
   int64_t* n_valid;
+  GsHandover* ho;
   IcpScratch sc;
   GridMem gm;
 };
@@ -1451,6 +1460,7 @@
   const int64_t rows = loc_rows(q.map);
   c.pix = reinterpret_cast<int32_t*>(p); p += gs_align(4 * (size_t)rows);
   c.n_valid = reinterpret_cast<int64_t*>(p); p += 256;
+  c.ho = reinterpret_cast<GsHandover*>(p); p += 256;
   c.sc = icp_carve(p, n_lat);
   c.gm = grid_carve(c.sc.grid, n_lat, rows);
   return c;
@@ -1471,7 +1481,7 @@
 }
 
 static int localize_chunk(const gs_localize_seq* seqs, int B, int H, int W, int ds, const gs_icp_params* prm,
-                          hipStream_t st, bool grid_cleared) {
+                          hipStream_t st, bool grid_cleared, const int* force_rebuild = nullptr) {
   const int64_t n_lat = loc_lattice(H, W, ds);
   const int Wl = (W + ds - 1) / ds;
   LocBatch lb;
@@ -1493,7 +1503,8 @@
     gm[b] = cv.gm;
     lb.s[b] = LocSeq{q.vertex, q.depth, q.prev_pose16, lattice, sc[b].state, q.out_pose16,
                      reinterpret_cast<char*>(gm[b].g), n_valid, nullptr, nullptr, nullptr,
-                     reinterpret_cast<unsigned*>(sc[b].rowred + LIN_NV)};
+                     reinterpret_cast<unsigned*>(sc[b].rowred + LIN_NV),
+                     grid_cleared ? nullptr : cv.ho};
     static int binned_normals = -1;
     if (binned_normals < 0) {
       const char* e = getenv("GRADSLAM_HIP_ICP_BINNED_NORMALS");
@@ -1501,7 +1512,8 @@
     }
     if (!binned_normals) gm[b].sorted_n = nullptr;
     gb.s[b] = GsGridSeq{q.map.points, GsCount{q.map.n_bound, q.map.n_dev}, pix, q.prev_pose16, q.K16,
-                        binned_normals ? q.map.normals : nullptr, gm[b]};
+                        binned_normals ? q.map.normals : nullptr, gm[b], grid_cleared ? cv.ho : nullptr, loc_rows(q.map),
+                        force_rebuild ? force_rebuild[b] : 1};
     if (g_gs_prof_on) GS_HIP(hipMemsetAsync(n_valid, 0, 8, st));
   }
   static int far_lists = -1;
@@ -1547,7 +1559,8 @@
   const unsigned nb_clear = (unsigned)gs_ceil_div((int64_t)(lb.clear_bytes / 16), 256 * LP_CLEAR_ITEMS);
   {
     double bytes = 0.0;
-    for (int b = 0; b < B; ++b) bytes += 28.0 * n_lat + 24.0 * seqs[b].map.n_bound + 16.0 * gb.cells_cap;
+    for (int b = 0; b < B; ++b)
+      bytes += 28.0 * n_lat + (gb.s[b].rec && !gb.s[b].force ? 0.0 : 24.0 * seqs[b].map.n_bound) + 16.0 * gb.cells_cap;
     GsProf prof(GS_PROF_COMPACT, bytes, st, grid_cleared ? 4 : 5);
     int rc;
     if (grid_cleared) {
@@ -1726,6 +1739,8 @@
       fb.compose16[b] = seqs[b].prev_pose16;
       fb.out_T16[b] = seqs[b].out_pose16;
       fb.sync[b] = persist_on ? lb.s[b].sync : nullptr;
+      fb.ho_bbox[b] = grid_cleared ? gm[b].bbox : nullptr;
+      fb.ho_rec[b] = gb.s[b].rec;
     }
     hipLaunchKernelGGL(gs_icp_finish_batch_kernel, dim3((unsigned)B), dim3(FS_BLOCK), 0, st, fb, n_src_c, h & 1, *prm);
   }
@@ -1734,7 +1749,7 @@
 }
 
 static int localize_batch(const gs_localize_seq* seqs_host, int B, int H, int W, int ds, const gs_icp_params* prm,
-                          void* stream, bool grid_cleared) {
+                          void* stream, bool grid_cleared, const int* force_rebuild = nullptr) {
   GS_REQUIRE(seqs_host && prm && B > 0 && H > 0 && W > 0 && ds > 0, "bad arguments");
   GS_REQUIRE(prm->numiters >= 0 && prm->numiters <= GS_ICP_MAX_ITERS, "numiters must be in [0, 1024]");
   GS_REQUIRE(prm->mode == 0 || prm->mode == 1, "mode must be 0 (ICP) or 1 (gradICP)");
@@ -1749,7 +1764,7 @@
   hipStream_t st = gs_stream(stream);
   for (int c0 = 0; c0 < B; c0 += GS_MAX_BATCH) {
     const int nb = B - c0 < GS_MAX_BATCH ? B - c0 : GS_MAX_BATCH;
-    const int rc = localize_chunk(seqs_host + c0, nb, H, W, ds, prm, st, grid_cleared);
+    const int rc = localize_chunk(seqs_host + c0, nb, H, W, ds, prm, st, grid_cleared, force_rebuild ? force_rebuild + c0 : nullptr);
     if (rc != GS_OK) return rc;
   }
   return GS_OK;
@@ -1838,6 +1853,45 @@
   return GS_OK;
 }
 
+extern "C" int64_t gs_localize_handover_offset(int H, int W, int ds, int64_t map_rows) {
+  if (H < 1 || W < 1 || ds < 1 || map_rows < 1) return -1;
+  gs_localize_seq q;
+  memset(&q, 0, sizeof(q));
+  q.map.capacity = map_rows; q.map.n_bound = map_rows;
+  return (int64_t)reinterpret_cast<intptr_t>(loc_carve(q, loc_lattice(H, W, ds)).ho);
+}
+
+extern "C" int gs_localize_handover_stats_i64(const void* scratch, int H, int W, int ds, int64_t map_rows, int64_t* out4_host,
+                                              void* stream) {
+  GS_REQUIRE(scratch && out4_host && H > 0 && W > 0 && ds > 0 && map_rows > 0, "bad arguments");
+  const int64_t n_lat = loc_lattice(H, W, ds);
+  gs_localize_seq q;
+  memset(&q, 0, sizeof(q));
+  q.scratch = const_cast<void*>(scratch);
+  q.map.capacity = map_rows; q.map.n_bound = map_rows;
+  const LocCarve cv = loc_carve(q, n_lat);
+  GsHandover h;
+  unsigned listed = 0;
+  hipStream_t st = gs_stream(stream);
+  GS_HIP(hipMemcpyAsync(&h, cv.ho, sizeof(h), hipMemcpyDeviceToHost, st));
+  GS_HIP(hipMemcpyAsync(&listed, cv.gm.bbox + 6, 4, hipMemcpyDeviceToHost, st));
+  GS_HIP(hipStreamSynchronize(st));
+  out4_host[0] = (int64_t)h.taken;
+  out4_host[1] = h.magic == GS_HANDOVER_MAGIC ? 1 : 0;
+  out4_host[2] = out4_host[1] ? h.count : 0;
+  out4_host[3] = out4_host[1] ? (int64_t)listed : 0;
+  return GS_OK;
+}
+
+static bool handover_enabled() {
+  static int on = -1;
+  if (on < 0) {
+    const char* e = getenv("GRADSLAM_HIP_TARGET_HANDOVER");
+    on = (e && atoi(e) == 0) ? 0 : 1;
+  }
+  return on == 1;
+}
+
 extern "C" int gs_pointfusion_step_batch_f32(const gs_step_seq* seqs_host, int B, int H, int W, int ds,
                                              const gs_icp_params* prm, float two_sigma_sq, float dist_th, float dot_th,
                                              int renorm_all, void* stream) {
@@ -1859,6 +1913,10 @@
   GS_REQUIRE(dstride >= P || B == 1, "overlapping depth images");
   const bool implicit_global = s0.gvertex == nullptr;
   std::unique_ptr<gs_update_seq[]> us(new gs_update_seq[B]);
+  const bool ho_on = handover_enabled();
+  const bool ho_emit = ho_on && prm->numiters > 0 && renorm_all != 0;
+  std::unique_ptr<GsTargetEmit[]> te(new GsTargetEmit[B]);
+  std::unique_ptr<int[]> force(new int[B]);
   for (int c0 = 0; c0 < B; c0 += GS_MAX_BATCH) {
     const int nb = B - c0 < GS_MAX_BATCH ? B - c0 : GS_MAX_BATCH;
     const gs_step_seq* sq = seqs_host + c0;
@@ -1872,15 +1930,23 @@
       u.alpha = q.alpha; u.pose16 = q.out_pose16; u.K16 = q.K16; u.gvertex = q.gvertex;
       u.gnormal = q.gnormal; u.best_pix = q.best_pix; u.new_count_out = q.new_count_out;
       u.scratch = q.upd_scratch;
+      force[c0 + b] = (!ho_on || q.force_rebuild) ? 1 : 0;
     }
     const int64_t n_lat = loc_lattice(H, W, ds);
     GsClearJob job;
     job.n = nb;
+    GsHandoverJob hoj;
+    hoj.n = nb;
     for (int b = 0; b < nb; ++b) {
       GS_REQUIRE(ls[b].map.points && ls[b].map.n_bound > 0, "every sequence needs a non-empty map");
       const LocCarve cv = loc_carve(ls[b], n_lat);
       job.ptr[b] = reinterpret_cast<char*>(cv.gm.g);
       if (b == 0) job.bytes = gs_knn_grid_clear_bytes(cv.gm, gs_knn_grid_cells_cap(n_lat));
+      hoj.q[b] = GsHandoverQuery{cv.ho, ls[b].prev_pose16, GsCount{ls[b].map.n_bound, ls[b].map.n_dev}, ls[b].map.points,
+                                 loc_rows(ls[b].map), H, W, ds, force[c0 + b]};
+      hoj.keep_lo16 = (unsigned)((reinterpret_cast<char*>(cv.gm.bbox) - reinterpret_cast<char*>(cv.gm.g)) / 16);
+      hoj.keep_hi16 = hoj.keep_lo16 + 2;
+      te[c0 + b] = GsTargetEmit{cv.pix, cv.gm.bbox, cv.gm.tlist, cv.ho, loc_rows(ls[b].map), ho_emit ? 1 : 0};
     }
     GsPixelTables tabs{};
     tabs.n = implicit_global ? nb : 0;
@@ -1890,12 +1956,12 @@
       tabs.best_pix[b] = sq[b].best_pix;
     }
     int rc = gs_frame_maps_batch_clear(sq[0].depth, dstride, P, sq[0].K16, nb, 1, H, W, two_sigma_sq, sq[0].vertex,
-                                       sq[0].normal, sq[0].alpha, &job, stream, &tabs);
+                                       sq[0].normal, sq[0].alpha, &job, stream, &tabs, &hoj);
     if (rc != GS_OK) return rc;
-    rc = localize_batch(ls, nb, H, W, ds, prm, stream, true);
+    rc = localize_batch(ls, nb, H, W, ds, prm, stream, true, force.get() + c0);
     if (rc != GS_OK) return rc;
   }
-  return gs_update_map_fusion_batch_impl(us.get(), B, H, W, dist_th, dot_th, renorm_all, stream, implicit_global);
+  return gs_update_map_fusion_batch_impl(us.get(), B, H, W, dist_th, dot_th, renorm_all, stream, implicit_global, te.get(), ds);
 }
 
 extern "C" int64_t gs_icp_tape_bytes(int64_t n_src, int numiters) { return (int64_t)gs_icp_tape_size(n_src, numiters); }
diff --git a/gradslam_amd/csrc/gs_knn.h b/gradslam_amd/csrc/gs_knn.h
--- a/gradslam_amd/csrc/gs_knn.h
+++ b/gradslam_amd/csrc/gs_knn.h
@@ -69,6 +69,9 @@
   const float* K16;
   const float* nrm;
   GridMem m;
+  GsHandover* rec;
+  int64_t rows;
+  int force;
 };
 struct GsGridBatch {
   int B, H, W, ds;
diff --git a/gradslam_amd/csrc/gs_knn_bbox.h b/gradslam_amd/csrc/gs_knn_bbox.h
--- a/gradslam_amd/csrc/gs_knn_bbox.h
+++ b/gradslam_amd/csrc/gs_knn_bbox.h
@@ -136,6 +136,16 @@
   const GsGridSeq& q = gb.s[bid % gb.B];
   const unsigned blk = bid / gb.B;
   const GsTargetFilter flt{q.pix, gb.W, gb.ds};
+  if (q.rec && q.pose16) {
+    const GsHandoverQuery h{q.rec, q.pose16, q.n_tgt, q.tgt, q.rows, gb.H, gb.W, gb.ds, q.force};
+    if (gs_handover_valid(h)) {
+      if (threadIdx.x == 0) {
+        if (blk == 0) { q.m.unres_count[0] = 0; q.m.unres_count[1] = 0; }
+        if ((int64_t)blk * GB_BLOCK * GB_ITEMS < gs_count(q.n_tgt)) atomicAdd(&q.rec->taken, 1u);
+      }
+      return;
+    }
+  }
   if (q.pose16) {
     const GsCamera cam = gs_camera(q.pose16, q.K16);
     grid_bbox_body(q.tgt, gs_count(q.n_tgt), flt, &cam, gb.H, u_hi, v_hi, q.pix, q.m.bbox, q.m.unres_count, q.m.tlist,
diff --git a/gradslam_amd/slam/_fastpath.py b/gradslam_amd/slam/_fastpath.py
--- a/gradslam_amd/slam/_fastpath.py
+++ b/gradslam_amd/slam/_fastpath.py
@@ -50,6 +50,7 @@
         self.caps = [-1] * B
         self.bufs = [None] * B
         self.scratch = [None] * B
+        self.stepped = [None] * B
         self.stream = _C.stream(device)
         self.stream_id = torch.cuda.current_stream(device).cuda_stream
 
@@ -66,9 +67,12 @@
             ws = _C.Workspace.get(self.device)
             loc = ws.bytes("localize%d" % b, self.lib.gs_localize_scratch_bytes(self.H, self.W, self.ds, cap))
             upd = ws.bytes("map_update%d" % b, self.lib.gs_update_map_scratch_bytes(cap, self.H, self.W))
+            off = int(self.lib.gs_localize_handover_offset(self.H, self.W, self.ds, cap))
+            loc[off:off + 256].zero_()
             self.scratch[b] = (loc, upd)
             q.loc_scratch, q.upd_scratch = loc.data_ptr(), upd.data_ptr()
             self.caps[b] = cap
+            self.stepped[b] = None
         self.bufs[b] = bufs
         return True
 
@@ -117,8 +121,14 @@
             q.new_count_out = c0 + 8 * b
             q.map.n_bound = bounds[b]
             q.map.n_dev = n_dev0 + 8 * b
+            last = self.stepped[b]
+            q.force_rebuild = 0 if (last is not None and last[2] is grp.dev and
+                                    all(t is u for t, u in zip(last[0], self.bufs[b])) and
+                                    last[1] == tuple(int(t._version) for t in self.bufs[b])) else 1
         _C.check(self.lib.gs_pointfusion_step_batch_f32(seqs, B, H, W, self.ds, self.prm, self.tss, self.dist_th,
                                                         self.dot_th, 1 if RENORMALIZE_UNMATCHED else 0, self.stream), "gs_pointfusion_step_batch_f32")
+        for b in range(B):
+            self.stepped[b] = (self.bufs[b], tuple(int(t._version) for t in self.bufs[b]), cnt_new)
         n3 = 3 * P * B
         live._vertex_map = out[:n3].view(B, 1, H, W, 3)
         live._normal_map = out[n3:2 * n3].view(B, 1, H, W, 3)
diff --git a/include/gradslam_hip.h b/include/gradslam_hip.h
--- a/include/gradslam_hip.h
+++ b/include/gradslam_hip.h
@@ -288,10 +288,14 @@
   gs_map_view map;
   void* loc_scratch;
   void* upd_scratch;
+  int32_t force_rebuild;
 } gs_step_seq;
 GS_API int gs_pointfusion_step_batch_f32(const gs_step_seq* seqs_host, int B, int H, int W, int ds,
                                          const gs_icp_params* params_host, float two_sigma_sq, float dist_th,
                                          float dot_th, int renorm_all, void* stream);
+GS_API int64_t gs_localize_handover_offset(int H, int W, int ds, int64_t map_rows);
+GS_API int gs_localize_handover_stats_i64(const void* scratch, int H, int W, int ds, int64_t map_rows, int64_t* out4_host,
+                                          void* stream);
 
 GS_API int gs_project_points_f32(const float* cam_coords, int cdim, int64_t n, const float* proj16, int64_t pts_per_mat,
                                  float* out_uv, void* stream);
```

Result: no change. 3793 (-0.4%).
